# lambdaclass/AES_zero_knowledge_proof_circuit

Hardware: AMD Instinct MI355X
Metric: AES-ECB blocks proven/sec (Marlin), proof verifies (higher is better)
Workload: dtype u32 limbs (253-bit Fr / 377-bit Fq modular integers)

## Files before the change

aes_zero_knowledge_proof_circuit_amd/api.py:

```python
import ctypes as C
import os

import numpy as np

HERE = os.path.dirname(os.path.abspath(__file__))
CIRCUIT_AES, CIRCUIT_OPS_XOR, CIRCUIT_OPS_ADD = 0, 1, 2
CIRCUIT_AES_CBC = 3
CIRCUIT_AES_CTR = 4
CIRCUIT_AES_GCM = 5
KEY_NO_TABLES = 1
PARITY = "parity"


class ZkAesError(RuntimeError):
    """The Err(..) side of the reference's anyhow::Result."""


def lib_path():
    return os.path.join(HERE, "libzkaes.so")


_lib = None


# ... 627 lines not shown
    return out.raw[:32 * n]


def z_poly_from_w(w, x_poly, n):
    out = C.create_string_buffer(32 * (n + 1))
    _check(lib().zkaes_z_poly_from_w(bytes(w), C.c_size_t(len(w) // 32), bytes(x_poly), C.c_uint32(len(x_poly) // 32), C.c_size_t(n), out))
    return out.raw


def ntt_padded(field_id, data_mont_bytes, n, inverse=False, coset_c=0, lg_big=0):
    out = C.create_string_buffer(32 * n)
    _check(lib().zkaes_ntt_padded(int(field_id), bytes(data_mont_bytes), C.c_size_t(len(data_mont_bytes) // 32), C.c_size_t(n), 1 if inverse else 0, int(coset_c), int(lg_big), out))
    return out.raw


def ntt_scaled(g, data_mont_bytes, n, inverse=False):
    out = C.create_string_buffer(32 * n)
    _check(lib().zkaes_ntt_scaled(bytes(g), bytes(data_mont_bytes), C.c_size_t(len(data_mont_bytes) // 32), C.c_size_t(n), 1 if inverse else 0, out))
    return out.raw


def _arith_ops():
    t = {}
    for base, f, n in ((0, "fr377", 8), (16, "fr381", 8), (32, "fq377", 12), (48, "fq381", 12)):
        for i, (name, nin) in enumerate((("mul", 2 * n), ("add", 2 * n), ("sub", 2 * n), ("neg", n), ("dbl", n), ("inverse", n), ("from_i64", 2), ("pow_u64", n + 2), ("from_raw", n), ("to_raw", n))):
            t["%s.%s" % (f, name)] = (base + i, nin, n)
    for base, f in ((64, "fq377x28"), (96, "fq381x28")):
        ops = [("mul", 28, 14), ("sqr", 14, 14), ("fma2", 56, 14), ("add", 28, 14), ("add_lazy", 28, 14), ("dbl_lazy", 14, 14)]
        ops += [("sub%d" % k, 28, 14) for k in (2, 3, 4, 5, 6, 7)] + [("sub_lazy%d" % k, 28, 14) for k in (2, 3)]
        ops += [("canonical", 14, 14), ("product_is_zero", 14, 1), ("is_zero_mod_p", 14, 1), ("from_std", 12, 14), ("to_std", 14, 12)]
        if f == "fq377x28":
            ops.append(("mul_biased", 28, 14))
        for i, (name, nin, nout) in enumerate(ops):
            t["%s.%s" % (f, name)] = (base + i, nin, nout)
    for base, f in ((128, "fr377x29"), (160, "fr381x29")):
        ops = [("mul", 18, 9), ("dot2", 36, 9), ("dot3", 54, 9), ("dot4", 72, 9), ("add", 18, 9), ("add_lazy", 18, 9)]
        ops += [("sub%d" % k, 18, 9) for k in (1, 2, 4, 8)] + [("sub_lazy2", 18, 9), ("normalized", 9, 9), ("shl5", 9, 9)]
        ops += [("canonical%d" % k, 9, 9) for k in (0, 1, 4)] + [("reduce_by_top_limb", 9, 9), ("twiddle_from_std", 8, 9), ("split", 8, 9), ("pack", 9, 8)]
        for i, (name, nin, nout) in enumerate(ops):
            t["%s.%s" % (f, name)] = (base + i, nin, nout)
    for i, (name, nin, nout) in enumerate((("te_madd", 98, 56), ("te_add", 112, 56), ("te_dbl", 56, 56), ("te_neg", 56, 56), ("te_to_std_point", 56, 48), ("niels_from_weierstrass", 24, 43),
                                           ("te_madd_hot", 142, 98), ("te_add_quad", 112, 56), ("te_dbl_quad", 56, 56))):
        t["te377.%s" % name] = (192 + i, nin, nout)
    for base, f in ((208, "w377"), (216, "w381")):
        for i, (name, nin, nout) in enumerate((("madd28", 84, 57), ("add28", 112, 56), ("dbl28", 56, 56), ("neg28", 56, 56), ("to_std_point", 56, 48))):
            t["%s.%s" % (f, name)] = (base + i, nin, nout)
    return t


ARITH_OPS = _arith_ops()
ARITH_QUAD_OPS = ("te377.te_add_quad", "te377.te_dbl_quad")


def arith_probe(op_name, cases):
    op, nin, nout = ARITH_OPS[op_name]
    cases = bytes(cases)
    n, rest = divmod(len(cases), 4 * nin)
    if rest:
        raise ZkAesError("arith_probe: %s takes %d words per case" % (op_name, nin))
    out = C.create_string_buffer(4 * nout * n or 1)
    _check(lib().zkaes_arith_probe(int(op), cases, C.c_size_t(n), out))
    return out.raw[:4 * nout * n]


def msm(curve_id, bases_bytes, scalars_bytes):
    n = len(scalars_bytes) // 32
    out = C.create_string_buffer(96)
    inf = C.c_int()
    _check(lib().zkaes_msm(int(curve_id), bytes(bases_bytes), bytes(scalars_bytes), C.c_size_t(n), out, C.byref(inf)))
    return out.raw, bool(inf.value)


def g1_sum(curve_id, points):
    n = len(points)
    buf = b"".join(bytes(p[0]) for p in points)
    inf = (C.c_int * max(n, 1))(*[1 if p[1] else 0 for p in points])
    out = C.create_string_buffer(96)
    oinf = C.c_int()
    _check(lib().zkaes_g1_sum(int(curve_id), buf, inf, C.c_size_t(n), out, C.byref(oinf)))
    return out.raw, bool(oinf.value)


def msm_sharded_plan(curve_id, n_total):
    c, w, b = C.c_int(), C.c_int(), C.c_size_t()
    _check(lib().zkaes_msm_sharded_plan(int(curve_id), C.c_size_t(n_total), C.byref(c), C.byref(w), C.byref(b)))
    return c.value, w.value, b.value


def msm_window_sums_dev(curve_id, bases_bytes, scalars_bytes, n_total, dev_ptr, dev_bytes):
    n = len(scalars_bytes) // 32
    _check(lib().zkaes_msm_window_sums_dev(int(curve_id), bytes(bases_bytes), bytes(scalars_bytes), C.c_size_t(n), C.c_size_t(n_total), C.c_void_p(dev_ptr), C.c_size_t(dev_bytes)))


def msm_fold_window_sums_dev(curve_id, dev_ptr, world, n_total):
    out = C.create_string_buffer(96)
    inf = C.c_int()
    _check(lib().zkaes_msm_fold_window_sums_dev(int(curve_id), C.c_void_p(dev_ptr), int(world), C.c_size_t(n_total), out, C.byref(inf)))
    return out.raw, bool(inf.value)


def msm_fold_partials_dev(curve_id, dev_ptr, world):
    out = C.create_string_buffer(96)
    inf = C.c_int()
    _check(lib().zkaes_msm_fold_partials_dev(int(curve_id), C.c_void_p(dev_ptr), int(world), out, C.byref(inf)))
    return out.raw, bool(inf.value)


def msm_table(curve_id, bases_bytes, scalars_bytes, window_bits, srs=False):
    n = len(scalars_bytes) // 32
    out = C.create_string_buffer(96)
    inf = C.c_int()
    if srs:
        if int(curve_id) != 377:
            raise ValueError("the SRS (twisted Edwards) table path exists for BLS12-377 only")
        _check(lib().zkaes_msm_table_srs(bytes(bases_bytes), bytes(scalars_bytes), C.c_size_t(n), int(window_bits), out, C.byref(inf)))
    else:
        _check(lib().zkaes_msm_table(int(curve_id), bytes(bases_bytes), bytes(scalars_bytes), C.c_size_t(n), int(window_bits), out, C.byref(inf)))
    return out.raw, bool(inf.value)


def msm_bench(curve_id, bases_bytes, scalars_bytes, reps=3):
    n = len(scalars_bytes) // 32
    t, a = C.c_double(), C.c_double()
    _check(lib().zkaes_msm_bench(int(curve_id), bytes(bases_bytes), bytes(scalars_bytes), C.c_size_t(n), int(reps), C.byref(t), C.byref(a)))
    return t.value, a.value


def msm_bench_synth(n, window_bits=0, reps=3, want_point=False):
    t, a = C.c_double(), C.c_double()
    out = C.create_string_buffer(96)
    _check(lib().zkaes_msm_bench_synth(C.c_size_t(n), int(window_bits), int(reps), C.byref(t), C.byref(a), out))
    return (t.value, a.value, out.raw) if want_point else (t.value, a.value)


def set_default_contexts(n):
    _check(lib().zkaes_set_default_contexts(C.c_size_t(n)))


def srs_hold(hold=True):
    _check(lib().zkaes_srs_hold(1 if hold else 0))


def int_rate_bench(seconds=0.5):
    out = (C.c_double * 8)()
    _check(lib().zkaes_int_rate_bench(C.c_double(seconds), out))
    return {"fq_products_per_s": out[0], "fq_stream_sclk_mhz": out[1], "mad_per_s": 378.0 * out[0], "hot_loop_l2_additions_per_s": out[2], "hot_loop_l2_sclk_mhz": out[3],
            "hot_loop_cycles_per_addition_per_wave": out[4], "rounds": int(out[5])}


def stream_copy_bench(nbytes=1 << 30, reps=20):
    g = C.c_double()
    _check(lib().zkaes_stream_copy_bench(C.c_size_t(nbytes), int(reps), C.byref(g)))
    return g.value


def mem_info():
    f, t = C.c_uint64(), C.c_uint64()
    _check(lib().zkaes_mem_info(C.byref(f), C.byref(t)))
    return int(f.value), int(t.value)


def msm_stats(reset=False):
    out = (C.c_double * 5)()
    _check(lib().zkaes_msm_stats(out, 1 if reset else 0))
    return dict(accumulate_ms=out[0], total_ms=out[1], points=int(out[2]), launches=int(out[3]), pairs=int(out[4]))
```

aes_zero_knowledge_proof_circuit_amd/csrc/arith_probe.cuh:

```cuda
#pragma once
#include "ff29.cuh"
#include "te28.cuh"

namespace zk {
namespace probe {

template <class T> ZK_HD T ld(const uint32_t *in) { T r; for (int i = 0; i < T::N; i++) r.l[i] = in[i]; return r; }
template <class T> ZK_HD void st(uint32_t *out, const T &v) { for (int i = 0; i < T::N; i++) out[i] = v.l[i]; }
struct OpBase { static constexpr bool QUAD = false; };

#define ZK_PROBE_UN(NAME, EXPR)                                                                                                                   \
    template <class T> struct NAME : OpBase { static constexpr int NIN = T::N, NOUT = T::N;                                                       \
        ZK_HD static void run(const uint32_t *in, uint32_t *out, uint64_t) { const T a = ld<T>(in); st<T>(out, EXPR); } };
#define ZK_PROBE_BIN(NAME, EXPR)                                                                                                                  \
    template <class T> struct NAME : OpBase { static constexpr int NIN = 2 * T::N, NOUT = T::N;                                                   \
        ZK_HD static void run(const uint32_t *in, uint32_t *out, uint64_t) { const T a = ld<T>(in), b = ld<T>(in + T::N); st<T>(out, EXPR); } };
#define ZK_PROBE_BIN_K(NAME, EXPR)                                                                                                                \
    template <class T, int K> struct NAME : OpBase { static constexpr int NIN = 2 * T::N, NOUT = T::N;                                            \
        ZK_HD static void run(const uint32_t *in, uint32_t *out, uint64_t) { const T a = ld<T>(in), b = ld<T>(in + T::N); st<T>(out, EXPR); } };
ZK_PROBE_BIN(Mul, a * b)
ZK_PROBE_BIN(Add, a + b)
ZK_PROBE_BIN(Sub, a - b)
ZK_PROBE_UN(Neg, a.neg())
ZK_PROBE_UN(Dbl, a.dbl())
// ... 32 lines not shown
    ZK_HD static void run(const uint32_t *in, uint32_t *out, uint64_t bias) { st<G>(out, G::mul_biased(ld<G>(in), ld<G>(in + G::N), bias)); } };

template <class S, int M> struct Dot : OpBase { static constexpr int NIN = 2 * M * S::N, NOUT = S::N;
    ZK_HD static void run(const uint32_t *in, uint32_t *out, uint64_t) {
        S a[M], b[M];
        for (int i = 0; i < M; i++) { a[i] = ld<S>(in + i * S::N); b[i] = ld<S>(in + (M + i) * S::N); }
        st<S>(out, S::template dot<M>(a, b));
    } };
template <class P> struct TwiddleFromStd : OpBase { static constexpr int NIN = P::N, NOUT = 9;
    ZK_HD static void run(const uint32_t *in, uint32_t *out, uint64_t) { st<Fp29<P>>(out, Fp29<P>::twiddle_from_std(ld<Fp<P>>(in))); } };
template <class P> struct Split29 : OpBase { static constexpr int NIN = P::N, NOUT = 9;
    ZK_HD static void run(const uint32_t *in, uint32_t *out, uint64_t) { st<Fp29<P>>(out, Fp29<P>::split(in)); } };
template <class P> struct Pack29 : OpBase { static constexpr int NIN = 9, NOUT = P::N;
    ZK_HD static void run(const uint32_t *in, uint32_t *out, uint64_t) { ld<Fp29<P>>(in).pack(out); } };

constexpr int GW = 14, PTW = 4 * GW, NIW = 3 * GW;
template <class P> ZK_HD AccTE<P> ld_te(const uint32_t *in) { AccTE<P> a; a.x = ld<FpMsm<P>>(in); a.y = ld<FpMsm<P>>(in + GW); a.z = ld<FpMsm<P>>(in + 2 * GW); a.t = ld<FpMsm<P>>(in + 3 * GW); return a; }
template <class P> ZK_HD void st_te(uint32_t *out, const AccTE<P> &a) { st(out, a.x); st(out + GW, a.y); st(out + 2 * GW, a.z); st(out + 3 * GW, a.t); }
template <class P> ZK_HD Acc28<P> ld_acc(const uint32_t *in) { Acc28<P> a; a.x = ld<FpMsm<P>>(in); a.y = ld<FpMsm<P>>(in + GW); a.zz = ld<FpMsm<P>>(in + 2 * GW); a.zzz = ld<FpMsm<P>>(in + 3 * GW); return a; }
template <class P> ZK_HD void st_acc(uint32_t *out, const Acc28<P> &a) { st(out, a.x); st(out + GW, a.y); st(out + 2 * GW, a.zz); st(out + 3 * GW, a.zzz); }
template <class P> ZK_HD Niels28<P> ld_niels(const uint32_t *in) {
    Niels28<P> n; n.ymx = ld<FpMsm<P>>(in); n.ypx = ld<FpMsm<P>>(in + GW); n.td = ld<FpMsm<P>>(in + 2 * GW);
    for (int i = 0; i < 6; i++) n.pad[i] = 0;
    return n;
}
template <class P> ZK_HD void st_niels(uint32_t *out, const Niels28<P> &n) { st(out, n.ymx); st(out + GW, n.ypx); st(out + 2 * GW, n.td); }
template <class P> ZK_HD void st_xyzz(uint32_t *out, const XYZZ<Fp<P>> &o) { st(out, o.x); st(out + P::N, o.y); st(out + 2 * P::N, o.zz); st(out + 3 * P::N, o.zzz); }

struct TeMadd : OpBase { using P = Fq377P; static constexpr int NIN = PTW + NIW, NOUT = PTW;
    ZK_HD static void run(const uint32_t *in, uint32_t *out, uint64_t) { AccTE<P> a = ld_te<P>(in); te_madd<P>(a, ld_niels<P>(in + PTW)); st_te<P>(out, a); } };
struct TeAdd : OpBase { using P = Fq377P; static constexpr int NIN = 2 * PTW, NOUT = PTW;
    ZK_HD static void run(const uint32_t *in, uint32_t *out, uint64_t) { AccTE<P> a = ld_te<P>(in); te_add<P>(a, ld_te<P>(in + PTW)); st_te<P>(out, a); } };
struct TeDbl : OpBase { using P = Fq377P; static constexpr int NIN = PTW, NOUT = PTW;
    ZK_HD static void run(const uint32_t *in, uint32_t *out, uint64_t) { AccTE<P> a = ld_te<P>(in); te_dbl<P>(a); st_te<P>(out, a); } };
struct TeNeg : OpBase { using P = Fq377P; static constexpr int NIN = PTW, NOUT = PTW;
    ZK_HD static void run(const uint32_t *in, uint32_t *out, uint64_t) { st_te<P>(out, te_neg<P>(ld_te<P>(in))); } };
struct TeToStd : OpBase { using P = Fq377P; static constexpr int NIN = PTW, NOUT = 4 * P::N;
    ZK_HD static void run(const uint32_t *in, uint32_t *out, uint64_t) { st_xyzz<P>(out, te_to_std_point<P>(ld_te<P>(in))); } };
struct NielsFromW : OpBase { using P = Fq377P; static constexpr int NIN = 2 * P::N, NOUT = NIW + 1;
    ZK_HD static void run(const uint32_t *in, uint32_t *out, uint64_t) {
        Affine<Fp<P>> p; p.x = ld<Fp<P>>(in); p.y = ld<Fp<P>>(in + P::N);
        bool bad = false;
        st_niels<P>(out, niels_from_weierstrass(p, &bad));
        out[NIW] = bad ? 1u : 0u;
    } };
struct TeMaddHot : OpBase { using P = Fq377P; static constexpr int NIN = PTW + 2 * NIW + 2, NOUT = PTW + NIW;
    ZK_HD static void run(const uint32_t *in, uint32_t *out, uint64_t bias) {
        AccTE<P> a = ld_te<P>(in);
        Niels28<P> n = ld_niels<P>(in + PTW);
        const Niels28<P> next = ld_niels<P>(in + PTW + NIW);
        te_madd_hot<P>(a, n, in[PTW + 2 * NIW] != 0, &next, in[PTW + 2 * NIW + 1] != 0, bias);
        st_te<P>(out, a); st_niels<P>(out + PTW, n);
    } };
template <class P> struct Madd28 : OpBase { static constexpr int NIN = PTW + 2 * GW, NOUT = PTW + 1;
    ZK_HD static void run(const uint32_t *in, uint32_t *out, uint64_t) {
        Acc28<P> a = ld_acc<P>(in);
        Affine28<P> q; q.x = ld<FpMsm<P>>(in + PTW); q.y = ld<FpMsm<P>>(in + PTW + GW);
        const bool ok = madd28<P>(a, q);
        st_acc<P>(out, a); out[PTW] = ok ? 1u : 0u;
    } };
template <class P> struct Add28 : OpBase { static constexpr int NIN = 2 * PTW, NOUT = PTW;
    ZK_HD static void run(const uint32_t *in, uint32_t *out, uint64_t) { Acc28<P> a = ld_acc<P>(in); add28<P>(a, ld_acc<P>(in + PTW)); st_acc<P>(out, a); } };
template <class P> struct Dbl28 : OpBase { static constexpr int NIN = PTW, NOUT = PTW;
    ZK_HD static void run(const uint32_t *in, uint32_t *out, uint64_t) { Acc28<P> a = ld_acc<P>(in); dbl28<P>(a); st_acc<P>(out, a); } };
template <class P> struct Neg28 : OpBase { static constexpr int NIN = PTW, NOUT = PTW;
    ZK_HD static void run(const uint32_t *in, uint32_t *out, uint64_t) { st_acc<P>(out, neg28<P>(ld_acc<P>(in))); } };
template <class P> struct ToStdPoint28 : OpBase { static constexpr int NIN = PTW, NOUT = 4 * P::N;
    ZK_HD static void run(const uint32_t *in, uint32_t *out, uint64_t) { st_xyzz<P>(out, to_std_point<P>(ld_acc<P>(in))); } };

struct TeAddQuad { using P = Fq377P; static constexpr bool QUAD = true; static constexpr int NIN = 2 * PTW, NOUT = PTW;
#if defined(__HIPCC__)
    __device__ __forceinline__ static void run_quad(const uint32_t *in, uint32_t *out, int q) { st(out + q * GW, te_add_quad<P>(ld<FpMsm<P>>(in + q * GW), ld<FpMsm<P>>(in + PTW + q * GW), q)); }
#endif
};
struct TeDblQuad { using P = Fq377P; static constexpr bool QUAD = true; static constexpr int NIN = PTW, NOUT = PTW;
#if defined(__HIPCC__)
    __device__ __forceinline__ static void run_quad(const uint32_t *in, uint32_t *out, int q) { st(out + q * GW, te_dbl_quad<P>(ld<FpMsm<P>>(in + q * GW), q)); }
#endif
};

#define ZK_PROBE_FP(X, B, F)                                                                                                                      \
    X(B + 0, Mul<F>) X(B + 1, Add<F>) X(B + 2, Sub<F>) X(B + 3, Neg<F>) X(B + 4, Dbl<F>) X(B + 5, Inverse<F>) X(B + 6, FromI64<F>) X(B + 7, PowU64<F>)       \
    X(B + 8, FromRaw<F>) X(B + 9, ToRaw<F>)
#define ZK_PROBE_FP28(X, B, P)                                                                                                                    \
    X(B + 0, Mul<Fp28<P>>) X(B + 1, Sqr<Fp28<P>>) X(B + 2, Fma2<Fp28<P>>) X(B + 3, Add<Fp28<P>>) X(B + 4, AddLazy<Fp28<P>>) X(B + 5, DblLazy<Fp28<P>>)          \
    X(B + 6, SubK<Fp28<P>, 2>) X(B + 7, SubK<Fp28<P>, 3>) X(B + 8, SubK<Fp28<P>, 4>) X(B + 9, SubK<Fp28<P>, 5>) X(B + 10, SubK<Fp28<P>, 6>) X(B + 11, SubK<Fp28<P>, 7>) \
    X(B + 12, SubLazyK<Fp28<P>, 2>) X(B + 13, SubLazyK<Fp28<P>, 3>) X(B + 14, Canonical<Fp28<P>>) X(B + 15, ProductIsZero<Fp28<P>>) X(B + 16, IsZeroModP<Fp28<P>>)   \
    X(B + 17, FromStd28<P>) X(B + 18, ToStd28<P>)
#define ZK_PROBE_FP29(X, B, P)                                                                                                                    \
    X(B + 0, Mul<Fp29<P>>) X(B + 1, Dot<Fp29<P>, 2>) X(B + 2, Dot<Fp29<P>, 3>) X(B + 3, Dot<Fp29<P>, 4>) X(B + 4, Add<Fp29<P>>) X(B + 5, AddLazy<Fp29<P>>)       \
    X(B + 6, SubK<Fp29<P>, 1>) X(B + 7, SubK<Fp29<P>, 2>) X(B + 8, SubK<Fp29<P>, 4>) X(B + 9, SubK<Fp29<P>, 8>) X(B + 10, SubLazyK<Fp29<P>, 2>)                \
    X(B + 11, Normalized<Fp29<P>>) X(B + 12, Shl5<Fp29<P>>) X(B + 13, CanonicalLog<Fp29<P>, 0>) X(B + 14, CanonicalLog<Fp29<P>, 1>) X(B + 15, CanonicalLog<Fp29<P>, 4>) \
    X(B + 16, ReduceTop<Fp29<P>>) X(B + 17, TwiddleFromStd<P>) X(B + 18, Split29<P>) X(B + 19, Pack29<P>)
#define ZK_PROBE_W28(X, B, P) X(B + 0, Madd28<P>) X(B + 1, Add28<P>) X(B + 2, Dbl28<P>) X(B + 3, Neg28<P>) X(B + 4, ToStdPoint28<P>)
#define ZK_PROBE_OPS(X)                                                                                                                           \
    ZK_PROBE_FP(X, 0, Fr377) ZK_PROBE_FP(X, 16, Fr381) ZK_PROBE_FP(X, 32, Fq377) ZK_PROBE_FP(X, 48, Fq381)                                         \
    ZK_PROBE_FP28(X, 64, Fq377P) X(64 + 19, MulBiased<Fp28<Fq377P>>) ZK_PROBE_FP28(X, 96, Fq381P)                                                  \
    ZK_PROBE_FP29(X, 128, Fr377P) ZK_PROBE_FP29(X, 160, Fr381P)                                                                                    \
    X(192, TeMadd) X(193, TeAdd) X(194, TeDbl) X(195, TeNeg) X(196, TeToStd) X(197, NielsFromW) X(198, TeMaddHot) X(199, TeAddQuad) X(200, TeDblQuad) \
    ZK_PROBE_W28(X, 208, Fq377P) ZK_PROBE_W28(X, 216, Fq381P)

template <class O> struct Tag { using type = O; };
template <class Fn> bool dispatch(int op, Fn &&fn) {
    switch (op) {
#define ZK_PROBE_CASE(ID, ...) case ID: fn(Tag<__VA_ARGS__>{}); return true;
        ZK_PROBE_OPS(ZK_PROBE_CASE)
#undef ZK_PROBE_CASE
        default: return false;
    }
}
constexpr int MAX_OP_ID = 224;
constexpr size_t MAX_CASES = (size_t)1 << 16;

}
}
```

aes_zero_knowledge_proof_circuit_amd/csrc/capi_kernels.hip:

```cpp
#include "../../include/zkaes.h"
#include <cstring>
#include <string>
#include <vector>
#include "hip_util.hpp"
#include "marlin.hpp"
#include "te28.cuh"
#include <algorithm>
#include <chrono>

typedef unsigned int v4u __attribute__((ext_vector_type(4)));
__global__ void __launch_bounds__(256) k_stream_copy(uint4 *__restrict__ dst_, const uint4 *__restrict__ src_, size_t n16) {
    v4u *dst = (v4u *)dst_; const v4u *src = (const v4u *)src_;
    size_t base = (size_t)blockIdx.x * 1024 + threadIdx.x;
    if (base + 768 < n16) {
        v4u v0 = __builtin_nontemporal_load(src + base), v1 = __builtin_nontemporal_load(src + base + 256);
        v4u v2 = __builtin_nontemporal_load(src + base + 512), v3 = __builtin_nontemporal_load(src + base + 768);
        __builtin_nontemporal_store(v0, dst + base); __builtin_nontemporal_store(v1, dst + base + 256);
        __builtin_nontemporal_store(v2, dst + base + 512); __builtin_nontemporal_store(v3, dst + base + 768);
    } else {
        for (size_t i = base; i < n16; i += 256) dst[i] = src[i];
    }
}


// ... 58 lines not shown
    if (!data) throw std::invalid_argument("zkaes_ntt: null data");
    zk::gpu::require_device();
    StreamGuard s;
    DevPtr<Fr> a(n), b(n);
    zk::gpu::h2d(a, data, n * sizeof(Fr), s);
    if (coset_c) zk::gpu::ntt_coset<Fr>(b, a, n, lg, inverse != 0, coset_c, lg_big, s);
    else zk::gpu::ntt<Fr>(b, a, n, lg, inverse != 0, s);
    zk::gpu::d2h(data, b, n * sizeof(Fr), s);
}
template <class Fr> void run_ntt_batch(uint8_t *data, size_t n, int count, int inverse, const int *coset_c, int lg_big) {
    const int lg = exact_log2(n, "zkaes_ntt_batch");
    if (count < 1 || count > 12) throw std::invalid_argument("zkaes_ntt_batch: 1..12 transforms");
    if (!data) throw std::invalid_argument("zkaes_ntt_batch: null data");
    zk::gpu::require_device();
    StreamGuard s;
    DevPtr<Fr> a((size_t)count * n), b((size_t)count * n);
    zk::gpu::h2d(a, data, (size_t)count * n * sizeof(Fr), s);
    zk::gpu::NttJob<Fr> jobs[12];
    for (int i = 0; i < count; i++) jobs[i] = zk::gpu::NttJob<Fr>{b + (size_t)i * n, a + (size_t)i * n, coset_c ? coset_c[i] : 0};
    zk::gpu::ntt_batch<Fr>(jobs, count, n, lg, inverse != 0, lg_big, s);
    zk::gpu::d2h(data, b, (size_t)count * n * sizeof(Fr), s);
}
template <class Fq> void give_affine(const zk::Affine<Fq> &a, uint8_t *out_xy, int *out_inf) {
    if (out_inf) *out_inf = a.is_inf() ? 1 : 0;
    if (out_xy) { memcpy(out_xy, a.x.l, 48); memcpy(out_xy + 48, a.y.l, 48); }
}
template <class Curve> void run_msm(const uint8_t *bases, const uint8_t *scalars, size_t n, uint8_t *out_xy, int *out_inf, int reps, double *ms_total, double *ms_acc) {
    using Fq = typename Curve::Fq; using Fr = typename Curve::Fr;
    if (n && (!bases || !scalars)) throw std::invalid_argument("zkaes_msm: null argument");
    if (n >= ((size_t)1 << 30)) throw std::invalid_argument("zkaes_msm: too many points");
    zk::gpu::require_device();
    StreamGuard s;
    DevPtr<zk::Affine<Fq>> db(n);
    DevPtr<Fr> ds(n);
    zk::gpu::h2d(db, bases, n * 96, s); zk::gpu::h2d(ds, scalars, n * 32, s);
    DevPtr<zk::Affine28<typename Curve::FqP>> db28(n);
    zk::gpu::convert_bases<Curve>(db28, db, n, s);
    zk::gpu::sync(s);
    WorkspaceGuard ws;
    zk::XYZZ<Fq> r = zk::gpu::msm<Curve>(ws, db28, ds, n, s);
    if (reps > 0) {
        zk::gpu::MsmStats before = zk::gpu::msm_stats(false);
        EventGuard e0, e1;
        zk::gpu::event_record(e0, s);
        for (int i = 0; i < reps; i++) r = zk::gpu::msm<Curve>(ws, db28, ds, n, s);
        zk::gpu::event_record(e1, s);
        float ms = zk::gpu::event_elapsed_ms(e0, e1);
        zk::gpu::MsmStats after = zk::gpu::msm_stats(false);
        if (ms_total) *ms_total = ms / reps;
        if (ms_acc) *ms_acc = (after.accumulate_ms - before.accumulate_ms) / reps;
    }
    give_affine(r.to_affine(), out_xy, out_inf);
}
template <class Curve, bool EDWARDS> void run_msm_table(const uint8_t *bases, const uint8_t *scalars, size_t n, int c, uint8_t *out_xy, int *out_inf) {
    using Fq = typename Curve::Fq; using Fr = typename Curve::Fr;
    if (c < 2 || c > 22) throw std::invalid_argument("window bits must be in [2, 22]");
    if (n && (!bases || !scalars)) throw std::invalid_argument("zkaes_msm_table: null argument");
    zk::gpu::require_device();
    const size_t nt = (size_t)zk::gpu::table_windows<Curve>(c);
    if ((uint64_t)nt * n >= (1ull << 30)) throw std::invalid_argument("zkaes_msm_table: n x table copies exceeds the 2^30 base indices of one MSM");
    StreamGuard s;
    DevPtr<zk::Affine<Fq>> tab(nt * n);
    DevPtr<Fr> ds(n);
    zk::gpu::h2d(tab, bases, n * 96, s); zk::gpu::h2d(ds, scalars, n * 32, s);
    zk::gpu::build_window_tables<Curve>(tab, n, c, s);
    WorkspaceGuard ws;
    zk::Affine<Fq> a;
    if constexpr (EDWARDS) {
        DevPtr<zk::Niels28<typename Curve::FqP>> tabte(nt * n);
        zk::gpu::convert_bases_te<Curve>(tabte, tab, nt * n, s);
        a = zk::gpu::msm_table<Curve>(ws, tabte, n, 0, c, ds, n, s).to_affine();
    } else {
        DevPtr<zk::Affine28<typename Curve::FqP>> tab28(nt * n);
        zk::gpu::convert_bases<Curve>(tab28, tab, nt * n, s);
        a = zk::gpu::msm_table<Curve>(ws, tab28, n, 0, c, ds, n, s).to_affine();
    }
    give_affine(a, out_xy, out_inf);
}
template <class Curve> void run_msm_window_sums_dev(const uint8_t *bases, const uint8_t *scalars, size_t n_local, size_t n_total, void *dev_out, size_t dev_out_bytes) {
    using Fq = typename Curve::Fq; using Fr = typename Curve::Fr;
    zk::gpu::require_device();
    int c = 0, nwin = 0;
    zk::gpu::msm_sharded_plan<Curve>(n_total, &c, &nwin);
    if (!dev_out || dev_out_bytes < (size_t)nwin * sizeof(zk::XYZZ<Fq>)) throw std::invalid_argument("zkaes_msm_window_sums_dev: device buffer too small for the window sums");
    if (n_local > n_total) throw std::invalid_argument("zkaes_msm_window_sums_dev: n_local > n_total");
    if (n_local && (!bases || !scalars)) throw std::invalid_argument("zkaes_msm_window_sums_dev: null argument");
    StreamGuard s;
    DevPtr<zk::Affine<Fq>> db(n_local);
    DevPtr<Fr> ds(n_local);
    zk::gpu::h2d(db, bases, n_local * 96, s); zk::gpu::h2d(ds, scalars, n_local * 32, s);
    DevPtr<zk::Affine28<typename Curve::FqP>> db28(n_local);
    zk::gpu::convert_bases<Curve>(db28, db, n_local, s);
    WorkspaceGuard ws;
    zk::gpu::msm_window_sums_device<Curve>(ws, db28, ds, n_local, n_total, (zk::XYZZ<Fq> *)dev_out, s);
}
constexpr int MAX_FOLD_WORLD = 4096;
template <class Curve> void run_msm_fold_dev(const void *dev_in, int world, size_t n_total, uint8_t *out_xy, int *out_inf) {
    using Fq = typename Curve::Fq;
    if (!dev_in || world < 1 || world > MAX_FOLD_WORLD) throw std::invalid_argument("zkaes_msm_fold_window_sums_dev: bad arguments (world must be 1..4096)");
    zk::gpu::require_device();
    StreamGuard s;
    give_affine(zk::gpu::msm_fold_window_sums_device<Curve>((const zk::XYZZ<Fq> *)dev_in, world, n_total, s).to_affine(), out_xy, out_inf);
}
template <class Curve> void run_g1_sum(const uint8_t *points_xy, const int *inf, size_t n, uint8_t *out_xy, int *out_inf) {
    using Fq = typename Curve::Fq;
    zk::XYZZ<Fq> acc = zk::XYZZ<Fq>::inf();
    for (size_t i = 0; i < n; i++) {
        if (inf && inf[i]) continue;
        zk::Affine<Fq> a;
        memcpy(a.x.l, points_xy + 96 * i, 48); memcpy(a.y.l, points_xy + 96 * i + 48, 48);
        acc.add(zk::XYZZ<Fq>::from_affine(a));
    }
    zk::Affine<Fq> r = acc.to_affine();
    *out_inf = r.is_inf() ? 1 : 0;
    memcpy(out_xy, r.x.l, 48); memcpy(out_xy + 48, r.y.l, 48);
}

using PF = zk::gpu::F;
PF load_f(const uint8_t *b, const char *who) {
    if (!b) throw std::invalid_argument(std::string(who) + ": null field element");
    PF x; memcpy(x.l, b, 32); return x;
}
void need(bool ok, const char *who, const char *what) { if (!ok) throw std::invalid_argument(std::string(who) + ": " + what); }
constexpr size_t POLY_MAX = (size_t)1 << 28;
// ... 1 lines not shown
    DevPtr<PF> d(count ? count : 1);
    zk::gpu::h2d(d, host, count * sizeof(PF), s);
    return d;
}
template <class Fr> void run_ntt_padded(const uint8_t *in, size_t in_len, size_t n, int inverse, int coset_c, int lg_big, uint8_t *out) {
    const int lg = exact_log2(n, "zkaes_ntt_padded");
    need(in_len <= n, "zkaes_ntt_padded", "in_len must not exceed n");
    need(out && (in || !in_len), "zkaes_ntt_padded", "null argument");
    need(coset_c >= 0, "zkaes_ntt_padded", "coset index must not be negative");
    zk::gpu::require_device();
    StreamGuard s;
    DevPtr<Fr> a(in_len ? in_len : 1), b(n);
    zk::gpu::h2d(a, in, in_len * sizeof(Fr), s);
    if (coset_c) zk::gpu::ntt_coset<Fr>(b, a, in_len, lg, inverse != 0, coset_c, lg_big, s);
    else zk::gpu::ntt<Fr>(b, a, in_len, lg, inverse != 0, s);
    zk::gpu::d2h(out, b, n * sizeof(Fr), s);
}
}

extern "C" {
int zkaes_msm_sharded_plan(int curve_id, size_t n_total, int *window_bits, int *n_windows, size_t *bytes_per_rank) {
    return guardk([&] {
        int c = 0, w = 0;
        if (curve_id == 381) zk::gpu::msm_sharded_plan<zk::Bls381>(n_total, &c, &w); else if (curve_id == 377) zk::gpu::msm_sharded_plan<zk::Bls377>(n_total, &c, &w); else throw std::invalid_argument("curve_id must be 377 or 381");
        if (window_bits) *window_bits = c;
        if (n_windows) *n_windows = w;
        if (bytes_per_rank) *bytes_per_rank = (size_t)w * 192;
    });
}
int zkaes_msm_window_sums_dev(int curve_id, const uint8_t *bases, const uint8_t *scalars, size_t n_local, size_t n_total, void *dev_out, size_t dev_out_bytes) {
    return guardk([&] { if (curve_id == 381) run_msm_window_sums_dev<zk::Bls381>(bases, scalars, n_local, n_total, dev_out, dev_out_bytes); else if (curve_id == 377) run_msm_window_sums_dev<zk::Bls377>(bases, scalars, n_local, n_total, dev_out, dev_out_bytes); else throw std::invalid_argument("curve_id must be 377 or 381"); });
}
int zkaes_msm_fold_window_sums_dev(int curve_id, const void *dev_in, int world, size_t n_total, uint8_t *out_xy, int *out_inf) {
    return guardk([&] { if (curve_id == 381) run_msm_fold_dev<zk::Bls381>(dev_in, world, n_total, out_xy, out_inf); else if (curve_id == 377) run_msm_fold_dev<zk::Bls377>(dev_in, world, n_total, out_xy, out_inf); else throw std::invalid_argument("curve_id must be 377 or 381"); });
}
int zkaes_g1_sum(int curve_id, const uint8_t *points_xy, const int *inf, size_t n, uint8_t *out_xy, int *out_inf) {
    return guardk([&] { if (curve_id == 381) run_g1_sum<zk::Bls381>(points_xy, inf, n, out_xy, out_inf); else if (curve_id == 377) run_g1_sum<zk::Bls377>(points_xy, inf, n, out_xy, out_inf); else throw std::invalid_argument("curve_id must be 377 or 381"); });
}
int zkaes_msm_fold_partials_dev(int curve_id, const void *dev_in, int world, uint8_t *out_xy, int *out_inf) {
    return guardk([&] {
        if (!dev_in || world < 1 || world > MAX_FOLD_WORLD) throw std::invalid_argument("zkaes_msm_fold_partials_dev: bad arguments (world must be 1..4096)");
        if (curve_id != 377 && curve_id != 381) throw std::invalid_argument("curve_id must be 377 or 381");
        zk::gpu::require_device();
        StreamGuard s;
        if (curve_id == 377) give_affine(zk::gpu::msm_fold_points_device<zk::Bls377>((const zk::XYZZ<zk::Fq377> *)dev_in, world, s).to_affine(), out_xy, out_inf);
        else give_affine(zk::gpu::msm_fold_points_device<zk::Bls381>((const zk::XYZZ<zk::Fq381> *)dev_in, world, s).to_affine(), out_xy, out_inf);
    });
}
int zkaes_msm_table(int curve_id, const uint8_t *bases, const uint8_t *scalars, size_t n, int window_bits, uint8_t *out_xy, int *out_inf) {
    return guardk([&] { if (curve_id == 381) run_msm_table<zk::Bls381, false>(bases, scalars, n, window_bits, out_xy, out_inf); else if (curve_id == 377) run_msm_table<zk::Bls377, false>(bases, scalars, n, window_bits, out_xy, out_inf); else throw std::invalid_argument("curve_id must be 377 or 381"); });
}
int zkaes_msm_table_srs(const uint8_t *bases, const uint8_t *scalars, size_t n, int window_bits, uint8_t *out_xy, int *out_inf) {
    return guardk([&] { run_msm_table<zk::Bls377, true>(bases, scalars, n, window_bits, out_xy, out_inf); });
}
int zkaes_set_device(int ordinal) { return guardk([&] { HIP_CHECK(hipSetDevice(ordinal)); }); }
int zkaes_ntt(int field_id, uint8_t *data, size_t n, int inverse) {
    return guardk([&] { if (field_id == 381) run_ntt<zk::Fr381>(data, n, inverse, 0, 0); else if (field_id == 377) run_ntt<zk::Fr377>(data, n, inverse, 0, 0); else throw std::invalid_argument("field_id must be 377 or 381"); });
}
int zkaes_ntt_coset(int field_id, uint8_t *data, size_t n, int inverse, int coset_c, int lg_big) {
    return guardk([&] {
        if (coset_c <= 0) throw std::invalid_argument("zkaes_ntt_coset: coset index must be positive");
        if (field_id == 381) run_ntt<zk::Fr381>(data, n, inverse, coset_c, lg_big); else if (field_id == 377) run_ntt<zk::Fr377>(data, n, inverse, coset_c, lg_big); else throw std::invalid_argument("field_id must be 377 or 381");
    });
}
int zkaes_ntt_batch(int field_id, uint8_t *data, size_t n, int count, int inverse, const int *coset_c, int lg_big) {
    return guardk([&] {
        if (field_id == 381) run_ntt_batch<zk::Fr381>(data, n, count, inverse, coset_c, lg_big); else if (field_id == 377) run_ntt_batch<zk::Fr377>(data, n, count, inverse, coset_c, lg_big);
        else throw std::invalid_argument("field_id must be 377 or 381");
    });
}
int zkaes_poly_divide_by_vanishing(const uint8_t *p, size_t len, size_t m, int with_scratch, uint8_t *q, uint8_t *rem_or_null) {
    return guardk([&] {
        const char *who = "zkaes_poly_divide_by_vanishing";
        if (m == 0 || len <= m) throw std::invalid_argument("divide_by_vanishing: dividend shorter than divisor");
        need(p && q, who, "null argument"); need(len <= POLY_MAX, who, "polynomial too long");
        zk::gpu::require_device();
        StreamGuard s;
        DevPtr<PF> dp = upload(p, len, s), dq(len - m), drem(m), scratch;
        size_t scratch_len = 0;
        if (with_scratch) { scratch_len = zk::gpu::divide_by_vanishing_scratch(len, m); scratch.alloc(scratch_len ? scratch_len : 1); }
        zk::gpu::divide_by_vanishing(dq, rem_or_null ? drem.get() : nullptr, dp, len, m, s, with_scratch ? scratch.get() : nullptr, scratch_len);
        zk::gpu::d2h(q, dq, (len - m) * sizeof(PF), s);
        if (rem_or_null) zk::gpu::d2h(rem_or_null, drem, m * sizeof(PF), s);
    });
}
int zkaes_poly_divide_by_linear(const uint8_t *p, size_t len, const uint8_t z[32], uint8_t *q) {
    return guardk([&] {
        const char *who = "zkaes_poly_divide_by_linear";
        const PF zf = load_f(z, who);
        need(len <= POLY_MAX, who, "polynomial too long"); need(len < 2 || (p && q), who, "null argument");
        if (len < 2) return;
        zk::gpu::require_device();
        StreamGuard s;
        const size_t scratch_len = zk::gpu::divide_by_linear_scratch(len);
        DevPtr<PF> dp = upload(p, len, s), dq(len - 1), scratch(scratch_len);
        zk::gpu::divide_by_linear(dq, dp, len, zf, scratch, scratch_len, s);
        zk::gpu::d2h(q, dq, (len - 1) * sizeof(PF), s);
    });
}
int zkaes_poly_eval_multi(const uint8_t *const *polys, const size_t *lens, const uint8_t *x, int count, uint8_t *out) {
    return guardk([&] {
        const char *who = "zkaes_poly_eval_multi";
        need(count >= 1 && count <= 8, who, "1..8 polynomials"); need(polys && lens && x && out, who, "null argument");
        size_t scratch_len = 8;
        for (int i = 0; i < count; i++) { need(lens[i] <= POLY_MAX, who, "polynomial too long"); need(!lens[i] || polys[i], who, "null polynomial"); scratch_len += zk::gpu::poly_eval_scratch(lens[i]); }
        zk::gpu::require_device();
// ... 274 lines not shown
```

aes_zero_knowledge_proof_circuit_amd/csrc/capi_probe.hip:

```cpp
#include "../../include/zkaes.h"
#include <stdexcept>
#include <string>
#include "hip_util.hpp"
#include "gpu.hpp"
#include "arith_probe.cuh"

template <class O> __global__ void __launch_bounds__(64) k_arith_probe(const uint32_t *__restrict__ in, uint32_t n_cases, uint32_t *__restrict__ out) {
    const uint64_t bias = zk::FpMsm<zk::Fq377P>::hot_loop_bias();
    const uint32_t c = blockIdx.x * 64 + threadIdx.x;
    if (c >= n_cases) return;
    uint32_t a[O::NIN], r[O::NOUT];
#pragma unroll
    for (int i = 0; i < O::NIN; i++) a[i] = in[(size_t)c * O::NIN + i];
    O::run(a, r, bias);
#pragma unroll
    for (int i = 0; i < O::NOUT; i++) out[(size_t)c * O::NOUT + i] = r[i];
}
template <class O> __global__ void __launch_bounds__(64) k_arith_probe_quad(const uint32_t *__restrict__ in, uint32_t n_cases, uint32_t *__restrict__ out) {
    const uint32_t t = blockIdx.x * 64 + threadIdx.x, c = t >> 2;
    const int q = (int)(t & 3);
    if (c < n_cases) O::run_quad(in + (size_t)c * O::NIN, out + (size_t)c * O::NOUT, q);
}

extern "C" const char *zkaes_last_error(void);
namespace zk { void capi_set_error(const std::string &); }

namespace {
using zk::gpu::DevPtr; using zk::gpu::StreamGuard;
template <class O> void run_probe(const uint32_t *in, size_t n, uint32_t *out) {
    zk::gpu::require_device();
    StreamGuard s;
    DevPtr<uint32_t> din(n * O::NIN), dout(n * O::NOUT);
    zk::gpu::h2d(din, in, n * O::NIN * sizeof(uint32_t), s);
    hipStream_t hs = (hipStream_t)s.h;
    if constexpr (O::QUAD) k_arith_probe_quad<O><<<(unsigned)((4 * n + 63) / 64), 64, 0, hs>>>(din, (uint32_t)n, dout);
    else k_arith_probe<O><<<(unsigned)((n + 63) / 64), 64, 0, hs>>>(din, (uint32_t)n, dout);
    HIP_LAUNCH_CHECK();
    zk::gpu::d2h(out, dout, n * O::NOUT * sizeof(uint32_t), s);
}
}

extern "C" int zkaes_arith_probe(int op, const uint32_t *in, size_t n_cases, uint32_t *out) {
    try {
        zk::capi_set_error("");
        if (!in || !out) throw std::invalid_argument("zkaes_arith_probe: null argument");
        if (n_cases == 0 || n_cases > zk::probe::MAX_CASES) throw std::invalid_argument("zkaes_arith_probe: n_cases must be in [1, 65536]");
        if (!zk::probe::dispatch(op, [&](auto tag) { run_probe<typename decltype(tag)::type>(in, n_cases, out); })) throw std::invalid_argument("zkaes_arith_probe: unknown op " + std::to_string(op));
        return 0;
    } catch (const std::exception &e) { zk::capi_set_error(e.what()); return 1; }
    catch (...) { zk::capi_set_error("unknown error"); return 1; }
}
```

aes_zero_knowledge_proof_circuit_amd/csrc/consts32.h:

```cpp
#pragma once
#include <stdint.h>
#define FR377_BITS 253
#define FR377_P_INIT {0x00000001u, 0x0a118000u, 0xd0000001u, 0x59aa76feu, 0x5c37b001u, 0x60b44d1eu, 0x9a2ca556u, 0x12ab655eu}
#define FR377_ONE_INIT {0xfffffff3u, 0x7d1c7fffu, 0x6ffffff2u, 0x7257f50fu, 0x512c0feeu, 0x16d81575u, 0x2bbb9a9du, 0x0d4bda32u}
#define FR377_R2_INIT {0xb861857bu, 0x25d577bau, 0x8860591fu, 0xcc2c27b5u, 0xe5dc8593u, 0xa7cc008fu, 0xeff1c939u, 0x011fdae7u}
static const uint32_t FR377_P[8] = {0x00000001u, 0x0a118000u, 0xd0000001u, 0x59aa76feu, 0x5c37b001u, 0x60b44d1eu, 0x9a2ca556u, 0x12ab655eu};
static const uint32_t FR377_ONE[8] = {0xfffffff3u, 0x7d1c7fffu, 0x6ffffff2u, 0x7257f50fu, 0x512c0feeu, 0x16d81575u, 0x2bbb9a9du, 0x0d4bda32u};
static const uint32_t FR377_R2[8] = {0xb861857bu, 0x25d577bau, 0x8860591fu, 0xcc2c27b5u, 0xe5dc8593u, 0xa7cc008fu, 0xeff1c939u, 0x011fdae7u};
static const uint32_t FR377_INV = 0xffffffffu;
#define FR381_BITS 255
#define FR381_P_INIT {0x00000001u, 0xffffffffu, 0xfffe5bfeu, 0x53bda402u, 0x09a1d805u, 0x3339d808u, 0x299d7d48u, 0x73eda753u}
#define FR381_ONE_INIT {0xfffffffeu, 0x00000001u, 0x00034802u, 0x5884b7fau, 0xecbc4ff5u, 0x998c4fefu, 0xacc5056fu, 0x1824b159u}
#define FR381_R2_INIT {0xf3f29c6du, 0xc999e990u, 0x87925c23u, 0x2b6cedcbu, 0x7254398fu, 0x05d31496u, 0x9f59ff11u, 0x0748d9d9u}
static const uint32_t FR381_P[8] = {0x00000001u, 0xffffffffu, 0xfffe5bfeu, 0x53bda402u, 0x09a1d805u, 0x3339d808u, 0x299d7d48u, 0x73eda753u};
static const uint32_t FR381_ONE[8] = {0xfffffffeu, 0x00000001u, 0x00034802u, 0x5884b7fau, 0xecbc4ff5u, 0x998c4fefu, 0xacc5056fu, 0x1824b159u};
static const uint32_t FR381_R2[8] = {0xf3f29c6du, 0xc999e990u, 0x87925c23u, 0x2b6cedcbu, 0x7254398fu, 0x05d31496u, 0x9f59ff11u, 0x0748d9d9u};
static const uint32_t FR381_INV = 0xffffffffu;
#define FQ377_BITS 377
#define FQ377_P_INIT {0x00000001u, 0x8508c000u, 0x30000000u, 0x170b5d44u, 0xba094800u, 0x1ef3622fu, 0x00f5138fu, 0x1a22d9f3u, 0x6ca1493bu, 0xc63b05c0u, 0x17c510eau, 0x01ae3a46u}
#define FQ377_ONE_INIT {0xffffff68u, 0x02cdffffu, 0x7fffffb1u, 0x51409f83u, 0x8a7d3ff2u, 0x9f7db3a9u, 0x6e7c6305u, 0x7b4e97b7u, 0x803c84e8u, 0x4cf495bfu, 0xe2fdf49au, 0x008d6661u}
#define FQ377_R2_INIT {0x9400cd22u, 0xb786686cu, 0xb00431b1u, 0x0329fcaau, 0x62d6b46du, 0x22a5f111u, 0x827dc3acu, 0xbfdf7d03u, 0x41790bf9u, 0x837e92f0u, 0x1e914b88u, 0x006dfccbu}
static const uint32_t FQ377_P[12] = {0x00000001u, 0x8508c000u, 0x30000000u, 0x170b5d44u, 0xba094800u, 0x1ef3622fu, 0x00f5138fu, 0x1a22d9f3u, 0x6ca1493bu, 0xc63b05c0u, 0x17c510eau, 0x01ae3a46u};
static const uint32_t FQ377_ONE[12] = {0xffffff68u, 0x02cdffffu, 0x7fffffb1u, 0x51409f83u, 0x8a7d3ff2u, 0x9f7db3a9u, 0x6e7c6305u, 0x7b4e97b7u, 0x803c84e8u, 0x4cf495bfu, 0xe2fdf49au, 0x008d6661u};
static const uint32_t FQ377_R2[12] = {0x9400cd22u, 0xb786686cu, 0xb00431b1u, 0x0329fcaau, 0x62d6b46du, 0x22a5f111u, 0x827dc3acu, 0xbfdf7d03u, 0x41790bf9u, 0x837e92f0u, 0x1e914b88u, 0x006dfccbu};
static const uint32_t FQ377_INV = 0xffffffffu;
#define FQ381_BITS 381
#define FQ381_P_INIT {0xffffaaabu, 0xb9feffffu, 0xb153ffffu, 0x1eabfffeu, 0xf6b0f624u, 0x6730d2a0u, 0xf38512bfu, 0x64774b84u, 0x434bacd7u, 0x4b1ba7b6u, 0x397fe69au, 0x1a0111eau}
#define FQ381_ONE_INIT {0x0002fffdu, 0x76090000u, 0xc40c0002u, 0xebf4000bu, 0x53c758bau, 0x5f489857u, 0x70525745u, 0x77ce5853u, 0xa256ec6du, 0x5c071a97u, 0xfa80e493u, 0x15f65ec3u}
#define FQ381_R2_INIT {0x1c341746u, 0xf4df1f34u, 0x09d104f1u, 0x0a76e6a6u, 0x4c95b6d5u, 0x8de5476cu, 0x939d83c0u, 0x67eb88a9u, 0xb519952du, 0x9a793e85u, 0x92cae3aau, 0x11988fe5u}
static const uint32_t FQ381_P[12] = {0xffffaaabu, 0xb9feffffu, 0xb153ffffu, 0x1eabfffeu, 0xf6b0f624u, 0x6730d2a0u, 0xf38512bfu, 0x64774b84u, 0x434bacd7u, 0x4b1ba7b6u, 0x397fe69au, 0x1a0111eau};
static const uint32_t FQ381_ONE[12] = {0x0002fffdu, 0x76090000u, 0xc40c0002u, 0xebf4000bu, 0x53c758bau, 0x5f489857u, 0x70525745u, 0x77ce5853u, 0xa256ec6du, 0x5c071a97u, 0xfa80e493u, 0x15f65ec3u};
static const uint32_t FQ381_R2[12] = {0x1c341746u, 0xf4df1f34u, 0x09d104f1u, 0x0a76e6a6u, 0x4c95b6d5u, 0x8de5476cu, 0x939d83c0u, 0x67eb88a9u, 0xb519952du, 0x9a793e85u, 0x92cae3aau, 0x11988fe5u};
static const uint32_t FQ381_INV = 0xfffcfffdu;
#define FR377_TWO_ADICITY 47
static const uint32_t FR377_ROOT_MONT[8] = {0xda3ad648u, 0xaf80da4du, 0xfc381dacu, 0x5e223adbu, 0xb2f92525u, 0x03ba0666u, 0x3befb0ceu, 0x0f906c5bu};
static const uint32_t FR377_GEN_MONT[8] = {0xfffffed3u, 0x296c7fffu, 0x6ffffec7u, 0x92921665u, 0x92860e69u, 0x4c01534du, 0xb9819970u, 0x0c79cfc4u};
#define FR381_TWO_ADICITY 32
static const uint32_t FR381_ROOT_MONT[8] = {0x5f0e466au, 0xb9b58d8cu, 0x1819d7ecu, 0x5b1b4c80u, 0x52a31e64u, 0x0af53ae3u, 0x19e9b27bu, 0x5bf3addau};
static const uint32_t FR381_GEN_MONT[8] = {0xfffffff1u, 0x0000000eu, 0x00189c0fu, 0x17e363d3u, 0x6f8457b0u, 0xff9c5787u, 0x8fc5a8c4u, 0x35133220u};
static const uint32_t G1_377_X_MONT[12] = {0x772451f4u, 0x260f33b9u, 0x169d5658u, 0xc54dd773u, 0x69a510ddu, 0x5c1551c4u, 0x425e1698u, 0x761662e4u, 0x6f065272u, 0xc97d78ccu, 0xb361fd4du, 0x00a41206u};
static const uint32_t G1_377_Y_MONT[12] = {0xb8cb81f3u, 0x8193961fu, 0x5f44adb8u, 0x00638d4cu, 0xd4daf54au, 0xfafaf3dau, 0xd655cd18u, 0xc27849e2u, 0x01d52814u, 0x2ec3ddb4u, 0x26303c71u, 0x007da933u};
static const uint32_t G1_377_B_MONT[12] = {0xffffff68u, 0x02cdffffu, 0x7fffffb1u, 0x51409f83u, 0x8a7d3ff2u, 0x9f7db3a9u, 0x6e7c6305u, 0x7b4e97b7u, 0x803c84e8u, 0x4cf495bfu, 0xe2fdf49au, 0x008d6661u};
static const uint32_t G1_381_X_MONT[12] = {0xfd530c16u, 0x5cb38790u, 0x9976fff5u, 0x7817fc67u, 0x143ba1c1u, 0x154f95c7u, 0xf3d0e747u, 0xf0ae6acdu, 0x21dbf440u, 0xedce6eccu, 0x9e0bfb75u, 0x12017741u};
static const uint32_t G1_381_Y_MONT[12] = {0x0ce72271u, 0xbaac93d5u, 0x7918fd8eu, 0x8c22631au, 0x570725ceu, 0xdd595f13u, 0x50405194u, 0x51ac5829u, 0xad0059c0u, 0x0e1c8c3fu, 0x5008a26au, 0x0bbc3efcu};
static const uint32_t G1_381_B_MONT[12] = {0x000cfff3u, 0xaa270000u, 0xfc34000au, 0x53cc0032u, 0x6b0a807fu, 0x478fe97au, 0xe6ba24d7u, 0xb1d37ebeu, 0xbf78ab2fu, 0x8ec9733bu, 0x3d83de7eu, 0x09d64551u};
static const uint32_t FQ377_NONRES_MONT[12] = {0x000002fau, 0xfc0b8000u, 0xe000018bu, 0x97d39cf6u, 0xbfa05044u, 0x2072420fu, 0xd97c3802u, 0xcbbcbd50u, 0x5813f9ebu, 0x0baf1ec3u, 0xc0945ad2u, 0x009974a2u};
static const uint32_t G2_377_B_C0_MONT[12] = {0x00000000u, 0x00000000u, 0x00000000u, 0x00000000u, 0x00000000u, 0x00000000u, 0x00000000u, 0x00000000u, 0x00000000u, 0x00000000u, 0x00000000u, 0x00000000u};
static const uint32_t G2_377_B_C1_MONT[12] = {0x66666685u, 0x80722666u, 0x899999a9u, 0x8df55926u, 0xd64f34cfu, 0x7fe4561au, 0xb6e4f01bu, 0xb95da6d8u, 0xfc142743u, 0x4b747cccu, 0x70f49f43u, 0x0039c3fau};
static const uint32_t G2_377_X_C0_MONT[12] = {0x756a6edbu, 0x87e4cb96u, 0xfa9b9c4bu, 0x99aa13a4u, 0x38b86463u, 0xd702cf5fu, 0x24c167edu, 0x7ed4ce79u, 0xa9c5329fu, 0x1b447e91u, 0x63a498b7u, 0x0084963fu};
static const uint32_t G2_377_X_C1_MONT[12] = {0x76a27e27u, 0x8554a791u, 0xf79e64a3u, 0xba4edb07u, 0xfb15b037u, 0xe2dc99bdu, 0xf9d797f7u, 0xe7d8740fu, 0x6aa2ea12u, 0x140c90e8u, 0x95c622d3u, 0x00cab5f2u};
static const uint32_t G2_377_Y_C0_MONT[12] = {0xb82c312du, 0x64b8008du, 0x2f2e86dfu, 0xaf626ec3u, 0x16b1c4f8u, 0x071c6b62u, 0xf2e6ecb7u, 0x4938329du, 0x5683d6b6u, 0xce9093a6u, 0x84028208u, 0x004ded59u};
static const uint32_t G2_377_Y_C1_MONT[12] = {0xcce05131u, 0x3546c7c3u, 0x92e9b1eau, 0xaf87996cu, 0x3c252000u, 0xa026db71u, 0x40cfecb9u, 0x5ba778b8u, 0xf989bc4cu, 0x104fd72au, 0x7dc1f32bu, 0x00b841e4u};
#define G1_377_COFACTOR_LIMBS 4
static const uint32_t G1_377_COFACTOR[4] = {0x00000000u, 0x00000000u, 0x30000000u, 0x170b5d44u};
#define G2_377_COFACTOR_LIMBS 16
static const uint32_t G2_377_COFACTOR[16] = {0x00000001u, 0x00000000u, 0x90000000u, 0x452217ccu, 0xba094800u, 0xa0f3622fu, 0x6676bd09u, 0xd693e8c3u, 0xfae2e189u, 0x8c505634u, 0xe1dcc40cu, 0xfbb36b00u, 0xa6f6a829u, 0xddd88d99u, 0x8ae9562au, 0x0026ba55u};
static const uint64_t BLS12_377_X = 0x8508c00000000001ULL;
#define BLS12_377_FINAL_EXP_LIMBS 63
static const uint32_t BLS12_377_FINAL_EXP[63] = {0x00000002u, 0x0a118000u, 0xb0000001u, 0xcf664765u, 0xe68b3800u, 0xc242c0cbu, 0x0c71fe44u, 0xa47662d7u, 0x40a4efb0u, 0xffc594c3u, 0xb3ee4dc0u, 0x9d4f7bf7u, 0x22a24f5bu, 0x44805f5au, 0xa89998a8u, 0x2f530533u, 0x224ec7d8u, 0x5d716080u, 0xca519301u, 0x1368df8du, 0x17a058bfu, 0xef0199c1u, 0xe54706e1u, 0x4f168ac9u, 0x2eb34320u, 0x9c8f5a7bu, 0x7d50f353u, 0x7c976b42u, 0x027819b8u, 0xf3d95a3eu, 0xbdae7647u, 0x7fdda393u, 0x60f50b26u, 0xbee2660du, 0xe5546ebfu, 0x82fe2158u, 0x7e9fadc0u, 0xdc712eceu, 0x0db9ec0du, 0x898b8d13u, 0xc2bf75cfu, 0x555a89a4u, 0xac9eb555u, 0xa3f771b0u, 0xf2cfbf1fu, 0x7e79b0b2u, 0xfca5f4ebu, 0x13793762u, 0x04e2a70cu, 0x2ddd28e6u, 0xc8fd5918u, 0x621371f3u, 0x8c5374bau, 0x7f41de8du, 0xff3f31bfu, 0xd2f282b4u, 0x748856b5u, 0x4a82c4feu, 0x66da4c66u, 0x06c94748u, 0xaf4801c5u, 0x41d9d66cu, 0x0134ed81u};
#define FQ377_TE_S_INIT {0xd831a0a2u, 0x6de9ca9au, 0x0eb51c8eu, 0xa8aff422u, 0x93607959u, 0x5a76e6c5u, 0xd3806339u, 0x57f38956u, 0xa0c6fe30u, 0xc50636f4u, 0xf52bfd14u, 0x018f4652u}
#define FQ377_TE_SI_INIT {0x8894e1e4u, 0x3fabdfd0u, 0xcc1f55aau, 0xcbf921ddu, 0x460edc0cu, 0xd17deff1u, 0x7897028du, 0xd394e81eu, 0x0912681au, 0xc29c995du, 0xaff9d568u, 0x01515e6cu}
#define FQ377_TE_F_INIT {0xead605e4u, 0xfb7c0ab8u, 0xe2752c7au, 0x363b93d1u, 0x144be536u, 0xd2246835u, 0x429f2077u, 0xeb8bf6ddu, 0x0234d423u, 0x3a9efda2u, 0xba0c72a4u, 0x013c7943u}
#define FQ377_TE_FI_INIT {0xfd76a6bdu, 0x3b092ce1u, 0xbba32683u, 0x925230d9u, 0xe991a197u, 0x872d5d2fu, 0xa82b2ab0u, 0x8367c527u, 0xef662a15u, 0xe285bbb3u, 0x9283e729u, 0x0160527au}
#define FQ377_TE_K2D_INIT {0x44a706c6u, 0xf24b7e84u, 0x80faa8fau, 0xeae02375u, 0x7ef38fa5u, 0x0f4d7cf2u, 0xc5f2bb26u, 0x5597097du, 0x0d95a93eu, 0x8bf6c1ddu, 0xfbff628au, 0x01784602u}
#define FQ377_TE_SIF_INIT {0xa38cfd11u, 0xface0c97u, 0x0adb8383u, 0x8cc7c229u, 0xd44ae9cbu, 0x4765cd5fu, 0x22354029u, 0x9ae986d8u, 0x252ab9bdu, 0xc3dc7860u, 0xc8942395u, 0x00486011u}
#define FQ377_TE_K2D_28_INIT {0x706c521u, 0xdf4444au, 0x8fa7e68u, 0x371b2aau, 0xdd6cd3du, 0xebe579eu, 0x3577a6au, 0x1d3f1c6u, 0x2ada318u, 0x2a73d9du, 0x7da6ef5u, 0xce09495u, 0xfed4ab8u, 0x0001813u}
#define FQ377_TE_SI_28_INIT {0x4e1e338u, 0x09d0889u, 0x5a9d7bdu, 0x00869f5u, 0xcb9f841u, 0xfcb79bcu, 0x14fcb3bu, 0xd78b460u, 0x9add89fu, 0x66e4a72u, 0xcdeb434u, 0x3157be7u, 0x5ed67e0u, 0x000140eu}
#define FQ377_TE_SIF_28_INIT {0xcfd10d5u, 0x9457a38u, 0x383e475u, 0x7e96cb8u, 0x388e8d9u, 0xd00b5abu, 0xd32ebe1u, 0x0c15e03u, 0x5ac3c51u, 0xa270ad8u, 0xe68d2ebu, 0xbe54908u, 0x8029609u, 0x00001c4u}
static const uint8_t ARK_TEST_RNG_SEED[32] = {1,0,0,0, 23,0,0,0, 200,1,0,0, 210,30,0,0, 0,0,0,0, 0,0,0,0, 0,0,0,0, 0,0,0,0};
```

aes_zero_knowledge_proof_circuit_amd/csrc/ff28.cuh:

```cuda
#pragma once
#include "ff.cuh"

namespace zk {

template <class P>
struct Fp28 {
    static constexpr int N = 14;
    static constexpr uint32_t MASK = (1u << 28) - 1;
    uint32_t l[N];

    ZK_HD static constexpr uint32_t mod28(int i) {
        int bit = 28 * i, w = bit >> 5, sh = bit & 31;
        uint64_t two = (w < P::N ? (uint64_t)P::mod(w) : 0) | ((w + 1 < P::N ? (uint64_t)P::mod(w + 1) : 0) << 32);
        return (uint32_t)(two >> sh) & MASK;
    }
    static constexpr uint32_t PINV = P::INV & MASK;

    ZK_HD static Fp28 zero() { Fp28 r; for (int i = 0; i < N; i++) r.l[i] = 0; return r; }
    ZK_HD bool limbs_zero() const { uint32_t o = 0; for (int i = 0; i < N; i++) o |= l[i]; return o == 0; }
    ZK_HD static bool product_is_zero(const Fp28 &v) {
        if (v.l[0] != 0u && v.l[0] != mod28(0)) return false;
        uint32_t z0 = 0, zp = 0;
#pragma unroll
        for (int i = 0; i < N; i++) { z0 |= v.l[i]; zp |= v.l[i] ^ mod28(i); }
// ... 124 lines not shown
        return r;
    }
    ZK_HD static uint64_t hot_loop_bias() {
        uint64_t v = MASK;
#if defined(__HIP_DEVICE_COMPILE__)
        asm volatile("" : "+s"(v));
#endif
        return v;
    }
    ZK_HD static Fp28 fma2(const Fp28 &a, const Fp28 &b, const Fp28 &c, const Fp28 &d) {
        uint64_t t[2 * N];
#pragma unroll
        for (int i = 0; i < 2 * N; i++) t[i] = 0;
#pragma unroll
        for (int i = 0; i < N; i++) {
#pragma unroll
            for (int j = 0; j < N; j++) t[i + j] += (uint64_t)a.l[j] * b.l[i];
#pragma unroll
            for (int j = 0; j < N; j++) t[i + j] += (uint64_t)c.l[j] * d.l[i];
            reduce_row(t, i);
        }
        Fp28 r;
        uint64_t cy = 0;
#pragma unroll
        for (int i = 0; i < N - 1; i++) { uint64_t v = t[N + i] + cy; r.l[i] = (uint32_t)v & MASK; cy = v >> 28; }
        r.l[N - 1] = (uint32_t)(t[2 * N - 1] + cy);
        return r;
    }
    ZK_HD Fp28 sqr() const {
        uint64_t t[2 * N];
#pragma unroll
        for (int i = 0; i < 2 * N; i++) t[i] = 0;
        uint32_t d[N];
#pragma unroll
        for (int i = 0; i < N; i++) d[i] = l[i] << 1;
#pragma unroll
        for (int i = 0; i < N; i++) {
            t[2 * i] += (uint64_t)l[i] * l[i];
#pragma unroll
            for (int j = i + 1; j < N; j++) t[i + j] += (uint64_t)d[i] * l[j];
        }
#pragma unroll
        for (int i = 0; i < N; i++) {
            reduce_row(t, i);
        }
        Fp28 r;
        uint64_t c = 0;
#pragma unroll
        for (int i = 0; i < N - 1; i++) { uint64_t v = t[N + i] + c; r.l[i] = (uint32_t)v & MASK; c = v >> 28; }
        r.l[N - 1] = (uint32_t)(t[2 * N - 1] + c);
        return r;
    }

    ZK_HD Fp28 canonical() const {
        Fp28 v = *this;
#pragma unroll
        for (int k = 5; k >= 0; k--) {
            int64_t c = 0;
            uint32_t tl[N];
#pragma unroll
            for (int i = 0; i < N - 1; i++) { int64_t x = (int64_t)v.l[i] - ((int64_t)mod28(i) << k) + c; tl[i] = (uint32_t)x & MASK; c = x >> 28; }
            int64_t top = (int64_t)v.l[N - 1] - ((int64_t)mod28(N - 1) << k) + c;
            if (top >= 0) {
#pragma unroll
                for (int i = 0; i < N - 1; i++) v.l[i] = tl[i];
                v.l[N - 1] = (uint32_t)top;
            }
        }
        return v;
    }
    ZK_HD bool is_zero_mod_p() const { return canonical().limbs_zero(); }

    ZK_HD static Fp28 from_std(const Fp<P> &a) {
        Fp28 s = split(a.l);
        return s * k_2_400();
    }
    ZK_HD Fp<P> to_std() const {
        Fp28 y = (*this * k_2_384()).canonical();
        Fp<P> r;
        y.pack(r.l);
        return r;
    }
    ZK_HD static Fp28 k_2_384() { Fp<P> o = Fp<P>::one(); return split(o.l); }
    ZK_HD static Fp28 k_one() { return k_2_392(); }
    ZK_HD static Fp28 k_2_392() {
        Fp<P> v = Fp<P>::one();
        for (int i = 0; i < 8; i++) v = v.dbl();
        return split(v.l);
    }
    ZK_HD static Fp28 k_2_400() {
        Fp<P> v = Fp<P>::one();
        for (int i = 0; i < 16; i++) v = v.dbl();
        return split(v.l);
    }
};

using Fq377x28 = Fp28<Fq377P>;
using Fq381x28 = Fp28<Fq381P>;

}
```

aes_zero_knowledge_proof_circuit_amd/csrc/gpu.hpp:

```cpp
#pragma once
#include <cstddef>
#include <cstdint>
#include <stdexcept>
#include <string>
#include <utility>
#include <vector>
#include "ec.cuh"
#include "te28.cuh"

namespace zk {
namespace gpu {

struct GpuError : std::runtime_error { using std::runtime_error::runtime_error; };
typedef void *stream_t;

int device_count();
void require_device();
int current_device();
void set_device(int ordinal);
void *dmalloc(size_t bytes);
#ifdef ZKAES_MEASURE
int knockin();
#endif
size_t mem_free_bytes();
// ... 46 lines not shown
    H h = nullptr;
    Handle() : h(Create()) {}
    explicit Handle(H adopt) : h(adopt) {}
    Handle(const Handle &) = delete; Handle &operator=(const Handle &) = delete;
    Handle(Handle &&o) noexcept : h(o.h) { o.h = nullptr; }
    Handle &operator=(Handle &&o) noexcept { if (this != &o) { Destroy(h); h = o.h; o.h = nullptr; } return *this; }
    ~Handle() { Destroy(h); }
    operator H() const { return h; }
};
using StreamGuard = Handle<stream_t, stream_create, stream_destroy>;
using EventGuard = Handle<void *, event_create, event_destroy>;
struct PinnedPtr {
    void *host = nullptr, *dev = nullptr;
    PinnedPtr() = default;
    PinnedPtr(const PinnedPtr &) = delete; PinnedPtr &operator=(const PinnedPtr &) = delete;
    ~PinnedPtr() { pinned_free(host); }
    void alloc(size_t bytes) { pinned_free(host); host = dev = nullptr; host = pinned_alloc(bytes); dev = pinned_device_address(host); }
};

enum : int { OP_MSM_BUCKETS = 0, OP_MSM_SECOND_BASES = 1, OP_MSM_CLASS_SUM = 2 };
struct OpRecord { std::vector<std::pair<uint64_t, int>> ntt , msm ; };
void oplog_begin();
OpRecord oplog_end();
void oplog_ntt(uint64_t n, int count);
void oplog_msm(uint64_t points, int kind);

template <class Fr> void ntt(Fr *dst, const Fr *src, size_t in_len, int lg, bool inverse, stream_t s);
template <class Fr> void ntt_coset(Fr *dst, const Fr *src, size_t in_len, int lg, bool inverse, int coset_c, int lg_big, stream_t s);
template <class Fr> struct NttJob { Fr *dst; const Fr *src; int coset_c; };
template <class Fr> void ntt_batch(const NttJob<Fr> *jobs, int count, size_t in_len, int lg, bool inverse, int lg_big, stream_t s);
template <class Fr> DevPtr<void> coset_power_table(const Fr &g, size_t n, stream_t s);
template <class Fr> void ntt_scaled(Fr *dst, const Fr *src, size_t in_len, int lg, bool inverse, const void *table, stream_t s);
template <class Fr> const Fr *domain_elements(int lg);

struct MsmWorkspace;
MsmWorkspace *msm_workspace_create();
void msm_workspace_destroy(MsmWorkspace *ws);
using WorkspaceGuard = Handle<MsmWorkspace *, msm_workspace_create, msm_workspace_destroy>;
template <class Curve> void convert_bases(Affine28<typename Curve::FqP> *dst, const Affine<typename Curve::Fq> *src, size_t n, stream_t s);
template <class Curve>
XYZZ<typename Curve::Fq> msm(MsmWorkspace *ws, const Affine28<typename Curve::FqP> *bases, const typename Curve::Fr *scalars, size_t n, stream_t s);
template <class Curve>
void msm_prepare(MsmWorkspace *ws, const typename Curve::Fr *scal1, size_t n1, const typename Curve::Fr *scal2, size_t n2, size_t val_off2, stream_t s, int force_c = 0);
template <class Curve>
XYZZ<typename Curve::Fq> msm_finish(MsmWorkspace *ws, const Affine28<typename Curve::FqP> *bases, stream_t s);
template <class Curve> void convert_bases_te(Niels28<typename Curve::FqP> *dst, const Affine<typename Curve::Fq> *src, size_t n, stream_t s);
template <class Curve>
XYZZ<typename Curve::Fq> msm(MsmWorkspace *ws, const Niels28<typename Curve::FqP> *bases, const typename Curve::Fr *scalars, size_t n, stream_t s);
template <class Curve>
XYZZ<typename Curve::Fq> msm_finish(MsmWorkspace *ws, const Niels28<typename Curve::FqP> *bases, stream_t s);
template <class Curve>
void msm_finish2(MsmWorkspace *ws, const Niels28<typename Curve::FqP> *bases, const Niels28<typename Curve::FqP> *bases2, XYZZ<typename Curve::Fq> *out, stream_t s);
template <class Curve>
XYZZ<typename Curve::Fq> msm_table(MsmWorkspace *ws, const Niels28<typename Curve::FqP> *tables, size_t stride, size_t off, int c, const typename Curve::Fr *scalars, size_t n, stream_t s);
template <class Curve>
bool class_sum(MsmWorkspace *ws, const Niels28<typename Curve::FqP> *bases, const int8_t *vals, size_t n, XYZZ<typename Curve::Fq> *out, stream_t s);
template <class Curve> void msm_sharded_plan(size_t n_total, int *window_bits, int *n_windows);
template <class Curve>
void msm_window_sums_device(MsmWorkspace *ws, const Affine28<typename Curve::FqP> *bases, const typename Curve::Fr *scalars, size_t n_local, size_t n_total,
                            XYZZ<typename Curve::Fq> *dev_out, stream_t s);
template <class Curve>
XYZZ<typename Curve::Fq> msm_fold_window_sums_device(const XYZZ<typename Curve::Fq> *dev_in, int world, size_t n_total, stream_t s);
template <class Curve>
void msm_table_sum_device(MsmWorkspace *ws, const Niels28<typename Curve::FqP> *tables, size_t stride, size_t off, int c, const typename Curve::Fr *scalars, size_t n,
                          XYZZ<typename Curve::Fq> *dev_out, stream_t s);
template <class Curve>
XYZZ<typename Curve::Fq> msm_fold_points_device(const XYZZ<typename Curve::Fq> *dev_in, int world, stream_t s);
template <class Curve> int table_windows(int c);
template <class Curve> void build_window_tables(Affine<typename Curve::Fq> *tables, size_t stride, int c, stream_t s);
template <class Curve> void table_next(Affine<typename Curve::Fq> *next, const Affine<typename Curve::Fq> *prev, size_t count, int c, int j, stream_t s);
template <class Curve>
void msm_prepare_table(MsmWorkspace *ws, const typename Curve::Fr *scal1, size_t n1, size_t off1, const typename Curve::Fr *scal2, size_t n2, size_t off2, int c, size_t stride, stream_t s);
template <class Curve>
XYZZ<typename Curve::Fq> msm_table(MsmWorkspace *ws, const Affine28<typename Curve::FqP> *tables, size_t stride, size_t off, int c, const typename Curve::Fr *scalars, size_t n, stream_t s);
template <class Curve>
void fixed_base_powers(Affine<typename Curve::Fq> *out, const Affine<typename Curve::Fq> &base, const typename Curve::Fr &beta, size_t from, size_t count, stream_t s);
template <class Curve>
void fixed_base_scalars(Affine<typename Curve::Fq> *out, const Affine<typename Curve::Fq> &base, const typename Curve::Fr *scalars, size_t count, stream_t s);
template <class Curve>
bool class_sum(MsmWorkspace *ws, const Affine28<typename Curve::FqP> *bases, const int8_t *vals, size_t n, XYZZ<typename Curve::Fq> *out, stream_t s);
struct MsmStats { double accumulate_ms = 0; double total_ms = 0; uint64_t points = 0; uint64_t launches = 0; uint64_t pairs = 0; };
MsmStats msm_stats(bool reset);

}
}

namespace zk {
namespace gpu {
using F = Fr377;

void poly_set_at(F *p, size_t idx, const F &val, stream_t s);
void poly_add_at(F *p, size_t idx, const F &val, stream_t s);
void poly_scale(F *p, const F &sc, size_t n, stream_t s);
void poly_lincomb_n(F *out, size_t n, const F *const *polys, const size_t *lens, const F *scalars, int count, stream_t s);
size_t divide_by_vanishing_scratch(size_t len, size_t m);
void divide_by_vanishing(F *q, F *rem, const F *p, size_t len, size_t m, stream_t s, F *scratch = nullptr, size_t scratch_len = 0);
void divide_by_linear(F *q, const F *p, size_t len, const F &z, F *scratch, size_t scratch_elems, stream_t s);
size_t divide_by_linear_scratch(size_t len);
F poly_eval(const F *p, size_t len, const F &x, F *scratch, stream_t s);
size_t poly_eval_scratch(size_t len);
void poly_eval_multi(const F *const *p, const size_t *len, const F *x, int count, F *out, F *scratch, size_t scratch_elems, stream_t s);
void batch_inverse(F *v, size_t n, const F *post_or_null, stream_t s);
size_t vanishing_quotient_scratch(int lg_n, int ncosets);
void vanishing_quotient_evals(F *const *out, const F *g, int ncosets, const F &a, const F *elems, uint32_t n, int lg_n, F *scratch, size_t scratch_elems, stream_t s);
void f_evals_from_tables(F *out, const F *va, const F *vb, const F *vc, const F &ea, const F &eb, const F &ec, const F *ra, const F *rb, const uint32_t *ri, const uint32_t *ci, size_t k,
                         stream_t s);

void upload_sbox(const uint8_t table[256]);
void aes_trace(uint8_t *trace, size_t trace_stride, const uint8_t *msgs, const uint8_t *keys, uint32_t nproofs, uint32_t nblocks, stream_t s, size_t key_bytes = 16);
void aes_trace_cbc(uint8_t *trace, size_t trace_stride, const uint8_t *msgs, const uint8_t *keys, const uint8_t *ivs, uint32_t nproofs, uint32_t nblocks, stream_t s, size_t key_bytes = 16);
void aes_trace_ctr(uint8_t *trace, size_t trace_stride, const uint8_t *msgs, const uint8_t *keys, const uint8_t *icbs, uint32_t nproofs, uint32_t msg_len, stream_t s, size_t key_bytes = 16);
void aes_trace_gcm(uint8_t *trace, size_t trace_stride, const uint8_t *msgs, const uint8_t *keys, const uint8_t *hdrs, uint32_t nproofs, uint32_t msg_len, uint32_t aad_len, stream_t s, size_t key_bytes = 16);
void ghash_trace(uint8_t *trace, size_t trace_stride, uint32_t nproofs, uint32_t msg_len, uint32_t aad_len, stream_t s, size_t key_bytes = 16);
void witness_expand(uint8_t *z, const uint32_t *desc, uint32_t ncols, const uint8_t *trace, const uint32_t *sbox_in_off, const uint32_t *sbox_tmpl, stream_t s);
void spmv_bits(F *out, int8_t *small_out, size_t rows_out, const uint32_t *rowptr, const uint32_t *col, const int64_t *coeff, size_t rows, const uint8_t *z, stream_t s);
void w_classes(int8_t *out, const uint8_t *z, uint32_t n, uint32_t m, uint32_t num_witness, stream_t s);
void lagrange_scalars(F *lag, F *lag_w, const F *elems, const F &beta, uint32_t n, uint32_t m, stream_t s);
void w_evals(F *out, const uint8_t *z, const F *x_evals, uint32_t n, uint32_t m, uint32_t num_witness, stream_t s);
void bits_to_field(F *out, const uint8_t *z, size_t n, stream_t s);
constexpr uint32_t T_SEG = 32, T_HEAVY_SEGMENTS = 256;
void t_evals(F *out, uint32_t n, F *partial, uint32_t nseg, const uint32_t *col_seg_ptr, const uint32_t *seg_start, const uint32_t *seg_end, const uint32_t *heavy, uint32_t n_heavy,
             const uint32_t *row, const uint8_t *mat, const int64_t *coeff, const F *r_alpha, const F &eta_a, const F &eta_b, const F &eta_c, stream_t s);
uint64_t chacha_field_stream(F *out, size_t count, const uint32_t key[8], int rounds, uint64_t word_pos, void *scratch, size_t scratch_bytes, stream_t s);
void mask_fixup(F *p, size_t n, stream_t s);
void q1_coset_pointwise(F *out, const F *r, const F *za, const F *zb, const F *t, const F *z, const F &ca, const F &cb, const F &cz, const F &eta_a, const F &eta_b, const F &eta_c,
// ... 13 lines not shown
```

aes_zero_knowledge_proof_circuit_amd/csrc/kernels_msm.hip:

```cpp
#include <cstring>
#include <rocprim/device/device_radix_sort.hpp>
#include <rocprim/device/device_scan.hpp>
#include <chrono>
#include <cstdio>
#include <cstdlib>
#include <mutex>
#include <vector>
#include "hip_util.hpp"
#include "te28.cuh"

namespace zk {
namespace gpu {

template <class P> struct WeierLaw { using Params = P; using Base = Affine28<P>; using Acc = Acc28<P>; static constexpr bool edwards = false; };
template <class P> struct EdwardsLaw { using Params = P; using Base = Niels28<P>; using Acc = AccTE<P>; static constexpr bool edwards = true; };

static MsmStats g_stats;
static std::mutex g_stats_mu;
MsmStats msm_stats(bool reset) {
    std::lock_guard<std::mutex> g(g_stats_mu);
    MsmStats s = g_stats;
    if (reset) g_stats = MsmStats();
    return s;
}

constexpr uint32_t VAL_SKIP = 1u << 30, VAL_INDEX = VAL_SKIP - 1;
template <class Fr>
__global__ void k_digits(const Fr *__restrict__ scalars, uint32_t n, uint32_t i_off, uint32_t ntot, uint32_t val_off, int c, int nwin, uint32_t nb,
                         uint32_t *__restrict__ keys, uint32_t *__restrict__ vals) {
    uint32_t i = blockIdx.x * blockDim.x + threadIdx.x;
    if (i >= n) return;
    uint32_t raw[Fr::N + 1];
    scalars[i].to_raw(raw);
    raw[Fr::N] = 0;
    const uint32_t mask = (1u << c) - 1, half = 1u << (c - 1);
    uint32_t carry = 0;
    for (int w = 0; w < nwin; w++) {
        int bit = w * c, limb = bit >> 5, sh = bit & 31;
        uint64_t two = limb <= Fr::N - 1 ? ((uint64_t)raw[limb] | ((uint64_t)raw[limb + 1] << 32)) : 0;
        uint32_t v = ((uint32_t)(two >> sh) & mask) + carry;
        uint32_t neg = 0;
        carry = 0;
        if (v > half) { v = (1u << c) - v; neg = 1u << 31; carry = 1; }
        keys[(size_t)w * ntot + i_off + i] = ((uint32_t)w << (c - 1)) | (v ? v - 1 : 0u);
        vals[(size_t)w * ntot + i_off + i] = v ? ((val_off + i) | neg) : VAL_SKIP;
    }
}

struct TableLayout {
    int nwin, c_hi, n_hi;
    __host__ __device__ int width(int j) const { return j < n_hi ? c_hi : c_hi - 1; }
    __host__ __device__ int offset(int j) const { return j < n_hi ? j * c_hi : n_hi * c_hi + (j - n_hi) * (c_hi - 1); }
};
static TableLayout table_layout(int total_bits, int c) {
    TableLayout L;
    L.nwin = (total_bits + c - 1) / c;
    int base = total_bits / L.nwin, rem = total_bits % L.nwin;
    L.c_hi = base + (rem ? 1 : 0);
    L.n_hi = rem ? rem : L.nwin;
    return L;
}
template <class Fr>
__global__ void k_digits_table(const Fr *__restrict__ scalars, uint32_t n, uint32_t i_off, uint32_t ntot, uint32_t val_off, TableLayout L, uint32_t stride,
                               uint32_t *__restrict__ keys, uint32_t *__restrict__ vals) {
    uint32_t i = blockIdx.x * blockDim.x + threadIdx.x;
    if (i >= n) return;
    uint32_t raw[Fr::N + 1];
    scalars[i].to_raw(raw);
    raw[Fr::N] = 0;
    uint32_t carry = 0;
    for (int w = 0; w < L.nwin; w++) {
        const int c = L.width(w), bit = L.offset(w), limb = bit >> 5, sh = bit & 31;
        const uint32_t mask = (1u << c) - 1, half = 1u << (c - 1);
        uint64_t two = limb <= Fr::N - 1 ? ((uint64_t)raw[limb] | ((uint64_t)raw[limb + 1] << 32)) : 0;
        uint32_t v = ((uint32_t)(two >> sh) & mask) + carry;
        uint32_t neg = 0;
        carry = 0;
        if (v > half) { v = (1u << c) - v; neg = 1u << 31; carry = 1; }
        keys[(size_t)w * ntot + i_off + i] = v ? v - 1 : 0u;
        vals[(size_t)w * ntot + i_off + i] = v ? (((uint32_t)w * stride + val_off + i) | neg) : VAL_SKIP;
    }
}
template <class Fq>
__global__ void __launch_bounds__(64) k_table_next(const Affine<Fq> *__restrict__ prev, Affine<Fq> *__restrict__ next, uint32_t count, int c) {
    constexpr int B = 8;
    uint32_t t = blockIdx.x * blockDim.x + threadIdx.x;
    uint32_t s0 = t * B;
    if (s0 >= count) return;
    uint32_t e = s0 + B < count ? s0 + B : count;
    Fq xs[B], ys[B], zz[B], zzz[B], pre[B];
    Fq acc = Fq::one();
    for (uint32_t i = s0; i < e; i++) {
        XYZZ<Fq> p = XYZZ<Fq>::from_affine(prev[i]);
        for (int k = 0; k < c; k++) p = p.dbl();
        xs[i - s0] = p.x; ys[i - s0] = p.y; zz[i - s0] = p.zz; zzz[i - s0] = p.zzz;
        pre[i - s0] = acc;
        if (!p.zzz.is_zero()) acc = acc * p.zzz;
    }
    acc = acc.inverse();
    for (uint32_t i = e; i-- > s0;) {
        uint32_t q = i - s0;
        if (zzz[q].is_zero()) { next[i] = Affine<Fq>::inf(); continue; }
        Fq zi3 = acc * pre[q];
        acc = acc * zzz[q];
        Fq zi2 = (zi3 * zz[q]).sqr();
        Affine<Fq> a; a.x = xs[q] * zi2; a.y = ys[q] * zi3;
        next[i] = a;
    }
}

__device__ __forceinline__ uint32_t bounds_rank(uint32_t key, int cbits, uint32_t nwin) { return nwin == 1 ? key : (key & ((1u << cbits) - 1)) * nwin + (key >> cbits); }
__device__ __forceinline__ uint32_t bounds_key(uint32_t rank, int cbits, uint32_t nwin) { return nwin == 1 ? rank : ((rank % nwin) << cbits) | (rank / nwin); }
__global__ void k_bounds(const uint32_t *__restrict__ keys, size_t total, int cbits, uint32_t nwin, uint32_t *__restrict__ start, uint32_t *__restrict__ end) {
    size_t i0 = ((size_t)blockIdx.x * blockDim.x + threadIdx.x) * 4;
    if (i0 >= total) return;
    const uint32_t nb = nwin << cbits;
    uint32_t k[6];
    if (i0 + 4 <= total) { uint4 v = *reinterpret_cast<const uint4 *>(keys + i0); k[1] = v.x; k[2] = v.y; k[3] = v.z; k[4] = v.w; }
    else { for (int j = 0; j < 4; j++) k[1 + j] = i0 + j < total ? keys[i0 + j] : 0u; }
    k[0] = i0 ? keys[i0 - 1] : 0u;
    k[5] = i0 + 4 < total ? keys[i0 + 4] : 0u;
// ... 72 lines not shown
        for (int u = 0; u < 8; u++) sum += c[u];
    }
    for (; i0 < nblk; i0++) sum += hist[(size_t)i0 * ORD_BINS + t];
    uint32_t run = block_exclusive(sum);
    for (i0 = 0; i0 + 8 <= nblk; i0 += 8) {
        uint32_t c[8];
#pragma unroll
        for (int u = 0; u < 8; u++) c[u] = hist[(size_t)(i0 + u) * ORD_BINS + t];
#pragma unroll
        for (int u = 0; u < 8; u++) { offs[(size_t)(i0 + u) * ORD_BINS + t] = run; run += c[u]; }
    }
    for (; i0 < nblk; i0++) { const uint32_t c = hist[(size_t)i0 * ORD_BINS + t]; offs[(size_t)i0 * ORD_BINS + t] = run; run += c; }
    uint32_t n = ctrl[0];
    if (n > ovf_cap) n = ovf_cap;
    uint32_t base = 0;
    for (uint32_t c0 = 0; c0 < n; c0 += ORD_BINS) {
        __syncthreads();
        const uint32_t v = c0 + t < n ? ovf_nseg[c0 + t] : 0;
        const uint32_t ex = block_exclusive(v);
        if (c0 + t < n) ovf_off[c0 + t] = base + ex;
        base += part[ORD_BINS - 1];
    }
    __syncthreads();
    if (t == 0) { ovf_off[n] = base; ctrl[1] = n; ctrl[2] = base; ctrl[0] = 0; }
}
__global__ void __launch_bounds__(ORD_THREADS) k_order_scatter(const uint32_t *__restrict__ start, const uint32_t *__restrict__ end, uint32_t nb, uint32_t per_block,
                                                                const uint32_t *__restrict__ offs, uint32_t *__restrict__ order) {
    __shared__ uint32_t h[ORD_BINS];
    for (int b = threadIdx.x; b < ORD_BINS; b += ORD_THREADS) h[b] = 0;
    __syncthreads();
    const uint32_t lo = blockIdx.x * per_block, hi = lo + per_block < nb ? lo + per_block : nb;
    for (uint32_t k = lo + threadIdx.x; k < hi; k += ORD_THREADS) {
        const uint32_t key = order_key(end[k] - start[k]);
        order[offs[(size_t)blockIdx.x * ORD_BINS + key] + atomicAdd(&h[key], 1u)] = k;
    }
}

template <class Law>
__global__ void __launch_bounds__(64, 2) k_accumulate(const typename Law::Base *__restrict__ bases, const uint32_t *__restrict__ vals,
                                                       const uint32_t *__restrict__ start, const uint32_t *__restrict__ end, const uint32_t *__restrict__ order,
                                                       uint32_t nbuckets_total, uint32_t cap, typename Law::Acc *__restrict__ buckets,
                                                       uint32_t *__restrict__ deferred, uint32_t deferred_cap, uint32_t *__restrict__ deferred_count) {
    using P = typename Law::Params;
    using G = FpMsm<P>;
    [[maybe_unused]] uint64_t bias = 0;
    if constexpr (Law::edwards) bias = FpMsm<P>::hot_loop_bias();
    uint32_t t = blockIdx.x * blockDim.x + threadIdx.x;
    if (t >= nbuckets_total) return;
    uint32_t k = order[t];
    uint32_t s = start[k], e = end[k];
    if (e - s > cap) e = s + cap;
    if constexpr (Law::edwards) {
        AccTE<P> acc = te_identity<P>();
        if (s < e) {
            uint32_t idx = vals[s];
            Niels28<P> p = niels_load_signed<P>(bases + (idx & VAL_INDEX), idx >> 31);
            for (uint32_t i = s; i < e; i++) {
                const uint32_t cur = idx;
                if (i + 1 < e) idx = vals[i + 1];
                const Niels28<P> *next = bases + (idx & VAL_INDEX);
                if (cur & VAL_SKIP) { p = niels_load_signed<P>(next, idx >> 31); continue; }
                te_madd_hot<P>(acc, p, cur >> 31, next, idx >> 31, bias);
            }
        }
        buckets[k] = acc;
    } else {
        Acc28<P> acc;
        bool acc_inf = true;
        if (s < e) {
            uint32_t idx = vals[s];
            Affine28<P> nxt = bases[idx & VAL_INDEX];
            for (uint32_t i = s; i < e; i++) {
                Affine28<P> p = nxt;
                uint32_t cur = idx;
                if (i + 1 < e) { idx = vals[i + 1]; nxt = bases[idx & VAL_INDEX]; }
                if ((cur & VAL_SKIP) || p.is_inf()) continue;
                if (cur >> 31) p.y = G::zero().template sub<2>(p.y);
                if (acc_inf) { acc.x = p.x; acc.y = p.y; acc.zz = G::k_one(); acc.zzz = acc.zz; acc_inf = false; continue; }
                if (!madd28(acc, p)) {
                    uint32_t slot = atomicAdd(deferred_count, 1u);
                    if (slot < deferred_cap) { deferred[2 * slot] = k; deferred[2 * slot + 1] = cur; }
                }
            }
        }
        if (acc_inf) acc = inf28<P>();
        buckets[k] = acc;
    }
}
template <class P>
__device__ void accumulate_fixup(const Affine28<P> *__restrict__ bases, Acc28<P> *__restrict__ buckets, const uint32_t *__restrict__ deferred, uint32_t deferred_cap,
                                 const volatile uint32_t *deferred_count) {
    uint32_t n = *deferred_count;
    if (n > deferred_cap) n = deferred_cap;
    for (uint32_t i = 0; i < n; i++) {
        XYZZ<Fp<P>> b = to_std_point<P>(buckets[deferred[2 * i]]);
        uint32_t v = deferred[2 * i + 1];
        Affine<Fp<P>> q = bases[v & VAL_INDEX].to_std();
        b.madd((v >> 31) ? q.neg() : q);
        buckets[deferred[2 * i]] = from_std_point<P>(b);
    }
}

template <class Law>
__global__ void __launch_bounds__(64) k_accumulate_tail(const typename Law::Base *__restrict__ bases, const uint32_t *__restrict__ vals, const uint32_t *__restrict__ start,
                                                            const uint32_t *__restrict__ end, const uint32_t *__restrict__ ctrl, const uint32_t *__restrict__ ovf_bucket,
                                                            const uint32_t *__restrict__ ovf_off, uint32_t max_segments, uint32_t cap,
                                                            typename Law::Acc *__restrict__ partial, typename Law::Acc *__restrict__ buckets, uint32_t *__restrict__ deferred, uint32_t deferred_cap,
                                                            uint32_t *__restrict__ deferred_count) {
    using P = typename Law::Params;
// ... 766 lines not shown
    sync((stream_t)s);
}

template <class Curve>
void table_next(Affine<typename Curve::Fq> *next, const Affine<typename Curve::Fq> *prev, size_t count, int c, int j, stream_t s_) {
    const TableLayout L = table_layout(Curve::Fr::BITS + 1, c);
    if (j < 1 || j >= L.nwin) throw GpuError("table_next: window index out of range");
    uint32_t lanes = (uint32_t)((count + 7) / 8);
    hipLaunchKernelGGL((k_table_next<typename Curve::Fq>), dim3((lanes + 63) / 64), dim3(64), 0, (hipStream_t)s_, prev, next, (uint32_t)count, L.width(j - 1));
    HIP_LAUNCH_CHECK();
}

constexpr int PART_FINE_BITS = 9, PART_FINE = 1 << PART_FINE_BITS, PART_WBITS = 4, PART_KEYS = PART_FINE << PART_WBITS;
constexpr int PART_THREADS = 512, PART_SPT = 2, PART_TILE = PART_THREADS * PART_SPT;
constexpr int PART_MAXW = 1 << PART_WBITS;
constexpr int PART_STAGE = PART_TILE * PART_MAXW;
constexpr uint32_t PART_NBIN_MAX = 1024;
constexpr uint32_t PART_GRID = 512, PART_NONE = 0xffffffffu;
constexpr int PART_FINE_THREADS = 1024, PART_FINE_UNROLL = 8;

template <int NW>
__device__ __forceinline__ void part_digits(const uint32_t (&raw)[NW + 1], const TableLayout &L, uint32_t d[PART_MAXW]) {
    uint32_t carry = 0;
#pragma unroll
    for (int w = 0; w < PART_MAXW; w++) {
        d[w] = PART_NONE;
        if (w < L.nwin) {
            const int c = L.width(w), bit = L.offset(w), limb = bit >> 5, sh = bit & 31;
            const uint32_t mask = (1u << c) - 1, half = 1u << (c - 1);
            uint64_t two = limb <= NW - 1 ? ((uint64_t)raw[limb] | ((uint64_t)raw[limb + 1] << 32)) : 0;
            uint32_t v = ((uint32_t)(two >> sh) & mask) + carry;
            uint32_t neg = 0;
            carry = 0;
            if (v > half) { v = (1u << c) - v; neg = 1u << 31; carry = 1; }
            if (v) d[w] = (v - 1) | neg;
        }
    }
}
template <int THREADS>
__device__ __forceinline__ void part_block_scan(uint32_t *cnt, uint32_t len, uint32_t *wave_sums, uint32_t *total_out) {
    const uint32_t per = len / THREADS, t = threadIdx.x, base = t * per;
    uint32_t sum = 0;
    for (uint32_t i = 0; i < per; i++) sum += cnt[base + i];
    uint32_t incl = sum;
    for (int d = 1; d < 64; d <<= 1) { uint32_t v = __shfl_up(incl, d, 64); if ((int)(t & 63) >= d) incl += v; }
    if ((t & 63) == 63) wave_sums[t >> 6] = incl;
    __syncthreads();
    uint32_t run = incl - sum;
    for (uint32_t w = 0; w < (t >> 6); w++) run += wave_sums[w];
    for (uint32_t i = 0; i < per; i++) { const uint32_t c = cnt[base + i]; cnt[base + i] = run; run += c; }
    if (t == THREADS - 1) *total_out = run;
    __syncthreads();
}
template <class Fr>
__global__ void __launch_bounds__(PART_THREADS) k_part_hist(const Fr *__restrict__ s1, uint32_t n1, const Fr *__restrict__ s2, uint32_t n2, TableLayout L, uint32_t nbin,
                                                            uint32_t *__restrict__ canon, uint32_t *__restrict__ hist) {
    __shared__ uint32_t sh[PART_NBIN_MAX];
    for (uint32_t b = threadIdx.x; b < nbin; b += PART_THREADS) sh[b] = 0;
    __syncthreads();
    const uint32_t n = n1 + n2, ntiles = (n + PART_TILE - 1) / PART_TILE, per_wg = (ntiles + gridDim.x - 1) / gridDim.x;
    const uint32_t tile_lo = blockIdx.x * per_wg, tile_hi = tile_lo + per_wg < ntiles ? tile_lo + per_wg : ntiles;
    for (uint32_t tile = tile_lo; tile < tile_hi; tile++)
        for (int q = 0; q < PART_SPT; q++) {
            const uint32_t g = tile * PART_TILE + q * PART_THREADS + threadIdx.x;
            if (g >= n) continue;
            uint32_t d[PART_MAXW], raw[Fr::N + 1];
            (g < n1 ? s1[g] : s2[g - n1]).to_raw(raw);
            raw[Fr::N] = 0;
            part_digits<Fr::N>(raw, L, d);
#pragma unroll
            for (int w = 0; w < PART_MAXW; w++) if (d[w] != PART_NONE) atomicAdd(&sh[(d[w] & 0x7fffffffu) >> PART_FINE_BITS], 1u);
            static_assert(Fr::N == 8, "the canonical scalar is stored as two 16-byte words");
            uint4 *dst = reinterpret_cast<uint4 *>(canon + (size_t)g * Fr::N);
            dst[0] = make_uint4(raw[0], raw[1], raw[2], raw[3]); dst[1] = make_uint4(raw[4], raw[5], raw[6], raw[7]);
        }
    __syncthreads();
    for (uint32_t b = threadIdx.x; b < nbin; b += PART_THREADS) hist[(size_t)b * gridDim.x + blockIdx.x] = sh[b];
    if (blockIdx.x == 0 && threadIdx.x == 0) hist[(size_t)nbin * gridDim.x] = 0;
}
template <int NW>
__global__ void __launch_bounds__(PART_THREADS) k_part_scatter(const uint32_t *__restrict__ canon, uint32_t n, uint32_t n1, TableLayout L, uint32_t off1, uint32_t off2, uint32_t stride,
                                                               uint32_t nbin, const uint32_t *__restrict__ offs, uint32_t *__restrict__ out_val, uint16_t *__restrict__ out_key) {
    __shared__ uint32_t cursor[PART_NBIN_MAX], cnt[PART_NBIN_MAX], fill[PART_NBIN_MAX], st_val[PART_STAGE], st_key[PART_STAGE];
    __shared__ uint32_t wave_sums[PART_THREADS / 64], total;
    for (uint32_t b = threadIdx.x; b < nbin; b += PART_THREADS) cursor[b] = offs[(size_t)b * gridDim.x + blockIdx.x];
    const uint32_t ntiles = (n + PART_TILE - 1) / PART_TILE, per_wg = (ntiles + gridDim.x - 1) / gridDim.x;
    const uint32_t tile_lo = blockIdx.x * per_wg, tile_hi = tile_lo + per_wg < ntiles ? tile_lo + per_wg : ntiles;
    for (uint32_t tile = tile_lo; tile < tile_hi; tile++) {
        for (uint32_t b = threadIdx.x; b < PART_NBIN_MAX; b += PART_THREADS) { cnt[b] = 0; fill[b] = 0; }
        __syncthreads();
        uint32_t d[PART_SPT][PART_MAXW];
#pragma unroll
        for (int q = 0; q < PART_SPT; q++) {
            const uint32_t g = tile * PART_TILE + q * PART_THREADS + threadIdx.x;
            if (g < n) {
                uint32_t raw[NW + 1];
                const uint4 *src = reinterpret_cast<const uint4 *>(canon + (size_t)g * NW);
                const uint4 a = src[0], b = src[1];
                raw[0] = a.x; raw[1] = a.y; raw[2] = a.z; raw[3] = a.w; raw[4] = b.x; raw[5] = b.y; raw[6] = b.z; raw[7] = b.w; raw[NW] = 0;
                part_digits<NW>(raw, L, d[q]);
            } else {
#pragma unroll
                for (int w = 0; w < PART_MAXW; w++) d[q][w] = PART_NONE;
            }
#pragma unroll
            for (int w = 0; w < PART_MAXW; w++) if (d[q][w] != PART_NONE) atomicAdd(&cnt[(d[q][w] & 0x7fffffffu) >> PART_FINE_BITS], 1u);
        }
        __syncthreads();
        part_block_scan<PART_THREADS>(cnt, PART_NBIN_MAX, wave_sums, &total);
#pragma unroll
        for (int q = 0; q < PART_SPT; q++) {
            const uint32_t g = tile * PART_TILE + q * PART_THREADS + threadIdx.x;
            const uint32_t base = g < n1 ? off1 + g : off2 + (g - n1);
#pragma unroll
            for (int w = 0; w < PART_MAXW; w++) {
                if (d[q][w] == PART_NONE) continue;
                const uint32_t bucket = d[q][w] & 0x7fffffffu, bin = bucket >> PART_FINE_BITS;
                const uint32_t e = cnt[bin] + atomicAdd(&fill[bin], 1u);
                st_val[e] = ((uint32_t)w * stride + base) | (d[q][w] & 0x80000000u);
                st_key[e] = bucket | ((uint32_t)w << 20);
            }
        }
        __syncthreads();
        const uint32_t tot = total;
        for (uint32_t e = threadIdx.x; e < tot; e += PART_THREADS) {
            const uint32_t key = st_key[e], bucket = key & 0xfffffu, bin = bucket >> PART_FINE_BITS, dst = cursor[bin] + (e - cnt[bin]);
            out_val[dst] = st_val[e];
            out_key[dst] = (uint16_t)(((bucket & (PART_FINE - 1)) << PART_WBITS) | (key >> 20));
        }
        __syncthreads();
        for (uint32_t b = threadIdx.x; b < nbin; b += PART_THREADS) cursor[b] += fill[b];
        __syncthreads();
    }
}
constexpr uint32_t PART_FINE_STAGE = 30720;
__global__ void __launch_bounds__(PART_FINE_THREADS) k_part_fine(const uint32_t *__restrict__ offs, uint32_t grid_a, const uint32_t *__restrict__ in_val, const uint16_t *__restrict__ in_key,
                                                                 uint32_t *__restrict__ out_val, uint32_t *__restrict__ start, uint32_t *__restrict__ end) {
    __shared__ uint32_t cur[PART_KEYS], stage[PART_FINE_STAGE], wave_sums[PART_FINE_THREADS / 64], total, split_key;
    const uint32_t bin = blockIdx.x, t = threadIdx.x;
    const uint32_t lo = offs[(size_t)bin * grid_a], hi = offs[(size_t)(bin + 1) * grid_a];
    for (uint32_t f = t; f < PART_KEYS; f += PART_FINE_THREADS) cur[f] = 0;
    __syncthreads();
    for (uint32_t e0 = lo + t; e0 < hi; e0 += PART_FINE_THREADS * PART_FINE_UNROLL) {
        uint32_t key[PART_FINE_UNROLL];
#pragma unroll
        for (int u = 0; u < PART_FINE_UNROLL; u++) { const uint32_t e = e0 + u * PART_FINE_THREADS; key[u] = e < hi ? in_key[e] : PART_NONE; }
#pragma unroll
        for (int u = 0; u < PART_FINE_UNROLL; u++) if (key[u] != PART_NONE) atomicAdd(&cur[key[u]], 1u);
    }
    __syncthreads();
    part_block_scan<PART_FINE_THREADS>(cur, PART_KEYS, wave_sums, &total);
    for (uint32_t f = t; f < PART_FINE; f += PART_FINE_THREADS) {
        const uint32_t k = bin * PART_FINE + f;
        start[k] = lo + cur[f << PART_WBITS];
        end[k] = lo + (f + 1 < PART_FINE ? cur[(f + 1) << PART_WBITS] : total);
    }
    __syncthreads();
    const uint32_t tot = total;
    uint32_t k_lo = 0, base = 0;
    while (base < tot) {
        const uint32_t lim = base + PART_FINE_STAGE;
        if (tot <= lim) { if (t == 0) split_key = PART_KEYS; }
        else for (uint32_t f = k_lo + t; f < PART_KEYS; f += PART_FINE_THREADS) {
            const uint32_t e_f = f + 1 < PART_KEYS ? cur[f + 1] : tot;
            if (cur[f] <= lim && e_f > lim) split_key = f;
        }
        __syncthreads();
        uint32_t k_hi = split_key;
        const bool direct = k_hi == k_lo;
        if (direct) k_hi = k_lo + 1;
        const uint32_t stop = k_hi < PART_KEYS ? cur[k_hi] : tot;
        __syncthreads();
        for (uint32_t e0 = lo + t; e0 < hi; e0 += PART_FINE_THREADS * PART_FINE_UNROLL) {
            uint32_t key[PART_FINE_UNROLL], val[PART_FINE_UNROLL];
#pragma unroll
            for (int u = 0; u < PART_FINE_UNROLL; u++) {
                const uint32_t e = e0 + u * PART_FINE_THREADS;
                key[u] = PART_NONE;
                if (e < hi) { key[u] = in_key[e]; val[u] = in_val[e]; }
            }
#pragma unroll
            for (int u = 0; u < PART_FINE_UNROLL; u++) if (key[u] >= k_lo && key[u] < k_hi) {
                const uint32_t pos = atomicAdd(&cur[key[u]], 1u);
                if (direct) out_val[lo + pos] = val[u]; else stage[pos - base] = val[u];
            }
        }
        __syncthreads();
        if (!direct) for (uint32_t i = t; i < stop - base; i += PART_FINE_THREADS) out_val[lo + base + i] = stage[i];
        __syncthreads();
        base = stop; k_lo = k_hi;
    }
}
template <class Fr>
static void partition_buckets(MsmWorkspace &S, const Fr *scal1, size_t n1, size_t off1, const Fr *scal2, size_t n2, size_t off2, const TableLayout &L, size_t stride, uint32_t cap, hipStream_t s) {
    const int B = L.c_hi - 1;
    const uint32_t nbin = 1u << (B - PART_FINE_BITS), G = PART_GRID;
    const size_t n = n1 + n2, nb = (size_t)1 << B, nh = (size_t)nbin * G + 1;
    S.canon.grow(n * Fr::N);
    grow_together({nh, nh}, S.part_hist, S.part_offs);
#ifdef ZKAES_MEASURE
    for (int rep = (knockin() & 1) ? 0 : 1; rep < 2; rep++)
#endif
    {
    hipLaunchKernelGGL((k_part_hist<Fr>), dim3(G), dim3(PART_THREADS), 0, s, scal1, (uint32_t)n1, scal2, (uint32_t)n2, L, nbin, S.canon, S.part_hist);
    HIP_LAUNCH_CHECK();
    size_t tb = 0;
    HIP_CHECK(rocprim::exclusive_scan(nullptr, tb, S.part_hist.p, S.part_offs.p, 0u, nh, rocprim::plus<uint32_t>(), s));
    S.tmp.grow(tb);
    HIP_CHECK(rocprim::exclusive_scan(S.tmp.p, tb, S.part_hist.p, S.part_offs.p, 0u, nh, rocprim::plus<uint32_t>(), s));
    hipLaunchKernelGGL((k_part_scatter<Fr::N>), dim3(G), dim3(PART_THREADS), 0, s, (const uint32_t *)S.canon, (uint32_t)n, (uint32_t)n1, L, (uint32_t)off1, (uint32_t)off2, (uint32_t)stride, nbin,
                       (const uint32_t *)S.part_offs, S.vals_a, (uint16_t *)S.keys_a.p);
    HIP_LAUNCH_CHECK();
    hipLaunchKernelGGL(k_part_fine, dim3(nbin), dim3(PART_FINE_THREADS), 0, s, (const uint32_t *)S.part_offs, G, (const uint32_t *)S.vals_a, (const uint16_t *)S.keys_a.p, S.vals_b, S.start, S.end);
    HIP_LAUNCH_CHECK();
    }
    S.sorted_vals = S.vals_b; S.sorted_keys = nullptr;
    order_buckets(S, nb, cap, s);
}

template <class Curve>
void msm_prepare_table(MsmWorkspace *ws_, const typename Curve::Fr *scal1, size_t n1, size_t off1, const typename Curve::Fr *scal2, size_t n2, size_t off2, int c, size_t stride,
                       stream_t s_) {
    using Fr = typename Curve::Fr;
    hipStream_t s = (hipStream_t)s_;
    if (!ws_) throw GpuError("msm: null workspace");
    MsmWorkspace &S = *ws_;
    size_t n = n1 + n2;
    S.plan_n = n;
    if (n == 0) return;
    if (c < 4 || c > 24) throw GpuError("msm_table: window bits out of range");
    const TableLayout L = table_layout(Fr::BITS + 1, c);
    const int nwin = L.nwin;
    if (off1 + n1 > stride || off2 + n2 > stride) throw GpuError("msm_table: range exceeds the table");
    if ((uint64_t)nwin * stride >= (1ull << 30) || (uint64_t)n * nwin >= (1ull << 31)) throw GpuError("msm_table: index range too large");
    size_t pairs = n * (size_t)nwin;
    const size_t nb = (size_t)1 << (L.c_hi - 1);
    uint32_t cap = BUCKET_CAP_TABLE;
    while ((uint64_t)cap < 2 * (pairs / nb) + 64) cap <<= 1;
    S.plan_c = L.c_hi; S.plan_nwin = nwin; S.plan_pairs = pairs; S.plan_table = true; S.plan_cap = cap;
    ensure_scratch(S, pairs, nb, cap);
    const int B = L.c_hi - 1;
    if (B > PART_FINE_BITS && (1u << (B - PART_FINE_BITS)) <= PART_NBIN_MAX && nwin <= PART_MAXW && pairs >= ((size_t)1 << 16)) {
        partition_buckets<Fr>(S, scal1, n1, off1, scal2, n2, off2, L, stride, cap, s);
        return;
    }
    if (n1) { hipLaunchKernelGGL((k_digits_table<Fr>), dim3((unsigned)((n1 + 255) / 256)), dim3(256), 0, s, scal1, (uint32_t)n1, 0u, (uint32_t)n, (uint32_t)off1, L, (uint32_t)stride, S.keys_a, S.vals_a); HIP_LAUNCH_CHECK(); }
    if (n2) { hipLaunchKernelGGL((k_digits_table<Fr>), dim3((unsigned)((n2 + 255) / 256)), dim3(256), 0, s, scal2, (uint32_t)n2, (uint32_t)n1, (uint32_t)n, (uint32_t)off2, L, (uint32_t)stride, S.keys_a, S.vals_a); HIP_LAUNCH_CHECK(); }
    prepare_buckets<typename Curve::FqP>(S, pairs, L.c_hi - 1, 1, L.c_hi - 1, cap, s);
}
template <class Curve>
XYZZ<typename Curve::Fq> msm_table(MsmWorkspace *ws_, const Affine28<typename Curve::FqP> *tables, size_t stride, size_t off, int c, const typename Curve::Fr *scalars, size_t n, stream_t s_) {
    if (n == 0) return XYZZ<typename Curve::Fq>::inf();
    msm_prepare_table<Curve>(ws_, scalars, n, off, nullptr, 0, 0, c, stride, s_);
    return msm_finish<Curve>(ws_, tables, s_);
}
template <class Curve>
XYZZ<typename Curve::Fq> msm_table(MsmWorkspace *ws_, const Niels28<typename Curve::FqP> *tables, size_t stride, size_t off, int c, const typename Curve::Fr *scalars, size_t n, stream_t s_) {
    if (n == 0) return XYZZ<typename Curve::Fq>::inf();
    msm_prepare_table<Curve>(ws_, scalars, n, off, nullptr, 0, 0, c, stride, s_);
    return msm_finish<Curve>(ws_, tables, s_);
}

template <class Fr>
__global__ void k_power_scalars(Fr beta, uint64_t from, uint32_t count, Fr *__restrict__ out) {
    uint32_t i = blockIdx.x * blockDim.x + threadIdx.x;
    if (i >= count) return;
    out[i] = beta.pow_u64(from + i);
}
template <class Fq, class Fr>
__global__ void __launch_bounds__(64) k_fixed_base(const Affine<Fq> *__restrict__ table, const Fr *__restrict__ scalars, uint32_t count, Affine<Fq> *__restrict__ out) {
    uint32_t i = blockIdx.x * blockDim.x + threadIdx.x;
    if (i >= count) return;
    uint32_t raw[Fr::N];
    scalars[i].to_raw(raw);
    XYZZ<Fq> acc = XYZZ<Fq>::inf();
    for (int w = 0; w < Fr::N * 4; w++) {
        uint32_t d = (raw[w >> 2] >> ((w & 3) * 8)) & 0xff;
        if (d) acc.madd(table[w * 255 + d - 1]);
    }
    out[i] = acc.to_affine();
}

namespace {
template <class Curve>
DevPtr<Affine<typename Curve::Fq>> upload_fixed_base_table(const Affine<typename Curve::Fq> &base, hipStream_t s) {
    using Fq = typename Curve::Fq;
    const int NW = Curve::Fr::N * 4;
    std::vector<Affine<Fq>> table((size_t)NW * 255);
    XYZZ<Fq> wb = XYZZ<Fq>::from_affine(base);
    for (int w = 0; w < NW; w++) {
        XYZZ<Fq> acc = wb;
        for (int d = 1; d <= 255; d++) { table[(size_t)w * 255 + d - 1] = acc.to_affine(); acc.add(wb); }
        for (int k = 0; k < 8; k++) wb = wb.dbl();
    }
    DevPtr<Affine<Fq>> d_table(table.size());
    HIP_CHECK(hipMemcpyAsync(d_table, table.data(), table.size() * sizeof(Affine<Fq>), hipMemcpyHostToDevice, s));
    sync((stream_t)s);
    return d_table;
}
}

template <class Curve>
void fixed_base_powers(Affine<typename Curve::Fq> *out, const Affine<typename Curve::Fq> &base, const typename Curve::Fr &beta, size_t from, size_t count, stream_t s_) {
    using Fq = typename Curve::Fq;
    using Fr = typename Curve::Fr;
    hipStream_t s = (hipStream_t)s_;
    if (!count) return;
    DevPtr<Affine<Fq>> d_table = upload_fixed_base_table<Curve>(base, s);
    const size_t CH = 1 << 20;
    DevPtr<Fr> d_sc(CH);
    for (size_t off = 0; off < count; off += CH) {
        uint32_t m = (uint32_t)((count - off) < CH ? (count - off) : CH);
        hipLaunchKernelGGL((k_power_scalars<Fr>), dim3((m + 255) / 256), dim3(256), 0, s, beta, (uint64_t)(from + off), m, d_sc.get());
// ... 101 lines not shown
__global__ void __launch_bounds__(64) k_class_result(const A *__restrict__ in, uint32_t *__restrict__ flags, XYZZ<Fp<typename PtOps<A>::Params>> *__restrict__ out) {
    uint32_t i = threadIdx.x;
    if (i < 2) out[i] = PtOps<A>::to_std(in[i]);
    if (i == 2) { *reinterpret_cast<uint32_t *>(out + 2) = *flags; *flags = 0; }
}

template <class Curve, class Law>
static bool class_sum_impl(MsmWorkspace *ws_, const typename Law::Base *bases, const int8_t *vals, size_t n, XYZZ<typename Curve::Fq> *out, stream_t s_) {
    using A = typename Law::Acc;
    using Fq = typename Curve::Fq;
    hipStream_t s = (hipStream_t)s_;
    *out = XYZZ<Fq>::inf();
    if (n == 0) return true;
    if (!ws_) throw GpuError("class_sum: null workspace");
    MsmWorkspace &S = *ws_;
    uint32_t chunks = (uint32_t)((n + CLS_CHUNK - 1) / CLS_CHUNK), mid = (chunks + 255) / 256;
    size_t need_buckets = 2 * (size_t)chunks + 2 * mid + 8;
    ensure_scratch(S, 1, need_buckets, 0);
    A *p1 = (A *)S.buckets.p, *p2 = p1 + chunks, *m1 = p2 + chunks, *m2 = m1 + mid, *fin = m2 + mid;
    hipLaunchKernelGGL((k_class_partials<Law>), dim3((chunks + 63) / 64), dim3(64), 0, s, bases, vals, (uint32_t)n, p1, p2, S.ctrl + 3);
    HIP_LAUNCH_CHECK();
    (void)p2; (void)m2;
    if constexpr (Law::edwards) {
        hipLaunchKernelGGL((k_quad_sum<typename Law::Params>), dim3(mid, 2), dim3(RQ_THREADS), 0, s, (const A *)p1, chunks, 256u, m1, chunks, mid); HIP_LAUNCH_CHECK();
        hipLaunchKernelGGL((k_quad_sum<typename Law::Params>), dim3(1, 2), dim3(RQ_THREADS), 0, s, (const A *)m1, mid, mid, fin, mid, 1u); HIP_LAUNCH_CHECK();
    } else {
        hipLaunchKernelGGL((k_sum_tree<A>), dim3(mid, 2), dim3(256), 0, s, (const A *)p1, chunks, 256u, m1, chunks, mid); HIP_LAUNCH_CHECK();
        hipLaunchKernelGGL((k_sum_tree<A>), dim3(1, 2), dim3(256), 0, s, (const A *)m1, mid, mid, fin, mid, 1u); HIP_LAUNCH_CHECK();
    }
    hipLaunchKernelGGL((k_class_result<A>), dim3(1), dim3(64), 0, s, (const A *)fin, S.ctrl + 3, (XYZZ<Fq> *)S.h_res.dev); HIP_LAUNCH_CHECK();
    XYZZ<Fq> r[2];
    uint32_t flags = 0;
    sync((stream_t)s);
    memcpy(r, S.h_res.host, sizeof r);
    memcpy(&flags, (const char *)S.h_res.host + sizeof r, 4);
    if (flags) return false;
    oplog_msm(n, OP_MSM_CLASS_SUM);
    XYZZ<Fq> t = r[1].dbl();
    t.add(r[0]);
    *out = t;
    return true;
}
template <class Curve>
bool class_sum(MsmWorkspace *ws_, const Affine28<typename Curve::FqP> *bases, const int8_t *vals, size_t n, XYZZ<typename Curve::Fq> *out, stream_t s_) {
    return class_sum_impl<Curve, WeierLaw<typename Curve::FqP>>(ws_, bases, vals, n, out, s_);
}
template <class Curve>
bool class_sum(MsmWorkspace *ws_, const Niels28<typename Curve::FqP> *bases, const int8_t *vals, size_t n, XYZZ<typename Curve::Fq> *out, stream_t s_) {
    return class_sum_impl<Curve, EdwardsLaw<typename Curve::FqP>>(ws_, bases, vals, n, out, s_);
}
template XYZZ<Fq377> msm_finish<Bls377>(MsmWorkspace *, const Niels28<Fq377P> *, stream_t);
template void msm_finish2<Bls377>(MsmWorkspace *, const Niels28<Fq377P> *, const Niels28<Fq377P> *, XYZZ<Fq377> *, stream_t);
template XYZZ<Fq377> msm<Bls377>(MsmWorkspace *, const Niels28<Fq377P> *, const Fr377 *, size_t, stream_t);
template XYZZ<Fq377> msm_table<Bls377>(MsmWorkspace *, const Niels28<Fq377P> *, size_t, size_t, int, const Fr377 *, size_t, stream_t);
template bool class_sum<Bls377>(MsmWorkspace *, const Niels28<Fq377P> *, const int8_t *, size_t, XYZZ<Fq377> *, stream_t);

template void msm_table_sum_device<Bls377>(MsmWorkspace *, const Niels28<Fq377P> *, size_t, size_t, int, const Fr377 *, size_t, XYZZ<Fq377> *, stream_t);
template XYZZ<Fq377> msm_fold_points_device<Bls377>(const XYZZ<Fq377> *, int, stream_t);
template XYZZ<Fq381> msm_fold_points_device<Bls381>(const XYZZ<Fq381> *, int, stream_t);
template void msm_sharded_plan<Bls377>(size_t, int *, int *);
template void msm_sharded_plan<Bls381>(size_t, int *, int *);
template void msm_window_sums_device<Bls377>(MsmWorkspace *, const Affine28<Fq377P> *, const Fr377 *, size_t, size_t, XYZZ<Fq377> *, stream_t);
template void msm_window_sums_device<Bls381>(MsmWorkspace *, const Affine28<Fq381P> *, const Fr381 *, size_t, size_t, XYZZ<Fq381> *, stream_t);
template XYZZ<Fq377> msm_fold_window_sums_device<Bls377>(const XYZZ<Fq377> *, int, size_t, stream_t);
template XYZZ<Fq381> msm_fold_window_sums_device<Bls381>(const XYZZ<Fq381> *, int, size_t, stream_t);
template void msm_prepare_table<Bls377>(MsmWorkspace *, const Fr377 *, size_t, size_t, const Fr377 *, size_t, size_t, int, size_t, stream_t);
template void msm_prepare_table<Bls381>(MsmWorkspace *, const Fr381 *, size_t, size_t, const Fr381 *, size_t, size_t, int, size_t, stream_t);
template XYZZ<Fq377> msm_table<Bls377>(MsmWorkspace *, const Affine28<Fq377P> *, size_t, size_t, int, const Fr377 *, size_t, stream_t);
template XYZZ<Fq381> msm_table<Bls381>(MsmWorkspace *, const Affine28<Fq381P> *, size_t, size_t, int, const Fr381 *, size_t, stream_t);
template void convert_bases<Bls377>(Affine28<Fq377P> *, const Affine<Fq377> *, size_t, stream_t);
template void convert_bases<Bls381>(Affine28<Fq381P> *, const Affine<Fq381> *, size_t, stream_t);
template void build_window_tables<Bls377>(Affine<Fq377> *, size_t, int, stream_t);
template void table_next<Bls377>(Affine<Fq377> *, const Affine<Fq377> *, size_t, int, int, stream_t);
template void table_next<Bls381>(Affine<Fq381> *, const Affine<Fq381> *, size_t, int, int, stream_t);
template void build_window_tables<Bls381>(Affine<Fq381> *, size_t, int, stream_t);
template int table_windows<Bls377>(int);
template int table_windows<Bls381>(int);
template void msm_prepare<Bls377>(MsmWorkspace *, const Fr377 *, size_t, const Fr377 *, size_t, size_t, stream_t, int);
template void msm_prepare<Bls381>(MsmWorkspace *, const Fr381 *, size_t, const Fr381 *, size_t, size_t, stream_t, int);
template XYZZ<Fq377> msm_finish<Bls377>(MsmWorkspace *, const Affine28<Fq377P> *, stream_t);
template XYZZ<Fq381> msm_finish<Bls381>(MsmWorkspace *, const Affine28<Fq381P> *, stream_t);
template XYZZ<Fq377> msm<Bls377>(MsmWorkspace *, const Affine28<Fq377P> *, const Fr377 *, size_t, stream_t);
template XYZZ<Fq381> msm<Bls381>(MsmWorkspace *, const Affine28<Fq381P> *, const Fr381 *, size_t, stream_t);
template void fixed_base_scalars<Bls377>(Affine<Fq377> *, const Affine<Fq377> &, const Fr377 *, size_t, stream_t);
template bool class_sum<Bls377>(MsmWorkspace *, const Affine28<Fq377P> *, const int8_t *, size_t, XYZZ<Fq377> *, stream_t);
template void fixed_base_powers<Bls377>(Affine<Fq377> *, const Affine<Fq377> &, const Fr377 &, size_t, size_t, stream_t);
template void fixed_base_powers<Bls381>(Affine<Fq381> *, const Affine<Fq381> &, const Fr381 &, size_t, size_t, stream_t);

}
}
```

aes_zero_knowledge_proof_circuit_amd/csrc/marlin.cpp:

```cpp
#include "marlin.hpp"
#include "../../include/zkaes.h"
#include <algorithm>
#include <cstdio>
#include <chrono>
#include <cstdlib>
#include <cstring>
#include <atomic>
#include <map>
#include <mutex>
#include <future>
#include <deque>
#include <condition_variable>
#include <thread>
#include <functional>
#include <stdexcept>
#include <cerrno>
#include <sys/random.h>
#include "gpu.hpp"
#include "trace_layout.h"
#include "transcript.hpp"
#include "marlin_host.hpp"

namespace zk {
namespace {
// ... 221 lines not shown
    int table_c = 20;
    bool use_tables = false;
    std::atomic<size_t> n_contexts{0};
    double setup_srs_s = 0, setup_total_s = 0;
    DevPtr<uint32_t> d_desc, d_sbox_in, d_sbox_tmpl;
    DevPtr<uint32_t> d_a_rowptr, d_a_col, d_b_rowptr, d_b_col;
    DevPtr<int64_t> d_a_coeff, d_b_coeff;
    DevPtr<uint32_t> d_t_colptr, d_t_seg_start, d_t_seg_end, d_t_row; DevPtr<uint8_t> d_t_mat; DevPtr<int64_t> d_t_coeff;
    uint32_t t_nseg = 0, t_nheavy = 0;
    DevPtr<uint32_t> d_t_heavy;
    DevPtr<uint32_t> d_ix_ci, d_ix_ri;
    DevPtr<F> ix_ev[6], ix_co[6], ix_cs[6];
    Fr coset_g, coset_g_inv, coset_vk_inv;
    DevPtr<void> coset_tab, coset_tab_inv;
    ProverTimings last_timings;

    std::mutex ctx_mu;
    std::vector<std::unique_ptr<ProverContext>> ctxs;

    ProverContext &context(size_t i) {
        gpu::set_device(device);
        std::lock_guard<std::mutex> g(ctx_mu);
        while (ctxs.size() <= i) {
            std::unique_ptr<ProverContext> c(new ProverContext());
            alloc_workspace(*c);
            ctxs.push_back(std::move(c));
        }
        return *ctxs[i];
    }
    void alloc_workspace(ProverContext &cx) {
        const Circuit &c = circuit;
        size_t n4 = next_pow2(3 * n + 1);
        cx.d_trace.alloc(c.trace_bytes + 64); cx.d_z.alloc(c.num_variables() + 64);
        cx.d_msg.alloc(std::max<size_t>(message_len, 16)); cx.d_key.alloc(c.key_bytes); cx.d_iv.alloc(std::max<size_t>(16, 12 + c.aad_bytes));
        for (auto &p : cx.d_cls) p.alloc(n + 64);
        { size_t ncand = (size_t)(3.0 * n / 0.58 * 1.02) + 8192; cx.d_rng.alloc((ncand * 8 / 16 + 2) * 64 + ncand * 8 + (4u << 20)); }
        cx.za_ev.alloc(n); cx.zb_ev.alloc(n); cx.x_poly.alloc(m); cx.x_tmp.alloc(m); cx.x_evals.alloc(n); cx.tmp_n.alloc(n + 1); cx.ra_ev.alloc(n); cx.ra_poly.alloc(n);
        cx.zpoly.alloc(n + 1); cx.t_partial.alloc(t_nseg + 1);
        size_t caps[9] = {n + 1, n + 1, n + 1, 3 * n, n, n, 3 * n, k, k + 1};
        for (int i = 0; i < 9; i++) cx.poly[i].alloc(caps[i]);
        size_t big = std::max(n4, k);
        for (auto &b : cx.e) b.alloc(big);
        cx.f_poly.alloc(k);
        cx.acc.alloc(std::max(3 * n, k) + 1); cx.wit.alloc(std::max(3 * n, k) + 1); cx.wit2.alloc(std::max(n, k) + 1); cx.scratch.alloc(std::max(8 + 3 * gpu::poly_eval_scratch(n + 1) + gpu::poly_eval_scratch(k), gpu::divide_by_linear_scratch(std::max(3 * n, k) + 1)));
    }

    template <class T> static DevPtr<T> upload(const std::vector<T> &v, gpu::stream_t s) {
        DevPtr<T> d(v.size());
        gpu::h2d(d, v.data(), v.size() * sizeof(T), s);
        return d;
    }

    bool table_ok(const ProverContext &, size_t len) const { return use_tables && len >= table_min_n; }
    using Lane = ProverContext::Lane;
    XYZZ<Fq377> msm_powers(ProverContext &cx, Lane &ln, bool shifted, size_t off, const F *scalars, size_t len) {
        if (len == 0) return XYZZ<Fq377>::inf();
        size_t avail = shifted ? (bounds[1] + 1) : (supported_degree + 1);
        if (off + len > avail) throw std::runtime_error("KZG10: polynomial degree exceeds the committer key");
        if (table_ok(cx, len)) return gpu::msm_table<Bls377>(ln.ws, d_powers, srs_stride, (shifted ? lowest_shift : 0) + off, table_c, scalars, len, ln.stream);
        return gpu::msm<Bls377>(ln.ws, (shifted ? d_shifted : d_powers) + off, scalars, len, ln.stream);
    }
    struct Labeled { int idx; long bound; bool hiding; KzgRand rand, shifted_rand; Commitment comm; };
    static void draw_rand(Labeled &lp, ChaChaRng &zk) {
        auto draw = [&](KzgRand &r) { r.hiding = lp.hiding; for (auto &x : r.b) x = Fr::zero(); if (lp.hiding) for (int i = 0; i < 3; i++) r.b[i] = zk.rand_field<Fr>(); };
        draw(lp.rand);
        if (lp.bound >= 0) draw(lp.shifted_rand);
    }
    void hide(XYZZ<Fq377> &c, const KzgRand &rnd) const { if (rnd.hiding) for (int i = 0; i < 3; i++) c.add(srs->gamma_tab[i].mul(rnd.b[i])); }
    bool lagrange_commit(ProverContext &cx, Lane &ln, int which, const std::vector<uint8_t> &inst, const Fr &rho, const KzgRand &rnd, G1A &out) {
        XYZZ<Fq377> c;
        if (!gpu::class_sum<Bls377>(ln.ws, which == 0 ? lag->d_lag_w : lag->d_lag_h, cx.d_cls[which], n, &c, ln.stream)) return false;
        if (which == 0) for (size_t j = 0; j < m; j++) if (inst[j]) c.madd(lag->lag_pj[j].neg());
        c.add((which == 0 ? lag->lag_vw_tab : lag->lag_vh_tab).mul(rho));
        hide(c, rnd);
        out = c.to_affine();
        return true;
    }
    void mpc_commit(ProverContext &cx, Lane &ln, Labeled &lp) {
        const F *coeffs = cx.poly[lp.idx].p;
        size_t len = cx.poly_len[lp.idx];
        lp.comm.has_shifted = false;
        const bool bounded = lp.bound >= 0;
        const size_t off = bounded ? (max_degree - (size_t)lp.bound) - lowest_shift : 0;
        if (len > supported_degree + 1 || (bounded && off + len > bounds[1] + 1)) throw std::runtime_error("KZG10: polynomial degree exceeds the committer key");
        if (len) {
            if (table_ok(cx, len)) gpu::msm_prepare_table<Bls377>(ln.ws, coeffs, len, 0, nullptr, 0, 0, table_c, srs_stride, ln.stream);
            else gpu::msm_prepare<Bls377>(ln.ws, coeffs, len, nullptr, 0, 0, ln.stream);
        }
        XYZZ<Fq377> c12[2] = {XYZZ<Fq377>::inf(), XYZZ<Fq377>::inf()}, h12[2] = {XYZZ<Fq377>::inf(), XYZZ<Fq377>::inf()};
        hide(h12[0], lp.rand);
        if (bounded) hide(h12[1], lp.shifted_rand);
        if (len) {
            if (bounded) gpu::msm_finish2<Bls377>(ln.ws, d_powers, d_shifted + off, c12, ln.stream);
            else c12[0] = gpu::msm_finish<Bls377>(ln.ws, d_powers, ln.stream);
        }
        c12[0].add(h12[0]);
        lp.comm.comm = c12[0].to_affine();
        if (bounded) { c12[1].add(h12[1]); lp.comm.shifted = c12[1].to_affine(); lp.comm.has_shifted = true; }
    }
    void msm_opening_prepare(ProverContext &cx, Lane &ln, const F *wit, size_t wlen, const F *swit, size_t slen, size_t shift_off) {
        if (wlen > supported_degree + 1 || shift_off + slen > bounds[1] + 1) throw std::runtime_error("KZG10: polynomial degree exceeds the committer key");
        if (table_ok(cx, wlen + slen)) gpu::msm_prepare_table<Bls377>(ln.ws, wit, wlen, 0, swit, slen, lowest_shift + shift_off, table_c, srs_stride, ln.stream);
        else gpu::msm_prepare<Bls377>(ln.ws, wit, wlen, swit, slen, lowest_shift + shift_off, ln.stream);
    }
    XYZZ<Fq377> msm_opening_finish(Lane &ln) { return gpu::msm_finish<Bls377>(ln.ws, d_powers, ln.stream); }
    bool use_lanes = true;
    struct RoundJobs {
        ProvingKeyImpl &K; ProverContext &cx;
        const bool async;
        struct Slot { std::string err; std::function<void(Lane &)> fn; std::promise<void> done; std::future<void> fut; bool queued = false; };
        std::vector<std::unique_ptr<Slot>> slots;
        RoundJobs(ProvingKeyImpl &k, ProverContext &c) : K(k), cx(c), async(!c.throughput && k.use_lanes) { if (async) cx.ensure_lanes(); }
        void start(int lane_i, std::function<void(Lane &)> fn, bool gate) {
            std::unique_ptr<Slot> sl(new Slot());
            sl->fn = std::move(fn);
            Slot *p = sl.get();
            slots.push_back(std::move(sl));
            if (!async) return;
            if (lane_i < 1 || lane_i >= ProverContext::N_LANES) throw std::logic_error("RoundJobs: bad lane");
            Lane &ln = cx.lane[lane_i];
            if (gate) { gpu::event_record(ln.ready, cx.stream); gpu::stream_wait_event(ln.stream, ln.ready); }
            const int dev = K.device;
            p->fut = p->done.get_future(); p->queued = true;
            ln.worker->submit([p, &ln, dev] {
                try { gpu::set_device(dev); p->fn(ln); } catch (const std::exception &e) { p->err = e.what(); if (p->err.empty()) p->err = "error"; } catch (...) { p->err = "error"; }
                p->done.set_value();
            });
        }
        void join() {
            std::string first;
            for (auto &sl : slots) {
                if (async) { if (sl->queued) { sl->fut.wait(); sl->queued = false; } }
                else { try { sl->fn(cx.lane[0]); } catch (const std::exception &e) { sl->err = e.what(); if (sl->err.empty()) sl->err = "error"; } }
                if (first.empty() && !sl->err.empty()) first = sl->err;
            }
            slots.clear();
            if (!first.empty()) throw std::runtime_error(first);
        }
        void wait_all() noexcept { for (auto &sl : slots) if (sl->queued) sl->fut.wait(); }
        ~RoundJobs() { wait_all(); }
    };

    struct ProofRun {
        ProverContext &cx;
        const uint8_t *host_trace, *msg; size_t len; const uint8_t *key, *iv;
        Clock::time_point t_all, t0;
        ChaChaRng zk;
        FiatShamirRng fs;
        Labeled r1[4], r2[3], r3[2];
        Fr rhos[3];
        std::vector<uint8_t> inst;
        bool declined[3] = {false, false, false};
        Fr alpha, eta_a, eta_b, eta_c, vh_alpha, beta, vh_beta, ea_vv, eb_vv, ec_vv, alpha_beta, gamma;
        Proof pf;
        bool early_evals = false;
        std::atomic<bool> g2_quotient_queued{false};
        RoundJobs jobs;
        ProofRun(ProvingKeyImpl &K, ProverContext &c, const uint8_t *trace, const uint8_t *msg_, size_t len_, const uint8_t *key_, const uint8_t *iv_, const uint8_t *zk_seed)
// ... 327 lines not shown
    { Bytes o; for (auto &lp : R.r3) o.commitment_tobytes(lp.comm); R.fs.absorb(o.b); }
    R.gamma = R.fs.rng().rand_field<Fr>();
    cx.timings.round3_ms = ms_since(R.t0); R.t0 = Clock::now();
}

void ProvingKeyImpl::prove_open(ProofRun &R) {
    ProverContext &cx = R.cx;
    gpu::stream_t s = cx.stream;
    if (R.early_evals) {
        const F *ps[1] = {cx.poly[7].p};
        const size_t ls[1] = {cx.poly_len[7]};
        gpu::poly_eval_multi(ps, ls, &R.gamma, 1, &R.pf.evals[1], cx.scratch.p, cx.scratch.n, s);
    } else {
        const F *ps[4] = {cx.poly[5].p, cx.poly[7].p, cx.poly[4].p, cx.poly[2].p};
        const size_t ls[4] = {cx.poly_len[5], cx.poly_len[7], cx.poly_len[4], cx.poly_len[2]};
        const Fr at[4] = {R.beta, R.gamma, R.beta, R.beta};
        gpu::poly_eval_multi(ps, ls, at, 4, R.pf.evals, cx.scratch.p, cx.scratch.n, s);
    }
    const Fr g2_g = R.pf.evals[1], t_b = R.pf.evals[2], zb_b = R.pf.evals[3];
    { Bytes o; for (auto &v : R.pf.evals) o.field(v); R.fs.absorb(o.b); }
    Fr ch;
    { uint64_t lo = R.fs.rng().next_u64(), hi = R.fs.rng().next_u64(); uint32_t raw[8] = {(uint32_t)lo, (uint32_t)(lo >> 32), (uint32_t)hi, (uint32_t)(hi >> 32), 0, 0, 0, 0}; ch = Fr::from_raw(raw); }
    Fr r_alpha_at_beta = (R.vh_alpha - R.vh_beta) * (R.alpha - R.beta).inverse();
    Fr vx_beta = eval_vanishing(m, R.beta);
    Fr c_za = r_alpha_at_beta * (R.eta_a + R.eta_c * zb_b), c_w = (t_b * vx_beta).neg(), c_h1 = R.vh_beta.neg();
    Fr vk_gamma = eval_vanishing(k, R.gamma);
    Fr bmul = R.gamma * g2_g + t_b * Fr::from_u64(k).inverse();
    Fr c_row = R.alpha * bmul, c_col = R.beta * bmul, c_rc = bmul.neg(), c_h2 = vk_gamma.neg();
    Fr chp[5]; chp[0] = Fr::one(); for (int i = 1; i < 5; i++) chp[i] = chp[i - 1] * ch;
    auto rand_axpy = [](Fr out[3], const Fr &sc, const KzgRand &r) { if (r.hiding) for (int i = 0; i < 3; i++) out[i] = out[i] + sc * r.b[i]; };
    auto host_divide_by_linear = [](Fr q[2], const Fr p[3], const Fr &z) { q[1] = p[2]; q[0] = p[1] + z * p[2]; };
    auto host_eval3 = [](const Fr p[3], const Fr &z) { return p[0] + z * (p[1] + z * p[2]); };
    if (R.jobs.async && !cx.ev_aux) {
        cx.acc_b.alloc(cx.acc.n); cx.wit_b.alloc(cx.wit.n); cx.wit2_b.alloc(cx.wit2.n); cx.scratch_b.alloc(cx.scratch.n);
        cx.scratch_c.alloc(gpu::divide_by_linear_scratch(std::max(n, k) + 1)); cx.ev_aux = gpu::EventGuard();
    }
    const bool two_sets = cx.ev_aux != nullptr && R.jobs.async;
    if (R.jobs.async) gpu::sync(s);
    struct WaitJobs { RoundJobs &j; ~WaitJobs() { j.wait_all(); } } wait_jobs{R.jobs};
    R.jobs.start(1, [&](Lane &ln) {
        gpu::stream_t ls_ = ln.stream;
        size_t plen = 3 * n;
        Fr rb[3] = {Fr::zero(), Fr::zero(), Fr::zero()};
        {
            const F *ps[7] = {cx.poly[5].p, cx.poly[3].p, cx.poly[1].p, cx.poly[0].p, cx.poly[6].p, cx.poly[4].p, cx.poly[2].p};
            size_t ls[7] = {cx.poly_len[5], cx.poly_len[3], cx.poly_len[1], cx.poly_len[0], cx.poly_len[6], cx.poly_len[4], cx.poly_len[2]};
            Fr sc[7] = {chp[0], chp[2], chp[2] * c_za, chp[2] * c_w, chp[2] * c_h1, chp[3], chp[4]};
            gpu::poly_lincomb_n(cx.acc.p, plen, ps, ls, sc, 7, ls_);
        }
        rand_axpy(rb, chp[0], R.r2[1].rand); rand_axpy(rb, chp[2] * c_za, R.r1[1].rand); rand_axpy(rb, chp[2] * c_w, R.r1[0].rand); rand_axpy(rb, chp[4], R.r1[2].rand);
        if (!R.early_evals) gpu::divide_by_linear(cx.wit2.p, cx.poly[5].p, cx.poly_len[5], R.beta, cx.scratch.p, cx.scratch.n, ls_);
        gpu::divide_by_linear(cx.wit.p, cx.acc.p, plen, R.beta, cx.scratch.p, cx.scratch.n, ls_);
        gpu::poly_scale(cx.wit2.p, chp[1], cx.poly_len[5] - 1, ls_);
        msm_opening_prepare(cx, ln, cx.wit.p, plen - 1, cx.wit2.p, cx.poly_len[5] - 1, bounds[1] - (n - 2));
        XYZZ<Fq377> hw = XYZZ<Fq377>::inf();
        Fr rq[2]; host_divide_by_linear(rq, rb, R.beta);
        for (int i = 0; i < 2; i++) hw.add(srs->gamma_tab[i].mul(rq[i]));
        Fr rv = host_eval3(rb, R.beta);
        Fr srb[3]; for (int i = 0; i < 3; i++) srb[i] = chp[1] * R.r2[1].shifted_rand.b[i];
        host_divide_by_linear(rq, srb, R.beta);
        for (int i = 0; i < 2; i++) hw.add(srs->gamma_tab[i].mul(rq[i]));
        rv = rv + host_eval3(srb, R.beta);
        XYZZ<Fq377> w = msm_opening_finish(ln);
        w.add(hw);
        R.pf.w_beta = w.to_affine(); R.pf.random_v_beta = rv;
    }, false);
    R.jobs.start(2, [&](Lane &ln) {
        gpu::stream_t ls_ = ln.stream;
        DevPtr<F> &acc_ = two_sets ? cx.acc_b : cx.acc, &wit_ = two_sets ? cx.wit_b : cx.wit, &wit2_ = two_sets ? cx.wit2_b : cx.wit2, &scr_ = two_sets ? cx.scratch_b : cx.scratch;
        size_t plen = k;
        {
            const F *ps[8] = {cx.poly[7].p, ix_co[2].p, ix_co[3].p, ix_co[4].p, ix_co[0].p, ix_co[1].p, ix_co[5].p, cx.poly[8].p};
            size_t ls[8] = {cx.poly_len[7], k, k, k, k, k, k, cx.poly_len[8]};
            Fr sc[8] = {chp[0], chp[2] * R.ea_vv, chp[2] * R.eb_vv, chp[2] * R.ec_vv, chp[2] * c_row, chp[2] * c_col, chp[2] * c_rc, chp[2] * c_h2};
            gpu::poly_lincomb_n(acc_.p, plen, ps, ls, sc, 8, ls_);
        }
        gpu::divide_by_linear(wit_.p, acc_.p, plen, R.gamma, scr_.p, scr_.n, ls_);
        if (R.jobs.async) {
            while (!R.g2_quotient_queued.load(std::memory_order_acquire)) std::this_thread::yield();
            gpu::stream_wait_event(ls_, cx.ev_aux);
        } else {
            gpu::divide_by_linear(wit2_.p, cx.poly[7].p, cx.poly_len[7], R.gamma, scr_.p, scr_.n, ls_);
            gpu::poly_scale(wit2_.p, chp[1], cx.poly_len[7] - 1, ls_);
        }
        msm_opening_prepare(cx, ln, wit_.p, plen - 1, wit2_.p, cx.poly_len[7] - 1, bounds[1] - (k - 2));
        XYZZ<Fq377> w = msm_opening_finish(ln);
        R.pf.w_gamma = w.to_affine();
    }, false);
    if (R.jobs.async) {
        try {
            gpu::divide_by_linear(cx.wit2_b.p, cx.poly[7].p, cx.poly_len[7], R.gamma, cx.scratch_c.p, cx.scratch_c.n, s);
            gpu::poly_scale(cx.wit2_b.p, chp[1], cx.poly_len[7] - 1, s);
            gpu::event_record(cx.ev_aux, s);
        } catch (...) { R.g2_quotient_queued.store(true, std::memory_order_release); throw; }
        R.g2_quotient_queued.store(true, std::memory_order_release);
    }
    R.jobs.join();
}

Proof ProvingKeyImpl::prove(ProverContext &cx, const uint8_t *host_trace, const uint8_t *msg, size_t len, const uint8_t *key, const uint8_t *zk_seed, bool throughput, const uint8_t *iv) {
    gpu::set_device(device);
    std::lock_guard<std::mutex> busy(cx.in_use);
    cx.throughput = throughput;
    ProofRun R(*this, cx, host_trace, msg, len, key, iv, zk_seed);
    prove_round1(R);
    prove_round2(R);
    prove_round3(R);
    prove_open(R);
    for (int i = 0; i < 4; i++) R.pf.comms[i] = R.r1[i].comm;
    for (int i = 0; i < 3; i++) R.pf.comms[4 + i] = R.r2[i].comm;
    for (int i = 0; i < 2; i++) R.pf.comms[7 + i] = R.r3[i].comm;
    cx.timings.open_ms = ms_since(R.t0);
    cx.timings.total_ms = ms_since(R.t_all);
    { std::lock_guard<std::mutex> g(ctx_mu); last_timings = cx.timings; }
    return R.pf;
}

ProvingKey::~ProvingKey() { if (impl) { DeviceScope on(impl->device); delete impl; } }
const VerifyingKey &ProvingKey::vk() const { return impl->vk; }
const Circuit &ProvingKey::circuit() const { return impl->circuit; }
const ProverTimings &ProvingKey::last_timings() const { return impl->last_timings; }
bool ProvingKey::tables_built(uint64_t *bytes) const {
    if (bytes) *bytes = impl->use_tables ? impl->srs->bytes() : 0;
    return impl->use_tables;
}
void ProvingKey::srs_info(uint64_t out[6], double secs[2]) const {
    const UniversalSrs &U = *impl->srs;
    out[0] = U.max_degree; out[1] = U.stride; out[2] = U.n_tab; out[3] = U.bytes();
    out[4] = (uint64_t)impl->srs.use_count();
    out[5] = impl->lag ? 2 * (uint64_t)impl->lag->n * sizeof(SrsPoint) : 0;
    if (secs) { secs[0] = impl->setup_srs_s; secs[1] = impl->setup_total_s; }
}
size_t ProvingKey::contexts() const { size_t v = impl->n_contexts.load(); return v ? v : default_contexts(); }
void ProvingKey::set_contexts(size_t n) {
    if (n > 64) throw std::invalid_argument("set_contexts: at most 64 prover contexts per key");
    impl->n_contexts.store(n);
}
void ProvingKey::msm_powers_partial_device(const uint8_t *scalars, size_t n_local, size_t offset, void *dev_out) {
    gpu::set_device(impl->device);
// ... 321 lines not shown
```

aes_zero_knowledge_proof_circuit_amd/csrc/te28.cuh:

```cuda
#pragma once
#include "ec28.cuh"

namespace zk {

template <class P>
struct alignas(64) Niels28 { FpMsm<P> ymx, ypx, td; uint32_t pad[6]; };
template <class P>
struct AccTE { FpMsm<P> x, y, z, t; };

struct Te377 {
    using P = Fq377P;
    using G = Fp28<P>;
    using F = Fp<P>;
    ZK_HD static G lit28(const uint32_t (&t)[14]) { G r; for (int i = 0; i < 14; i++) r.l[i] = t[i]; return r; }
    ZK_HD static F lit(const uint32_t (&t)[12]) { F r; for (int i = 0; i < 12; i++) r.l[i] = t[i]; return r; }
    ZK_HD static F s_std() { constexpr uint32_t t[12] = FQ377_TE_S_INIT; return lit(t); }
    ZK_HD static F f_std() { constexpr uint32_t t[12] = FQ377_TE_F_INIT; return lit(t); }
    ZK_HD static F k2d_std() { constexpr uint32_t t[12] = FQ377_TE_K2D_INIT; return lit(t); }
    ZK_HD static G k2d() { constexpr uint32_t t[14] = FQ377_TE_K2D_28_INIT; return lit28(t); }
    ZK_HD static G si() { constexpr uint32_t t[14] = FQ377_TE_SI_28_INIT; return lit28(t); }
    ZK_HD static G sif() { constexpr uint32_t t[14] = FQ377_TE_SIF_28_INIT; return lit28(t); }
};

template <class P>
ZK_HD AccTE<P> te_identity() { AccTE<P> r; r.x = FpMsm<P>::zero(); r.t = r.x; r.y = FpMsm<P>::k_one(); r.z = r.y; return r; }
template <class P>
ZK_HD Niels28<P> niels_identity() { Niels28<P> r; r.ymx = FpMsm<P>::k_one(); r.ypx = r.ymx; r.td = FpMsm<P>::zero(); return r; }
template <class P>
ZK_HD Niels28<P> niels_neg(const Niels28<P> &n) { Niels28<P> r; r.ymx = n.ypx; r.ypx = n.ymx; r.td = FpMsm<P>::zero().template sub<2>(n.td); return r; }

template <class P>
ZK_HD void te_madd(AccTE<P> &a, const Niels28<P> &n) {
    using G = FpMsm<P>;
    G A = a.y.template sub_lazy<3>(a.x) * n.ymx;
    G B = a.y.add_lazy(a.x) * n.ypx;
    G C = a.t * n.td;
    G D = a.z.dbl_lazy();
    G E = B.template sub<2>(A), H = B.add_lazy(A);
    G F = D.template sub_lazy<2>(C), Gg = D + C;
    a.x = E * F; a.y = Gg * H; a.t = E * H; a.z = F * Gg;
}
template <class P>
ZK_HD Niels28<P> niels_load_signed(const Niels28<P> *rec, bool neg) {
    const FpMsm<P> *f = &rec->ymx;
    Niels28<P> r;
    r.ymx = f[neg ? 1 : 0]; r.ypx = f[neg ? 0 : 1]; r.td = rec->td;
    return r;
}
template <class P>
ZK_HD void te_madd_hot(AccTE<P> &a, Niels28<P> &n, bool neg, const Niels28<P> *next, bool next_neg, uint64_t bias) {
    using G = FpMsm<P>;
    G A = G::mul_biased(a.y.template sub_lazy<3>(a.x), n.ymx, bias);
    G B = G::mul_biased(a.y.add_lazy(a.x), n.ypx, bias);
    G C = G::mul_biased(a.t, n.td, bias);
#if defined(__HIP_DEVICE_COMPILE__)
    asm volatile("" : "+v"(A.l[G::N - 1]), "+v"(B.l[G::N - 1]), "+v"(C.l[G::N - 1]) : : "memory");
#endif
    n = niels_load_signed<P>(next, next_neg);
#if defined(__HIP_DEVICE_COMPILE__)
    asm volatile("" : "+v"(A.l[0]), "+v"(C.l[0]) : : "memory");
#endif
    G E = B.template sub_lazy<2>(A), H = B.add_lazy(A);
    G D = a.z.dbl_lazy();
    G U = D.template sub_lazy<2>(C), V = D.add_lazy(C), F, Gg;
#pragma unroll
    for (int i = 0; i < G::N; i++) { F.l[i] = neg ? V.l[i] : U.l[i]; Gg.l[i] = neg ? U.l[i] : V.l[i]; }
    a.x = G::mul_biased(E, F, bias); a.y = G::mul_biased(Gg, H, bias); a.t = G::mul_biased(E, H, bias); a.z = G::mul_biased(F, Gg, bias);
}
template <class P>
ZK_HD void te_add_inline(AccTE<P> &a, const AccTE<P> &b) {
    using G = FpMsm<P>;
    G A = a.y.template sub<3>(a.x) * b.y.template sub<3>(b.x);
    G B = (a.y + a.x) * (b.y + b.x);
    G C = (a.t * b.t) * Te377::k2d();
    G D = (a.z * b.z).dbl();
    G E = B.template sub<2>(A), H = B + A;
    G F = D.template sub<2>(C), Gg = D + C;
    a.x = E * F; a.y = Gg * H; a.t = E * H; a.z = F * Gg;
}
template <class P>
ZK_EC_FN void te_add(AccTE<P> &a, const AccTE<P> &b) { te_add_inline<P>(a, b); }
template <class P>
ZK_EC_FN void te_dbl(AccTE<P> &a) {
    using G = FpMsm<P>;
    G A = a.x.sqr(), B = a.y.sqr(), C = a.z.sqr().dbl();
    G S = (a.x + a.y).sqr(), AB = A + B;
    G E = S.template sub<3>(AB);
    G Gg = B.template sub<2>(A);
    G F = Gg.template sub<3>(C);
    G H = G::zero().template sub<3>(AB);
    a.x = E * F; a.y = Gg * H; a.t = E * H; a.z = F * Gg;
}
template <class P>
ZK_HD AccTE<P> te_neg(const AccTE<P> &a) {
    AccTE<P> r = a;
    if (!a.x.limbs_zero()) r.x = FpMsm<P>::zero().template sub<2>(a.x);
    if (!a.t.limbs_zero()) r.t = FpMsm<P>::zero().template sub<2>(a.t);
    return r;
}

template <class P>
ZK_HD XYZZ<Fp<P>> te_to_std_point(const AccTE<P> &a) {
    using G = FpMsm<P>;
    G zmy = a.z.template sub<3>(a.y), zpy = a.z + a.y;
    G xz = a.x * zmy;
    G zz = xz.sqr();
    if (zz.is_zero_mod_p()) return XYZZ<Fp<P>>::inf();
    G numx = (Te377::si() * zpy).template sub<6>(zmy);
    XYZZ<Fp<P>> o;
    o.x = ((numx * a.x) * xz).to_std();
    o.y = (((Te377::sif() * a.z) * zpy) * zz).to_std();
    o.zz = zz.to_std();
    o.zzz = (zz * xz).to_std();
    return o;
}

struct TeMapParts { Fp<Fq377P> u, v, den; };
ZK_HD TeMapParts te_map_parts(const Affine<Fp<Fq377P>> &p) {
    using F = Fp<Fq377P>;
    TeMapParts m;
// ... 95 lines not shown
```

include/zkaes.h:

```cpp
#ifndef ZKAES_H
#define ZKAES_H
#include <stddef.h>
#include <stdint.h>
#ifdef __cplusplus
extern "C" {
#endif

typedef struct zkaes_pk zkaes_pk;
typedef struct zkaes_vk zkaes_vk;

const char *zkaes_last_error(void);
void zkaes_bytes_free(uint8_t *p);
void zkaes_pk_free(zkaes_pk *pk);
void zkaes_vk_free(zkaes_vk *vk);
int zkaes_device_count(void);
int zkaes_set_device(int ordinal);

int zkaes_synthesize_keys(size_t plaintext_length, zkaes_pk **pk, zkaes_vk **vk);
int zkaes_encrypt(const uint8_t *message, size_t message_len, const uint8_t secret_key[16], const zkaes_pk *pk, uint8_t **proof, size_t *proof_len);
int zkaes_verify_encryption(const zkaes_vk *vk, const uint8_t *proof, size_t proof_len, const uint8_t *ciphertext, size_t ciphertext_len, int *accepted);
int zkaes_proof_roundtrip(const uint8_t *proof, size_t proof_len, uint8_t **out, size_t *out_len);

#define ZKAES_CIRCUIT_AES 0
#define ZKAES_CIRCUIT_OPS_XOR 1
// ... 77 lines not shown
                         const uint8_t tag16[16], uint8_t *message, int *ok);
int zkaes_prove_ops(const zkaes_pk *pk, uint32_t x, uint32_t y, const uint8_t *zk_seed32, uint8_t **proof, size_t *proof_len);
int zkaes_verify(const zkaes_vk *vk, const uint8_t *proof, size_t proof_len, const uint8_t *public_input_bits, size_t n_bits, int *accepted);
int zkaes_vk_serialize(const zkaes_vk *vk, uint8_t **out, size_t *out_len);
int zkaes_vk_deserialize(const uint8_t *bytes, size_t len, zkaes_vk **vk);
int zkaes_vk_serialize_ark(const zkaes_vk *vk, uint8_t **out, size_t *out_len);
int zkaes_vk_deserialize_ark(const uint8_t *bytes, size_t len, zkaes_vk **vk);
int zkaes_vk_serialize_ark_uncompressed(const zkaes_vk *vk, uint8_t **out, size_t *out_len);

int zkaes_vk_from_trapdoor(const uint64_t info[7], const uint8_t *index_comms, const uint8_t *beta, zkaes_vk **vk);

int zkaes_pk_info(const zkaes_pk *pk, uint64_t out[12]);
int zkaes_circuit_info(int circuit_kind, size_t plaintext_length, uint64_t out[12]);
int zkaes_circuit_matrix(int circuit_kind, size_t plaintext_length, int which, uint64_t *n_rows, uint64_t *nnz, uint32_t *rowptr, uint32_t *col, int64_t *coeff);
int zkaes_pk_debug_fetch(const zkaes_pk *pk, const char *name, uint8_t **out, size_t *len);
int zkaes_pk_timings(const zkaes_pk *pk, double out[6]);
int zkaes_msm_stats(double out[5], int reset);
int zkaes_pk_op_lists(const zkaes_pk *pk, const uint8_t *message, size_t message_len, const uint8_t secret_key[16], int throughput_path, uint8_t **json, size_t *json_len);
int zkaes_mem_info(uint64_t *free_bytes, uint64_t *total_bytes);

int zkaes_ntt(int field_id, uint8_t *data, size_t n, int inverse);
int zkaes_ntt_coset(int field_id, uint8_t *data, size_t n, int inverse, int coset_c, int lg_big);
int zkaes_ntt_batch(int field_id, uint8_t *data, size_t n, int count, int inverse, const int *coset_c, int lg_big);
int zkaes_poly_divide_by_vanishing(const uint8_t *p, size_t len, size_t m, int with_scratch, uint8_t *q, uint8_t *rem_or_null);
int zkaes_poly_divide_by_linear(const uint8_t *p, size_t len, const uint8_t z[32], uint8_t *q);
int zkaes_poly_eval_multi(const uint8_t *const *polys, const size_t *lens, const uint8_t *x, int count, uint8_t *out);
int zkaes_batch_inverse(uint8_t *v, size_t n, const uint8_t *post_or_null, int throughput_variant);
int zkaes_poly_lincomb(const uint8_t *const *polys, const size_t *lens, const uint8_t *scalars, int count, size_t n, uint8_t *out);
int zkaes_vanishing_quotient_evals(int lg_n, const uint8_t *g, int ncosets, const uint8_t a[32], const uint32_t *idx_or_null, size_t nidx, uint8_t *out);
int zkaes_q1_coset_pointwise(const uint8_t *r, const uint8_t *za, const uint8_t *zb, const uint8_t *t, const uint8_t *z, const uint8_t consts[192], size_t n, uint8_t *out);
int zkaes_h2_coset(const uint8_t *const arrays[7], const uint8_t consts[224], size_t k, uint8_t *out);
int zkaes_q1_combine(const uint8_t *q0, const uint8_t *q1, const uint8_t *q3, const uint8_t *mask, const uint8_t inv2[32], const uint8_t inv2zeta[32], size_t n, uint8_t *h1, uint8_t *g1);
int zkaes_coset_scale(const uint8_t *in, size_t in_len, const uint8_t g[32], size_t n, uint8_t *out);
int zkaes_z_poly_from_w(const uint8_t *w, size_t wlen, const uint8_t *x_poly, uint32_t m, size_t n, uint8_t *zp);
int zkaes_ntt_padded(int field_id, const uint8_t *in, size_t in_len, size_t n, int inverse, int coset_c, int lg_big, uint8_t *out);
int zkaes_ntt_scaled(const uint8_t g[32], const uint8_t *in, size_t in_len, size_t n, int inverse, uint8_t *out);
int zkaes_arith_probe(int op, const uint32_t *in, size_t n_cases, uint32_t *out);

int zkaes_msm(int curve_id, const uint8_t *bases, const uint8_t *scalars, size_t n, uint8_t *out_xy, int *out_inf);
int zkaes_g1_sum(int curve_id, const uint8_t *points_xy, const int *inf, size_t n, uint8_t *out_xy, int *out_inf);
int zkaes_msm_sharded_plan(int curve_id, size_t n_total, int *window_bits, int *n_windows, size_t *bytes_per_rank);
int zkaes_msm_window_sums_dev(int curve_id, const uint8_t *bases, const uint8_t *scalars, size_t n_local, size_t n_total, void *dev_out, size_t dev_out_bytes);
int zkaes_msm_fold_window_sums_dev(int curve_id, const void *dev_in, int world, size_t n_total, uint8_t *out_xy, int *out_inf);
int zkaes_pk_msm_partial_dev(const zkaes_pk *pk, const uint8_t *scalars, size_t n_local, size_t offset, void *dev_out, size_t dev_out_bytes);
int zkaes_msm_fold_partials_dev(int curve_id, const void *dev_in, int world, uint8_t *out_xy, int *out_inf);
int zkaes_pk_serialize_ark_to_file(const zkaes_pk *pk, const char *path, uint64_t *bytes_written);
int zkaes_pk_serialize_ark_to_file_ex(const zkaes_pk *pk, const char *path, int uncompressed, uint64_t *bytes_written);
int zkaes_pk_tables_built(const zkaes_pk *pk, int *built, uint64_t *table_bytes);
int zkaes_pk_srs_info(const zkaes_pk *pk, uint64_t out[6], double secs[2]);
int zkaes_set_default_contexts(size_t n);
int zkaes_srs_hold(int hold);
int zkaes_msm_table(int curve_id, const uint8_t *bases, const uint8_t *scalars, size_t n, int window_bits, uint8_t *out_xy, int *out_inf);
int zkaes_msm_table_srs(const uint8_t *bases, const uint8_t *scalars, size_t n, int window_bits, uint8_t *out_xy, int *out_inf);
int zkaes_msm_bench(int curve_id, const uint8_t *bases, const uint8_t *scalars, size_t n, int reps, double *ms_total, double *ms_accumulate);
int zkaes_msm_bench_synth(size_t n, int window_bits, int reps, double *ms_total, double *ms_accumulate, uint8_t *out_xy);
int zkaes_stream_copy_bench(size_t bytes, int reps, double *gb_per_s);
int zkaes_int_rate_bench(double seconds, double out[8]);
int zkaes_aes_witness(const zkaes_pk *pk, const uint8_t *message, size_t message_len, const uint8_t secret_key[16], uint8_t *z, size_t z_cap, size_t *z_len);

#ifdef __cplusplus
}
#endif
#endif
```

Baseline: 95.71.

## Decompose Montgomery-form scalars directly in table MSM and seed bucket accumulators from Niels

```diff
diff --git a/aes_zero_knowledge_proof_circuit_amd/api.py b/aes_zero_knowledge_proof_circuit_amd/api.py
--- a/aes_zero_knowledge_proof_circuit_amd/api.py
+++ b/aes_zero_knowledge_proof_circuit_amd/api.py
@@ -703,8 +703,11 @@
 ARITH_QUAD_OPS = ("te377.te_add_quad", "te377.te_dbl_quad")
 
 
+ARITH_EXT_OPS = {"te377.te_seed_from_niels": (256, 43, 56), "te377.te_seed_hot": (257, 86, 98)}
+
+
 def arith_probe(op_name, cases):
-    op, nin, nout = ARITH_OPS[op_name]
+    op, nin, nout = ARITH_OPS[op_name] if op_name in ARITH_OPS else ARITH_EXT_OPS[op_name]
     cases = bytes(cases)
     n, rest = divmod(len(cases), 4 * nin)
     if rest:
@@ -757,14 +760,19 @@
     return out.raw, bool(inf.value)
 
 
-def msm_table(curve_id, bases_bytes, scalars_bytes, window_bits, srs=False):
+def msm_table(curve_id, bases_bytes, scalars_bytes, window_bits, srs=False, mont_digits=False):
+    if mont_digits and not srs:
+        raise ValueError("mont_digits is a mode of the SRS (twisted Edwards) table path")
     n = len(scalars_bytes) // 32
     out = C.create_string_buffer(96)
     inf = C.c_int()
     if srs:
         if int(curve_id) != 377:
             raise ValueError("the SRS (twisted Edwards) table path exists for BLS12-377 only")
-        _check(lib().zkaes_msm_table_srs(bytes(bases_bytes), bytes(scalars_bytes), C.c_size_t(n), int(window_bits), out, C.byref(inf)))
+        if mont_digits:
+            _check(lib().zkaes_msm_table_srs_flags(bytes(bases_bytes), bytes(scalars_bytes), C.c_size_t(n), int(window_bits), C.c_uint(1), out, C.byref(inf)))
+        else:
+            _check(lib().zkaes_msm_table_srs(bytes(bases_bytes), bytes(scalars_bytes), C.c_size_t(n), int(window_bits), out, C.byref(inf)))
     else:
         _check(lib().zkaes_msm_table(int(curve_id), bytes(bases_bytes), bytes(scalars_bytes), C.c_size_t(n), int(window_bits), out, C.byref(inf)))
     return out.raw, bool(inf.value)
diff --git a/aes_zero_knowledge_proof_circuit_amd/csrc/arith_probe.cuh b/aes_zero_knowledge_proof_circuit_amd/csrc/arith_probe.cuh
--- a/aes_zero_knowledge_proof_circuit_amd/csrc/arith_probe.cuh
+++ b/aes_zero_knowledge_proof_circuit_amd/csrc/arith_probe.cuh
@@ -108,6 +108,15 @@
         te_madd_hot<P>(a, n, in[PTW + 2 * NIW] != 0, &next, in[PTW + 2 * NIW + 1] != 0, bias);
         st_te<P>(out, a); st_niels<P>(out + PTW, n);
     } };
+struct TeSeed : OpBase { using P = Fq377P; static constexpr int NIN = NIW + 1, NOUT = PTW;
+    ZK_HD static void run(const uint32_t *in, uint32_t *out, uint64_t) { st_te<P>(out, te_seed_from_niels<P>(ld_niels<P>(in), in[NIW] != 0)); } };
+struct TeSeedHot : OpBase { using P = Fq377P; static constexpr int NIN = 2 * NIW + 2, NOUT = PTW + NIW;
+    ZK_HD static void run(const uint32_t *in, uint32_t *out, uint64_t) {
+        Niels28<P> n = ld_niels<P>(in);
+        const Niels28<P> next = ld_niels<P>(in + NIW);
+        const AccTE<P> a = te_seed_hot<P>(n, in[2 * NIW] != 0, &next, in[2 * NIW + 1] != 0);
+        st_te<P>(out, a); st_niels<P>(out + PTW, n);
+    } };
 template <class P> struct Madd28 : OpBase { static constexpr int NIN = PTW + 2 * GW, NOUT = PTW + 1;
     ZK_HD static void run(const uint32_t *in, uint32_t *out, uint64_t) {
         Acc28<P> a = ld_acc<P>(in);
@@ -156,11 +165,19 @@
     X(192, TeMadd) X(193, TeAdd) X(194, TeDbl) X(195, TeNeg) X(196, TeToStd) X(197, NielsFromW) X(198, TeMaddHot) X(199, TeAddQuad) X(200, TeDblQuad) \
     ZK_PROBE_W28(X, 208, Fq377P) ZK_PROBE_W28(X, 216, Fq381P)
 
+#define ZK_PROBE_EXT_OPS(X) X(256, TeSeed) X(257, TeSeedHot)
+
 template <class O> struct Tag { using type = O; };
 template <class Fn> bool dispatch(int op, Fn &&fn) {
     switch (op) {
 #define ZK_PROBE_CASE(ID, ...) case ID: fn(Tag<__VA_ARGS__>{}); return true;
         ZK_PROBE_OPS(ZK_PROBE_CASE)
+        default: return false;
+    }
+}
+template <class Fn> bool dispatch_ext(int op, Fn &&fn) {
+    switch (op) {
+        ZK_PROBE_EXT_OPS(ZK_PROBE_CASE)
 #undef ZK_PROBE_CASE
         default: return false;
     }
diff --git a/aes_zero_knowledge_proof_circuit_amd/csrc/capi_kernels.hip b/aes_zero_knowledge_proof_circuit_amd/csrc/capi_kernels.hip
--- a/aes_zero_knowledge_proof_circuit_amd/csrc/capi_kernels.hip
+++ b/aes_zero_knowledge_proof_circuit_amd/csrc/capi_kernels.hip
@@ -134,7 +134,7 @@
     }
     give_affine(r.to_affine(), out_xy, out_inf);
 }
-template <class Curve, bool EDWARDS> void run_msm_table(const uint8_t *bases, const uint8_t *scalars, size_t n, int c, uint8_t *out_xy, int *out_inf) {
+template <class Curve, bool EDWARDS> void run_msm_table(const uint8_t *bases, const uint8_t *scalars, size_t n, int c, uint8_t *out_xy, int *out_inf, bool mont_digits = false) {
     using Fq = typename Curve::Fq; using Fr = typename Curve::Fr;
     if (c < 2 || c > 22) throw std::invalid_argument("window bits must be in [2, 22]");
     if (n && (!bases || !scalars)) throw std::invalid_argument("zkaes_msm_table: null argument");
@@ -151,7 +151,7 @@
     if constexpr (EDWARDS) {
         DevPtr<zk::Niels28<typename Curve::FqP>> tabte(nt * n);
         zk::gpu::convert_bases_te<Curve>(tabte, tab, nt * n, s);
-        a = zk::gpu::msm_table<Curve>(ws, tabte, n, 0, c, ds, n, s).to_affine();
+        a = zk::gpu::msm_table<Curve>(ws, tabte, n, 0, c, ds, n, s, mont_digits).to_affine();
     } else {
         DevPtr<zk::Affine28<typename Curve::FqP>> tab28(nt * n);
         zk::gpu::convert_bases<Curve>(tab28, tab, nt * n, s);
@@ -259,6 +259,12 @@
 }
 int zkaes_msm_table_srs(const uint8_t *bases, const uint8_t *scalars, size_t n, int window_bits, uint8_t *out_xy, int *out_inf) {
     return guardk([&] { run_msm_table<zk::Bls377, true>(bases, scalars, n, window_bits, out_xy, out_inf); });
+}
+int zkaes_msm_table_srs_flags(const uint8_t *bases, const uint8_t *scalars, size_t n, int window_bits, unsigned flags, uint8_t *out_xy, int *out_inf) {
+    return guardk([&] {
+        if (flags & ~(unsigned)ZKAES_MSM_MONT_DIGITS) throw std::invalid_argument("zkaes_msm_table_srs_flags: unknown flag");
+        run_msm_table<zk::Bls377, true>(bases, scalars, n, window_bits, out_xy, out_inf, (flags & ZKAES_MSM_MONT_DIGITS) != 0);
+    });
 }
 int zkaes_set_device(int ordinal) { return guardk([&] { HIP_CHECK(hipSetDevice(ordinal)); }); }
 int zkaes_ntt(int field_id, uint8_t *data, size_t n, int inverse) {
diff --git a/aes_zero_knowledge_proof_circuit_amd/csrc/capi_probe.hip b/aes_zero_knowledge_proof_circuit_amd/csrc/capi_probe.hip
--- a/aes_zero_knowledge_proof_circuit_amd/csrc/capi_probe.hip
+++ b/aes_zero_knowledge_proof_circuit_amd/csrc/capi_probe.hip
@@ -45,7 +45,8 @@
         zk::capi_set_error("");
         if (!in || !out) throw std::invalid_argument("zkaes_arith_probe: null argument");
         if (n_cases == 0 || n_cases > zk::probe::MAX_CASES) throw std::invalid_argument("zkaes_arith_probe: n_cases must be in [1, 65536]");
-        if (!zk::probe::dispatch(op, [&](auto tag) { run_probe<typename decltype(tag)::type>(in, n_cases, out); })) throw std::invalid_argument("zkaes_arith_probe: unknown op " + std::to_string(op));
+        auto run = [&](auto tag) { run_probe<typename decltype(tag)::type>(in, n_cases, out); };
+        if (!zk::probe::dispatch(op, run) && !zk::probe::dispatch_ext(op, run)) throw std::invalid_argument("zkaes_arith_probe: unknown op " + std::to_string(op));
         return 0;
     } catch (const std::exception &e) { zk::capi_set_error(e.what()); return 1; }
     catch (...) { zk::capi_set_error("unknown error"); return 1; }
diff --git a/aes_zero_knowledge_proof_circuit_amd/csrc/consts32.h b/aes_zero_knowledge_proof_circuit_amd/csrc/consts32.h
--- a/aes_zero_knowledge_proof_circuit_amd/csrc/consts32.h
+++ b/aes_zero_knowledge_proof_circuit_amd/csrc/consts32.h
@@ -8,6 +8,7 @@
 static const uint32_t FR377_ONE[8] = {0xfffffff3u, 0x7d1c7fffu, 0x6ffffff2u, 0x7257f50fu, 0x512c0feeu, 0x16d81575u, 0x2bbb9a9du, 0x0d4bda32u};
 static const uint32_t FR377_R2[8] = {0xb861857bu, 0x25d577bau, 0x8860591fu, 0xcc2c27b5u, 0xe5dc8593u, 0xa7cc008fu, 0xeff1c939u, 0x011fdae7u};
 static const uint32_t FR377_INV = 0xffffffffu;
+static const uint32_t FR377_RINV[8] = {0x1beeec02u, 0x4122dd1au, 0x74fee875u, 0xbd1eae95u, 0x27b28e2fu, 0x838557e2u, 0x2290c02cu, 0x07b30191u};
 #define FR381_BITS 255
 #define FR381_P_INIT {0x00000001u, 0xffffffffu, 0xfffe5bfeu, 0x53bda402u, 0x09a1d805u, 0x3339d808u, 0x299d7d48u, 0x73eda753u}
 #define FR381_ONE_INIT {0xfffffffeu, 0x00000001u, 0x00034802u, 0x5884b7fau, 0xecbc4ff5u, 0x998c4fefu, 0xacc5056fu, 0x1824b159u}
@@ -16,6 +17,7 @@
 static const uint32_t FR381_ONE[8] = {0xfffffffeu, 0x00000001u, 0x00034802u, 0x5884b7fau, 0xecbc4ff5u, 0x998c4fefu, 0xacc5056fu, 0x1824b159u};
 static const uint32_t FR381_R2[8] = {0xf3f29c6du, 0xc999e990u, 0x87925c23u, 0x2b6cedcbu, 0x7254398fu, 0x05d31496u, 0x9f59ff11u, 0x0748d9d9u};
 static const uint32_t FR381_INV = 0xffffffffu;
+static const uint32_t FR381_RINV[8] = {0xfe75c040u, 0x13f75b69u, 0x09dc705fu, 0xab6fca8fu, 0x4f77266au, 0x7204078au, 0x30009d57u, 0x1bbe8693u};
 #define FQ377_BITS 377
 #define FQ377_P_INIT {0x00000001u, 0x8508c000u, 0x30000000u, 0x170b5d44u, 0xba094800u, 0x1ef3622fu, 0x00f5138fu, 0x1a22d9f3u, 0x6ca1493bu, 0xc63b05c0u, 0x17c510eau, 0x01ae3a46u}
 #define FQ377_ONE_INIT {0xffffff68u, 0x02cdffffu, 0x7fffffb1u, 0x51409f83u, 0x8a7d3ff2u, 0x9f7db3a9u, 0x6e7c6305u, 0x7b4e97b7u, 0x803c84e8u, 0x4cf495bfu, 0xe2fdf49au, 0x008d6661u}
@@ -67,4 +69,5 @@
 #define FQ377_TE_K2D_28_INIT {0x706c521u, 0xdf4444au, 0x8fa7e68u, 0x371b2aau, 0xdd6cd3du, 0xebe579eu, 0x3577a6au, 0x1d3f1c6u, 0x2ada318u, 0x2a73d9du, 0x7da6ef5u, 0xce09495u, 0xfed4ab8u, 0x0001813u}
 #define FQ377_TE_SI_28_INIT {0x4e1e338u, 0x09d0889u, 0x5a9d7bdu, 0x00869f5u, 0xcb9f841u, 0xfcb79bcu, 0x14fcb3bu, 0xd78b460u, 0x9add89fu, 0x66e4a72u, 0xcdeb434u, 0x3157be7u, 0x5ed67e0u, 0x000140eu}
 #define FQ377_TE_SIF_28_INIT {0xcfd10d5u, 0x9457a38u, 0x383e475u, 0x7e96cb8u, 0x388e8d9u, 0xd00b5abu, 0xd32ebe1u, 0x0c15e03u, 0x5ac3c51u, 0xa270ad8u, 0xe68d2ebu, 0xbe54908u, 0x8029609u, 0x00001c4u}
+#define FQ377_TE_DI_28_INIT {0xc7448d7u, 0xd9fdddau, 0x72e84acu, 0x7593d2au, 0x51c3a60u, 0xc66f1aeu, 0x9769153u, 0xd87e5d4u, 0x5ca9538u, 0x7670b3cu, 0x49cf899u, 0xca3cb94u, 0xb5300dbu, 0x0001a5eu}
 static const uint8_t ARK_TEST_RNG_SEED[32] = {1,0,0,0, 23,0,0,0, 200,1,0,0, 210,30,0,0, 0,0,0,0, 0,0,0,0, 0,0,0,0, 0,0,0,0};
diff --git a/aes_zero_knowledge_proof_circuit_amd/csrc/ff28.cuh b/aes_zero_knowledge_proof_circuit_amd/csrc/ff28.cuh
--- a/aes_zero_knowledge_proof_circuit_amd/csrc/ff28.cuh
+++ b/aes_zero_knowledge_proof_circuit_amd/csrc/ff28.cuh
@@ -200,10 +200,11 @@
         return r;
     }
 
-    ZK_HD Fp28 canonical() const {
+    ZK_HD Fp28 canonical() const { return canonical_below<5>(); }
+    template <int LOG> ZK_HD Fp28 canonical_below() const {
         Fp28 v = *this;
 #pragma unroll
-        for (int k = 5; k >= 0; k--) {
+        for (int k = LOG; k >= 0; k--) {
             int64_t c = 0;
             uint32_t tl[N];
 #pragma unroll
diff --git a/aes_zero_knowledge_proof_circuit_amd/csrc/gpu.hpp b/aes_zero_knowledge_proof_circuit_amd/csrc/gpu.hpp
--- a/aes_zero_knowledge_proof_circuit_amd/csrc/gpu.hpp
+++ b/aes_zero_knowledge_proof_circuit_amd/csrc/gpu.hpp
@@ -122,7 +122,8 @@
 template <class Curve>
 void msm_finish2(MsmWorkspace *ws, const Niels28<typename Curve::FqP> *bases, const Niels28<typename Curve::FqP> *bases2, XYZZ<typename Curve::Fq> *out, stream_t s);
 template <class Curve>
-XYZZ<typename Curve::Fq> msm_table(MsmWorkspace *ws, const Niels28<typename Curve::FqP> *tables, size_t stride, size_t off, int c, const typename Curve::Fr *scalars, size_t n, stream_t s);
+XYZZ<typename Curve::Fq> msm_table(MsmWorkspace *ws, const Niels28<typename Curve::FqP> *tables, size_t stride, size_t off, int c, const typename Curve::Fr *scalars, size_t n, stream_t s,
+                                   bool mont_digits = false);
 template <class Curve>
 bool class_sum(MsmWorkspace *ws, const Niels28<typename Curve::FqP> *bases, const int8_t *vals, size_t n, XYZZ<typename Curve::Fq> *out, stream_t s);
 template <class Curve> void msm_sharded_plan(size_t n_total, int *window_bits, int *n_windows);
@@ -140,7 +141,9 @@
 template <class Curve> void build_window_tables(Affine<typename Curve::Fq> *tables, size_t stride, int c, stream_t s);
 template <class Curve> void table_next(Affine<typename Curve::Fq> *next, const Affine<typename Curve::Fq> *prev, size_t count, int c, int j, stream_t s);
 template <class Curve>
-void msm_prepare_table(MsmWorkspace *ws, const typename Curve::Fr *scal1, size_t n1, size_t off1, const typename Curve::Fr *scal2, size_t n2, size_t off2, int c, size_t stride, stream_t s);
+void msm_prepare_table(MsmWorkspace *ws, const typename Curve::Fr *scal1, size_t n1, size_t off1, const typename Curve::Fr *scal2, size_t n2, size_t off2, int c, size_t stride, stream_t s,
+                       bool mont_digits = false);
+template <class Curve> XYZZ<typename Curve::Fq> msm_unmont(const XYZZ<typename Curve::Fq> &p);
 template <class Curve>
 XYZZ<typename Curve::Fq> msm_table(MsmWorkspace *ws, const Affine28<typename Curve::FqP> *tables, size_t stride, size_t off, int c, const typename Curve::Fr *scalars, size_t n, stream_t s);
 template <class Curve>
diff --git a/aes_zero_knowledge_proof_circuit_amd/csrc/kernels_msm.hip b/aes_zero_knowledge_proof_circuit_amd/csrc/kernels_msm.hip
--- a/aes_zero_knowledge_proof_circuit_amd/csrc/kernels_msm.hip
+++ b/aes_zero_knowledge_proof_circuit_amd/csrc/kernels_msm.hip
@@ -60,13 +60,14 @@
     L.n_hi = rem ? rem : L.nwin;
     return L;
 }
-template <class Fr>
+template <class Fr, bool MONT>
 __global__ void k_digits_table(const Fr *__restrict__ scalars, uint32_t n, uint32_t i_off, uint32_t ntot, uint32_t val_off, TableLayout L, uint32_t stride,
                                uint32_t *__restrict__ keys, uint32_t *__restrict__ vals) {
     uint32_t i = blockIdx.x * blockDim.x + threadIdx.x;
     if (i >= n) return;
     uint32_t raw[Fr::N + 1];
-    scalars[i].to_raw(raw);
+    if constexpr (MONT) { const Fr v = scalars[i]; for (int j = 0; j < Fr::N; j++) raw[j] = v.l[j]; }
+    else scalars[i].to_raw(raw);
     raw[Fr::N] = 0;
     uint32_t carry = 0;
     for (int w = 0; w < L.nwin; w++) {
@@ -245,9 +246,13 @@
     if (e - s > cap) e = s + cap;
     if constexpr (Law::edwards) {
         AccTE<P> acc = te_identity<P>();
+        uint32_t idx = VAL_SKIP;
+        while (s < e && ((idx = vals[s]) & VAL_SKIP)) s++;
         if (s < e) {
-            uint32_t idx = vals[s];
             Niels28<P> p = niels_load_signed<P>(bases + (idx & VAL_INDEX), idx >> 31);
+            const bool seed_neg = idx >> 31;
+            if (++s < e) idx = vals[s];
+            acc = te_seed_hot<P>(p, seed_neg, bases + (idx & VAL_INDEX), idx >> 31);
             for (uint32_t i = s; i < e; i++) {
                 const uint32_t cur = idx;
                 if (i + 1 < e) idx = vals[i + 1];
@@ -1120,7 +1125,7 @@
     if (t == THREADS - 1) *total_out = run;
     __syncthreads();
 }
-template <class Fr>
+template <class Fr, bool MONT>
 __global__ void __launch_bounds__(PART_THREADS) k_part_hist(const Fr *__restrict__ s1, uint32_t n1, const Fr *__restrict__ s2, uint32_t n2, TableLayout L, uint32_t nbin,
                                                             uint32_t *__restrict__ canon, uint32_t *__restrict__ hist) {
     __shared__ uint32_t sh[PART_NBIN_MAX];
@@ -1133,21 +1138,27 @@
             const uint32_t g = tile * PART_TILE + q * PART_THREADS + threadIdx.x;
             if (g >= n) continue;
             uint32_t d[PART_MAXW], raw[Fr::N + 1];
-            (g < n1 ? s1[g] : s2[g - n1]).to_raw(raw);
+            static_assert(Fr::N == 8, "a scalar is read and stored as two 16-byte words");
+            if constexpr (MONT) {
+                const uint4 *src = reinterpret_cast<const uint4 *>(g < n1 ? s1 + g : s2 + (g - n1));
+                const uint4 a = src[0], b = src[1];
+                raw[0] = a.x; raw[1] = a.y; raw[2] = a.z; raw[3] = a.w; raw[4] = b.x; raw[5] = b.y; raw[6] = b.z; raw[7] = b.w;
+            } else (g < n1 ? s1[g] : s2[g - n1]).to_raw(raw);
             raw[Fr::N] = 0;
             part_digits<Fr::N>(raw, L, d);
 #pragma unroll
             for (int w = 0; w < PART_MAXW; w++) if (d[w] != PART_NONE) atomicAdd(&sh[(d[w] & 0x7fffffffu) >> PART_FINE_BITS], 1u);
-            static_assert(Fr::N == 8, "the canonical scalar is stored as two 16-byte words");
-            uint4 *dst = reinterpret_cast<uint4 *>(canon + (size_t)g * Fr::N);
-            dst[0] = make_uint4(raw[0], raw[1], raw[2], raw[3]); dst[1] = make_uint4(raw[4], raw[5], raw[6], raw[7]);
+            if constexpr (!MONT) {
+                uint4 *dst = reinterpret_cast<uint4 *>(canon + (size_t)g * Fr::N);
+                dst[0] = make_uint4(raw[0], raw[1], raw[2], raw[3]); dst[1] = make_uint4(raw[4], raw[5], raw[6], raw[7]);
+            }
         }
     __syncthreads();
     for (uint32_t b = threadIdx.x; b < nbin; b += PART_THREADS) hist[(size_t)b * gridDim.x + blockIdx.x] = sh[b];
     if (blockIdx.x == 0 && threadIdx.x == 0) hist[(size_t)nbin * gridDim.x] = 0;
 }
 template <int NW>
-__global__ void __launch_bounds__(PART_THREADS) k_part_scatter(const uint32_t *__restrict__ canon, uint32_t n, uint32_t n1, TableLayout L, uint32_t off1, uint32_t off2, uint32_t stride,
+__global__ void __launch_bounds__(PART_THREADS) k_part_scatter(const uint32_t *__restrict__ src1, const uint32_t *__restrict__ src2, uint32_t n, uint32_t n1, TableLayout L, uint32_t off1, uint32_t off2, uint32_t stride,
                                                                uint32_t nbin, const uint32_t *__restrict__ offs, uint32_t *__restrict__ out_val, uint16_t *__restrict__ out_key) {
     __shared__ uint32_t cursor[PART_NBIN_MAX], cnt[PART_NBIN_MAX], fill[PART_NBIN_MAX], st_val[PART_STAGE], st_key[PART_STAGE];
     __shared__ uint32_t wave_sums[PART_THREADS / 64], total;
@@ -1163,7 +1174,7 @@
             const uint32_t g = tile * PART_TILE + q * PART_THREADS + threadIdx.x;
             if (g < n) {
                 uint32_t raw[NW + 1];
-                const uint4 *src = reinterpret_cast<const uint4 *>(canon + (size_t)g * NW);
+                const uint4 *src = reinterpret_cast<const uint4 *>(g < n1 ? src1 + (size_t)g * NW : src2 + (size_t)(g - n1) * NW);
                 const uint4 a = src[0], b = src[1];
                 raw[0] = a.x; raw[1] = a.y; raw[2] = a.z; raw[3] = a.w; raw[4] = b.x; raw[5] = b.y; raw[6] = b.z; raw[7] = b.w; raw[NW] = 0;
                 part_digits<NW>(raw, L, d[q]);
@@ -1260,23 +1271,25 @@
     }
 }
 template <class Fr>
-static void partition_buckets(MsmWorkspace &S, const Fr *scal1, size_t n1, size_t off1, const Fr *scal2, size_t n2, size_t off2, const TableLayout &L, size_t stride, uint32_t cap, hipStream_t s) {
+static void partition_buckets(MsmWorkspace &S, const Fr *scal1, size_t n1, size_t off1, const Fr *scal2, size_t n2, size_t off2, const TableLayout &L, size_t stride, uint32_t cap, bool mont, hipStream_t s) {
     const int B = L.c_hi - 1;
     const uint32_t nbin = 1u << (B - PART_FINE_BITS), G = PART_GRID;
     const size_t n = n1 + n2, nb = (size_t)1 << B, nh = (size_t)nbin * G + 1;
-    S.canon.grow(n * Fr::N);
+    if (!mont) S.canon.grow(n * Fr::N);
     grow_together({nh, nh}, S.part_hist, S.part_offs);
+    const uint32_t *src1 = mont ? (const uint32_t *)scal1 : (const uint32_t *)S.canon, *src2 = mont ? (const uint32_t *)scal2 : src1 + n1 * Fr::N;
 #ifdef ZKAES_MEASURE
     for (int rep = (knockin() & 1) ? 0 : 1; rep < 2; rep++)
 #endif
     {
-    hipLaunchKernelGGL((k_part_hist<Fr>), dim3(G), dim3(PART_THREADS), 0, s, scal1, (uint32_t)n1, scal2, (uint32_t)n2, L, nbin, S.canon, S.part_hist);
+    if (mont) hipLaunchKernelGGL((k_part_hist<Fr, true>), dim3(G), dim3(PART_THREADS), 0, s, scal1, (uint32_t)n1, scal2, (uint32_t)n2, L, nbin, (uint32_t *)nullptr, S.part_hist);
+    else hipLaunchKernelGGL((k_part_hist<Fr, false>), dim3(G), dim3(PART_THREADS), 0, s, scal1, (uint32_t)n1, scal2, (uint32_t)n2, L, nbin, S.canon, S.part_hist);
     HIP_LAUNCH_CHECK();
     size_t tb = 0;
     HIP_CHECK(rocprim::exclusive_scan(nullptr, tb, S.part_hist.p, S.part_offs.p, 0u, nh, rocprim::plus<uint32_t>(), s));
     S.tmp.grow(tb);
     HIP_CHECK(rocprim::exclusive_scan(S.tmp.p, tb, S.part_hist.p, S.part_offs.p, 0u, nh, rocprim::plus<uint32_t>(), s));
-    hipLaunchKernelGGL((k_part_scatter<Fr::N>), dim3(G), dim3(PART_THREADS), 0, s, (const uint32_t *)S.canon, (uint32_t)n, (uint32_t)n1, L, (uint32_t)off1, (uint32_t)off2, (uint32_t)stride, nbin,
+    hipLaunchKernelGGL((k_part_scatter<Fr::N>), dim3(G), dim3(PART_THREADS), 0, s, src1, src2, (uint32_t)n, (uint32_t)n1, L, (uint32_t)off1, (uint32_t)off2, (uint32_t)stride, nbin,
                        (const uint32_t *)S.part_offs, S.vals_a, (uint16_t *)S.keys_a.p);
     HIP_LAUNCH_CHECK();
     hipLaunchKernelGGL(k_part_fine, dim3(nbin), dim3(PART_FINE_THREADS), 0, s, (const uint32_t *)S.part_offs, G, (const uint32_t *)S.vals_a, (const uint16_t *)S.keys_a.p, S.vals_b, S.start, S.end);
@@ -1288,7 +1301,7 @@
 
 template <class Curve>
 void msm_prepare_table(MsmWorkspace *ws_, const typename Curve::Fr *scal1, size_t n1, size_t off1, const typename Curve::Fr *scal2, size_t n2, size_t off2, int c, size_t stride,
-                       stream_t s_) {
+                       stream_t s_, bool mont_digits) {
     using Fr = typename Curve::Fr;
     hipStream_t s = (hipStream_t)s_;
     if (!ws_) throw GpuError("msm: null workspace");
@@ -1309,11 +1322,18 @@
     ensure_scratch(S, pairs, nb, cap);
     const int B = L.c_hi - 1;
     if (B > PART_FINE_BITS && (1u << (B - PART_FINE_BITS)) <= PART_NBIN_MAX && nwin <= PART_MAXW && pairs >= ((size_t)1 << 16)) {
-        partition_buckets<Fr>(S, scal1, n1, off1, scal2, n2, off2, L, stride, cap, s);
+        partition_buckets<Fr>(S, scal1, n1, off1, scal2, n2, off2, L, stride, cap, mont_digits, s);
         return;
     }
-    if (n1) { hipLaunchKernelGGL((k_digits_table<Fr>), dim3((unsigned)((n1 + 255) / 256)), dim3(256), 0, s, scal1, (uint32_t)n1, 0u, (uint32_t)n, (uint32_t)off1, L, (uint32_t)stride, S.keys_a, S.vals_a); HIP_LAUNCH_CHECK(); }
-    if (n2) { hipLaunchKernelGGL((k_digits_table<Fr>), dim3((unsigned)((n2 + 255) / 256)), dim3(256), 0, s, scal2, (uint32_t)n2, (uint32_t)n1, (uint32_t)n, (uint32_t)off2, L, (uint32_t)stride, S.keys_a, S.vals_a); HIP_LAUNCH_CHECK(); }
+    auto digits = [&](const Fr *sc, size_t cnt, size_t i_off, size_t val_off) {
+        if (!cnt) return;
+        const dim3 grid((unsigned)((cnt + 255) / 256));
+        if (mont_digits) hipLaunchKernelGGL((k_digits_table<Fr, true>), grid, dim3(256), 0, s, sc, (uint32_t)cnt, (uint32_t)i_off, (uint32_t)n, (uint32_t)val_off, L, (uint32_t)stride, S.keys_a, S.vals_a);
+        else hipLaunchKernelGGL((k_digits_table<Fr, false>), grid, dim3(256), 0, s, sc, (uint32_t)cnt, (uint32_t)i_off, (uint32_t)n, (uint32_t)val_off, L, (uint32_t)stride, S.keys_a, S.vals_a);
+        HIP_LAUNCH_CHECK();
+    };
+    digits(scal1, n1, 0, off1);
+    digits(scal2, n2, n1, off2);
     prepare_buckets<typename Curve::FqP>(S, pairs, L.c_hi - 1, 1, L.c_hi - 1, cap, s);
 }
 template <class Curve>
@@ -1323,10 +1343,29 @@
     return msm_finish<Curve>(ws_, tables, s_);
 }
 template <class Curve>
-XYZZ<typename Curve::Fq> msm_table(MsmWorkspace *ws_, const Niels28<typename Curve::FqP> *tables, size_t stride, size_t off, int c, const typename Curve::Fr *scalars, size_t n, stream_t s_) {
+XYZZ<typename Curve::Fq> msm_table(MsmWorkspace *ws_, const Niels28<typename Curve::FqP> *tables, size_t stride, size_t off, int c, const typename Curve::Fr *scalars, size_t n, stream_t s_,
+                                   bool mont_digits) {
     if (n == 0) return XYZZ<typename Curve::Fq>::inf();
-    msm_prepare_table<Curve>(ws_, scalars, n, off, nullptr, 0, 0, c, stride, s_);
-    return msm_finish<Curve>(ws_, tables, s_);
+    msm_prepare_table<Curve>(ws_, scalars, n, off, nullptr, 0, 0, c, stride, s_, mont_digits);
+    const XYZZ<typename Curve::Fq> sum = msm_finish<Curve>(ws_, tables, s_);
+    return mont_digits ? msm_unmont<Curve>(sum) : sum;
+}
+
+template <class Curve>
+XYZZ<typename Curve::Fq> msm_unmont(const XYZZ<typename Curve::Fq> &p) {
+    using Fq = typename Curve::Fq;
+    if (p.is_inf()) return XYZZ<Fq>::inf();
+    const uint32_t *k = Curve::ID == 377 ? FR377_RINV : FR381_RINV;
+    XYZZ<Fq> tab[16];
+    tab[0] = XYZZ<Fq>::inf(); tab[1] = p;
+    for (int i = 2; i < 16; i++) { tab[i] = tab[i - 1]; tab[i].add(p); }
+    XYZZ<Fq> acc = XYZZ<Fq>::inf();
+    for (int w = Curve::Fr::N * 8 - 1; w >= 0; w--) {
+        if (!acc.is_inf()) for (int d = 0; d < 4; d++) acc = acc.dbl();
+        const uint32_t digit = (k[w >> 3] >> ((w & 7) * 4)) & 15u;
+        if (digit) acc.add(tab[digit]);
+    }
+    return acc;
 }
 
 template <class Fr>
@@ -1534,7 +1573,8 @@
 template XYZZ<Fq377> msm_finish<Bls377>(MsmWorkspace *, const Niels28<Fq377P> *, stream_t);
 template void msm_finish2<Bls377>(MsmWorkspace *, const Niels28<Fq377P> *, const Niels28<Fq377P> *, XYZZ<Fq377> *, stream_t);
 template XYZZ<Fq377> msm<Bls377>(MsmWorkspace *, const Niels28<Fq377P> *, const Fr377 *, size_t, stream_t);
-template XYZZ<Fq377> msm_table<Bls377>(MsmWorkspace *, const Niels28<Fq377P> *, size_t, size_t, int, const Fr377 *, size_t, stream_t);
+template XYZZ<Fq377> msm_table<Bls377>(MsmWorkspace *, const Niels28<Fq377P> *, size_t, size_t, int, const Fr377 *, size_t, stream_t, bool);
+template XYZZ<Fq377> msm_unmont<Bls377>(const XYZZ<Fq377> &);
 template bool class_sum<Bls377>(MsmWorkspace *, const Niels28<Fq377P> *, const int8_t *, size_t, XYZZ<Fq377> *, stream_t);
 
 template void msm_table_sum_device<Bls377>(MsmWorkspace *, const Niels28<Fq377P> *, size_t, size_t, int, const Fr377 *, size_t, XYZZ<Fq377> *, stream_t);
@@ -1546,8 +1586,8 @@
 template void msm_window_sums_device<Bls381>(MsmWorkspace *, const Affine28<Fq381P> *, const Fr381 *, size_t, size_t, XYZZ<Fq381> *, stream_t);
 template XYZZ<Fq377> msm_fold_window_sums_device<Bls377>(const XYZZ<Fq377> *, int, size_t, stream_t);
 template XYZZ<Fq381> msm_fold_window_sums_device<Bls381>(const XYZZ<Fq381> *, int, size_t, stream_t);
-template void msm_prepare_table<Bls377>(MsmWorkspace *, const Fr377 *, size_t, size_t, const Fr377 *, size_t, size_t, int, size_t, stream_t);
-template void msm_prepare_table<Bls381>(MsmWorkspace *, const Fr381 *, size_t, size_t, const Fr381 *, size_t, size_t, int, size_t, stream_t);
+template void msm_prepare_table<Bls377>(MsmWorkspace *, const Fr377 *, size_t, size_t, const Fr377 *, size_t, size_t, int, size_t, stream_t, bool);
+template void msm_prepare_table<Bls381>(MsmWorkspace *, const Fr381 *, size_t, size_t, const Fr381 *, size_t, size_t, int, size_t, stream_t, bool);
 template XYZZ<Fq377> msm_table<Bls377>(MsmWorkspace *, const Affine28<Fq377P> *, size_t, size_t, int, const Fr377 *, size_t, stream_t);
 template XYZZ<Fq381> msm_table<Bls381>(MsmWorkspace *, const Affine28<Fq381P> *, size_t, size_t, int, const Fr381 *, size_t, stream_t);
 template void convert_bases<Bls377>(Affine28<Fq377P> *, const Affine<Fq377> *, size_t, stream_t);
diff --git a/aes_zero_knowledge_proof_circuit_amd/csrc/marlin.cpp b/aes_zero_knowledge_proof_circuit_amd/csrc/marlin.cpp
--- a/aes_zero_knowledge_proof_circuit_amd/csrc/marlin.cpp
+++ b/aes_zero_knowledge_proof_circuit_amd/csrc/marlin.cpp
@@ -297,6 +297,8 @@
     }
 
     bool table_ok(const ProverContext &, size_t len) const { return use_tables && len >= table_min_n; }
+    bool mont_ok(const ProverContext &cx, size_t len) const { return cx.throughput && table_ok(cx, len); }
+    static XYZZ<Fq377> unmont(const XYZZ<Fq377> &p) { return gpu::msm_unmont<Bls377>(p); }
     using Lane = ProverContext::Lane;
     XYZZ<Fq377> msm_powers(ProverContext &cx, Lane &ln, bool shifted, size_t off, const F *scalars, size_t len) {
         if (len == 0) return XYZZ<Fq377>::inf();
@@ -328,8 +330,9 @@
         const bool bounded = lp.bound >= 0;
         const size_t off = bounded ? (max_degree - (size_t)lp.bound) - lowest_shift : 0;
         if (len > supported_degree + 1 || (bounded && off + len > bounds[1] + 1)) throw std::runtime_error("KZG10: polynomial degree exceeds the committer key");
+        const bool mont = mont_ok(cx, len);
         if (len) {
-            if (table_ok(cx, len)) gpu::msm_prepare_table<Bls377>(ln.ws, coeffs, len, 0, nullptr, 0, 0, table_c, srs_stride, ln.stream);
+            if (table_ok(cx, len)) gpu::msm_prepare_table<Bls377>(ln.ws, coeffs, len, 0, nullptr, 0, 0, table_c, srs_stride, ln.stream, mont);
             else gpu::msm_prepare<Bls377>(ln.ws, coeffs, len, nullptr, 0, 0, ln.stream);
         }
         XYZZ<Fq377> c12[2] = {XYZZ<Fq377>::inf(), XYZZ<Fq377>::inf()}, h12[2] = {XYZZ<Fq377>::inf(), XYZZ<Fq377>::inf()};
@@ -338,17 +341,23 @@
         if (len) {
             if (bounded) gpu::msm_finish2<Bls377>(ln.ws, d_powers, d_shifted + off, c12, ln.stream);
             else c12[0] = gpu::msm_finish<Bls377>(ln.ws, d_powers, ln.stream);
+            if (mont) { c12[0] = unmont(c12[0]); if (bounded) c12[1] = unmont(c12[1]); }
         }
         c12[0].add(h12[0]);
         lp.comm.comm = c12[0].to_affine();
         if (bounded) { c12[1].add(h12[1]); lp.comm.shifted = c12[1].to_affine(); lp.comm.has_shifted = true; }
     }
-    void msm_opening_prepare(ProverContext &cx, Lane &ln, const F *wit, size_t wlen, const F *swit, size_t slen, size_t shift_off) {
+    bool msm_opening_prepare(ProverContext &cx, Lane &ln, const F *wit, size_t wlen, const F *swit, size_t slen, size_t shift_off) {
         if (wlen > supported_degree + 1 || shift_off + slen > bounds[1] + 1) throw std::runtime_error("KZG10: polynomial degree exceeds the committer key");
-        if (table_ok(cx, wlen + slen)) gpu::msm_prepare_table<Bls377>(ln.ws, wit, wlen, 0, swit, slen, lowest_shift + shift_off, table_c, srs_stride, ln.stream);
+        const bool mont = mont_ok(cx, wlen + slen);
+        if (table_ok(cx, wlen + slen)) gpu::msm_prepare_table<Bls377>(ln.ws, wit, wlen, 0, swit, slen, lowest_shift + shift_off, table_c, srs_stride, ln.stream, mont);
         else gpu::msm_prepare<Bls377>(ln.ws, wit, wlen, swit, slen, lowest_shift + shift_off, ln.stream);
-    }
-    XYZZ<Fq377> msm_opening_finish(Lane &ln) { return gpu::msm_finish<Bls377>(ln.ws, d_powers, ln.stream); }
+        return mont;
+    }
+    XYZZ<Fq377> msm_opening_finish(Lane &ln, bool mont) {
+        const XYZZ<Fq377> sum = gpu::msm_finish<Bls377>(ln.ws, d_powers, ln.stream);
+        return mont ? unmont(sum) : sum;
+    }
     bool use_lanes = true;
     struct RoundJobs {
         ProvingKeyImpl &K; ProverContext &cx;
@@ -782,7 +791,7 @@
         if (!R.early_evals) gpu::divide_by_linear(cx.wit2.p, cx.poly[5].p, cx.poly_len[5], R.beta, cx.scratch.p, cx.scratch.n, ls_);
         gpu::divide_by_linear(cx.wit.p, cx.acc.p, plen, R.beta, cx.scratch.p, cx.scratch.n, ls_);
         gpu::poly_scale(cx.wit2.p, chp[1], cx.poly_len[5] - 1, ls_);
-        msm_opening_prepare(cx, ln, cx.wit.p, plen - 1, cx.wit2.p, cx.poly_len[5] - 1, bounds[1] - (n - 2));
+        const bool mont = msm_opening_prepare(cx, ln, cx.wit.p, plen - 1, cx.wit2.p, cx.poly_len[5] - 1, bounds[1] - (n - 2));
         XYZZ<Fq377> hw = XYZZ<Fq377>::inf();
         Fr rq[2]; host_divide_by_linear(rq, rb, R.beta);
         for (int i = 0; i < 2; i++) hw.add(srs->gamma_tab[i].mul(rq[i]));
@@ -791,7 +800,7 @@
         host_divide_by_linear(rq, srb, R.beta);
         for (int i = 0; i < 2; i++) hw.add(srs->gamma_tab[i].mul(rq[i]));
         rv = rv + host_eval3(srb, R.beta);
-        XYZZ<Fq377> w = msm_opening_finish(ln);
+        XYZZ<Fq377> w = msm_opening_finish(ln, mont);
         w.add(hw);
         R.pf.w_beta = w.to_affine(); R.pf.random_v_beta = rv;
     }, false);
@@ -813,8 +822,8 @@
             gpu::divide_by_linear(wit2_.p, cx.poly[7].p, cx.poly_len[7], R.gamma, scr_.p, scr_.n, ls_);
             gpu::poly_scale(wit2_.p, chp[1], cx.poly_len[7] - 1, ls_);
         }
-        msm_opening_prepare(cx, ln, wit_.p, plen - 1, wit2_.p, cx.poly_len[7] - 1, bounds[1] - (k - 2));
-        XYZZ<Fq377> w = msm_opening_finish(ln);
+        const bool mont = msm_opening_prepare(cx, ln, wit_.p, plen - 1, wit2_.p, cx.poly_len[7] - 1, bounds[1] - (k - 2));
+        XYZZ<Fq377> w = msm_opening_finish(ln, mont);
         R.pf.w_gamma = w.to_affine();
     }, false);
     if (R.jobs.async) {
diff --git a/aes_zero_knowledge_proof_circuit_amd/csrc/te28.cuh b/aes_zero_knowledge_proof_circuit_amd/csrc/te28.cuh
--- a/aes_zero_knowledge_proof_circuit_amd/csrc/te28.cuh
+++ b/aes_zero_knowledge_proof_circuit_amd/csrc/te28.cuh
@@ -20,6 +20,7 @@
     ZK_HD static G k2d() { constexpr uint32_t t[14] = FQ377_TE_K2D_28_INIT; return lit28(t); }
     ZK_HD static G si() { constexpr uint32_t t[14] = FQ377_TE_SI_28_INIT; return lit28(t); }
     ZK_HD static G sif() { constexpr uint32_t t[14] = FQ377_TE_SIF_28_INIT; return lit28(t); }
+    ZK_HD static G di() { constexpr uint32_t t[14] = FQ377_TE_DI_28_INIT; return lit28(t); }
 };
 
 template <class P>
@@ -66,6 +67,41 @@
 #pragma unroll
     for (int i = 0; i < G::N; i++) { F.l[i] = neg ? V.l[i] : U.l[i]; Gg.l[i] = neg ? U.l[i] : V.l[i]; }
     a.x = G::mul_biased(E, F, bias); a.y = G::mul_biased(Gg, H, bias); a.t = G::mul_biased(E, H, bias); a.z = G::mul_biased(F, Gg, bias);
+}
+template <class P>
+ZK_HD void te_seed_sums(AccTE<P> &r, FpMsm<P> &td, const Niels28<P> &n, bool neg) {
+    using G = FpMsm<P>;
+    r.x = n.ypx.template sub<2>(n.ymx).template canonical_below<1>();
+    r.y = (n.ypx + n.ymx).template canonical_below<1>();
+    r.z = G::k_one().dbl().template canonical_below<1>();
+    const G ntd = G::zero().template sub<2>(n.td);
+    const bool flip = neg && !n.td.limbs_zero();
+#pragma unroll
+    for (int i = 0; i < G::N; i++) td.l[i] = flip ? ntd.l[i] : n.td.l[i];
+}
+template <class P>
+ZK_HD AccTE<P> te_seed_from_niels(const Niels28<P> &n, bool neg) {
+    AccTE<P> r;
+    FpMsm<P> td;
+    te_seed_sums<P>(r, td, n, neg);
+    r.t = td * Te377::di();
+    return r;
+}
+template <class P>
+ZK_HD AccTE<P> te_seed_hot(Niels28<P> &n, bool neg, const Niels28<P> *next, bool next_neg) {
+    using G = FpMsm<P>;
+    AccTE<P> r;
+    G td;
+    te_seed_sums<P>(r, td, n, neg);
+#if defined(__HIP_DEVICE_COMPILE__)
+    asm volatile("" : "+v"(r.x.l[G::N - 1]), "+v"(r.y.l[G::N - 1]), "+v"(td.l[G::N - 1]) : : "memory");
+#endif
+    n = niels_load_signed<P>(next, next_neg);
+#if defined(__HIP_DEVICE_COMPILE__)
+    asm volatile("" : "+v"(td.l[0]) : : "memory");
+#endif
+    r.t = td * Te377::di();
+    return r;
 }
 template <class P>
 ZK_HD void te_add_inline(AccTE<P> &a, const AccTE<P> &b) {
diff --git a/include/zkaes.h b/include/zkaes.h
--- a/include/zkaes.h
+++ b/include/zkaes.h
@@ -153,6 +153,8 @@
 int zkaes_srs_hold(int hold);
 int zkaes_msm_table(int curve_id, const uint8_t *bases, const uint8_t *scalars, size_t n, int window_bits, uint8_t *out_xy, int *out_inf);
 int zkaes_msm_table_srs(const uint8_t *bases, const uint8_t *scalars, size_t n, int window_bits, uint8_t *out_xy, int *out_inf);
+#define ZKAES_MSM_MONT_DIGITS 1u
+int zkaes_msm_table_srs_flags(const uint8_t *bases, const uint8_t *scalars, size_t n, int window_bits, unsigned flags, uint8_t *out_xy, int *out_inf);
 int zkaes_msm_bench(int curve_id, const uint8_t *bases, const uint8_t *scalars, size_t n, int reps, double *ms_total, double *ms_accumulate);
 int zkaes_msm_bench_synth(size_t n, int window_bits, int reps, double *ms_total, double *ms_accumulate, uint8_t *out_xy);
 int zkaes_stream_copy_bench(size_t bytes, int reps, double *gb_per_s);
```

New measurement: 96.56 (median of 6 runs). No clear change (+0.9%).
